# disanda/Deep-GAN-Encoders

Measured on AMD Instinct MI355X. Metric: encoder-train images/sec (E_align_s2 step, StyleGAN2 FFHQ-1024), higher is better.
Workload: dtype bf16; 1 GPU; E_align_s2 two-phase step, StyleGAN2-1024 G (train mode) + BE(startf=16, L=9) + LPIPS-VGG16 (seeded stand-in weights), batch 8/GPU; global_batch=8, img_size=1024, parallelism=dp1

## Files before the change

deep-gan-encoders_amd/_lib.py:

```python
import ctypes as C
import os

_HERE = os.path.dirname(os.path.abspath(__file__))
LIB_PATH = os.environ.get("DGE_LIB_PATH", os.path.join(_HERE, "libdge_hip.so"))


class DgeError(RuntimeError):
    pass


class ConvDesc(C.Structure):
    _fields_ = [
        ("x", C.c_void_p), ("w_packed", C.c_void_p), ("y", C.c_void_p), ("addend", C.c_void_p), ("dot_src", C.c_void_p),
        ("in_scale", C.c_void_p), ("in_shift", C.c_void_p), ("out_scale", C.c_void_p),
        ("bias", C.c_void_p), ("noise", C.c_void_p), ("noise_w", C.c_void_p), ("stats", C.c_void_p),
        ("B", C.c_int), ("H", C.c_int), ("W", C.c_int), ("Cin", C.c_int), ("Cout", C.c_int),
        ("ksize", C.c_int), ("up", C.c_int), ("in_s2d", C.c_int), ("noise_batch", C.c_int), ("noise_w_per_channel", C.c_int),
        ("act", C.c_int), ("bias_scale", C.c_float), ("gain", C.c_float), ("add_scale", C.c_float),
        ("dtype", C.c_int), ("in_up2", C.c_int), ("in_relu", C.c_int), ("stats_slots", C.c_int), ("w_layout", C.c_int),
        ("prep", C.c_int), ("prep_gain", C.c_float), ("prep_noise", C.c_void_p), ("prep_ns", C.c_void_p), ("prep_noise_batch", C.c_int),
        ("prep_stats", C.c_void_p), ("mask_relu", C.c_int), ("in_t2d", C.c_int),
        ("rgb_w", C.c_void_p), ("rgb_style", C.c_void_p), ("rgb_bias", C.c_void_p), ("rgb_out", C.c_void_p), ("rgb_wscale", C.c_float),
        ("rgb_skip_y", C.c_int), ("pool_out", C.c_int), ("pool_mask", C.c_void_p),
        ("prefetch_w", C.c_void_p), ("prefetch_ntot", C.c_int), ("prefetch_cin", C.c_int), ("in_bwd_coef", C.c_void_p),
        ("in_bwd_extra", C.c_void_p), ("in_bwd_extra_scale", C.c_float), ("fr_img4", C.c_void_p), ("fr_out", C.c_void_p),
    ]


class ConvPPDesc(C.Structure):
    _fields_ = [
        ("x", C.c_void_p), ("w_pp", C.c_void_p), ("y", C.c_void_p), ("w_bstride", C.c_longlong),
        ("out_scale", C.c_void_p), ("bias", C.c_void_p), ("noise", C.c_void_p), ("noise_w", C.c_void_p),
        ("B", C.c_int), ("H", C.c_int), ("W", C.c_int), ("Cin", C.c_int), ("Cout", C.c_int),
        ("noise_batch", C.c_int), ("noise_w_per_channel", C.c_int), ("act", C.c_int), ("bias_scale", C.c_float), ("gain", C.c_float),
        ("dgrad", C.c_int), ("in_s2d", C.c_int), ("stats_slots", C.c_int), ("prep", C.c_int), ("prep_noise_batch", C.c_int), ("mask_relu", C.c_int),
        ("in_t2d", C.c_int), ("add_scale", C.c_float), ("prep_gain", C.c_float),
        ("dot_src", C.c_void_p), ("addend", C.c_void_p), ("stats", C.c_void_p), ("prep_stats", C.c_void_p), ("prep_noise", C.c_void_p), ("prep_ns", C.c_void_p),
    ]


class DenseLayer(C.Structure):
    _fields_ = [("w", C.c_void_p), ("bias", C.c_void_p), ("I", C.c_int), ("O", C.c_int), ("wscale", C.c_float), ("bscale", C.c_float),
                ("add", C.c_float), ("act", C.c_int), ("gain", C.c_float)]


class S2GradEntry(C.Structure):
    _fields_ = [("P", C.c_void_p), ("st", C.c_void_p), ("d", C.c_void_p), ("s", C.c_void_p), ("bias", C.c_void_p), ("wsq", C.c_void_p),
                ("gs", C.c_void_p), ("wstyle", C.c_void_p),
                ("nslot_p", C.c_int), ("nslot_s", C.c_int), ("in_c", C.c_int), ("out_c", C.c_int), ("row", C.c_int), ("bscale", C.c_float)]


class SumPlanarEntry(C.Structure):
    _fields_ = [("partial", C.c_void_p), ("out", C.c_void_p), ("nslot", C.c_int), ("C", C.c_int), ("NS", C.c_int), ("pad", C.c_int)]


_P, _I, _F = C.c_void_p, C.c_int, C.c_float
SIGNATURES = {
    "dge_conv2d": [C.POINTER(ConvDesc), _P],
    "dge_fir_t2d": [_P, _P, _P, _I, _I, _I, _I, _I, _P],
    "dge_s2_style_grads": [C.POINTER(S2GradEntry), _I, _P, _I, _I, _I, _F, _P],
    "dge_conv_small_supported": [_I, _I, _I, _I, _I, _I, _I, _I],
    "dge_torgb_bwd_prep": [_P, _P, _P, _P, _P, _P, _I, _P, _P, _P, _I, _I, _I, _F, _F, _I, _P],
    "dge_demod_bwd_prep": [_P, _I, _P, _P, _P, _I, _I, _F, _P],
    "dge_sum_slots": [_P, _P, _I, _I, _I, _P],
    "dge_sum_slots_planar": [_P, _P, _I, _I, _I, _P],
    "dge_set_deterministic": [_I],
    "dge_get_deterministic": [],
    "dge_packed_n": [_I],
    "dge_pack_conv_weight": [_P, _P, _I, _I, _I, _I, _I, _F, _P],
    "dge_pack_conv_weights_multi": [_P, _P, _I, _I, _P],
    "dge_pack_desc_bytes": [],
    "dge_weight_sumsq": [_P, _P, _I, _I, _I, _F, _P],
    "dge_linear": [_P, _I, _P, _P, _P, _I, _I, _I, _I, _F, _F, _F, _I, _F, _I, _P],
    "dge_pixelnorm": [_P, _P, _I, _I, _F, _P],
    "dge_truncation": [_P, _P, _P, _I, _I, _I, _F, _I, _I, _P],
    "dge_torgb": [_P, _P, _P, _P, _P, _P, _I, _I, _I, _I, _F, _I, _P],
    "dge_conv_rgb_supported": [_I, _I, _I, _I, _I, _I, _I],
    "dge_conv_in_bwd_supported": [_I, _I, _I, _I, _I, _I, _I],
    "dge_conv_in_bwd_fromrgb_supported": [_I, _I, _I, _I, _I, _I, _I],
    "dge_conv_in_bwd_x_supported": [_I, _I, _I, _I, _I, _I, _I],
    "dge_conv_pool_supported": [_I, _I, _I, _I, _I, _I, _I],
    "dge_rgb_upsample_add": [_P, _P, _I, _I, _I, _P],
    "dge_nchw_to_nhwc": [_P, _P, _I, _I, _I, _I, _I, _P],
    "dge_nhwc_to_nchw": [_P, _P, _I, _I, _I, _I, _P],
    "dge_fromrgb": [_P, _P, _P, _P, _P, _I, _I, _I, _I, _P],
    "dge_fromrgb2": [_P, _P, _P, _P, _P, _P, _I, _I, _I, _I, _P],
    "dge_stats_finalize": [_P, _P, _P, _P, _I, _I, _I, _F, _P],
    "dge_stats_finalize_slots": [_P, _I, _P, _P, _P, _I, _I, _I, _F, _P],
    "dge_blend": [_P, _P, _P, _P, _P, _P, _I, _I, _I, _I, _I, _F, _F, _I, _P],
    "dge_loss_reduce": [_P, _P, _P, _I, _I, _I, _I, _I, _I, _I, _I, _P],
    "dge_ssim_fwd": [_P, _P, _P, _P, _I, _I, _I, _P],
    "dge_ssim_box7": [_P, _P, _P, _I, _I, _I, _F, _F, _F, _P],
    "dge_ssim_bwd": [_P, _P, _P, _P, _I, _I, _I, _F, _I, _P],
    "dge_space_loss_finalize": [_P, _P, _P, _P, _F, _F, _I, _P],
    "dge_space_loss_bwd": [_P, _P, _P, _P, _P, _I, _I, _I, _I, _I, _I, _I, _I, _F, _F, _I, _P],
    "dge_axpy_scalar": [_P, _P, _P, C.c_long, _F, _I, _P],
    "dge_lreq_adam_multi": [_I, _P, _P, _P, _P, _P, _F, _F, _P, _P, _P],
    "dge_modconv_bwd_prep": [_P, _P, _P, _P, _P, _P, _I, _I, _I, _I, _F, _I, _P],
    "dge_demod_bwd": [_P, _P, _P, _P, _P, _I, _I, _F, _P],
    "dge_linear_t": [_P, _I, _I, _P, _P, _P, _I, _I, _I, _I, _I, _F, _I, _P],
    "dge_torgb_bwd": [_P, _P, _P, _P, _P, _P, _I, _I, _I, _F, _I, _P],
    "dge_up2_bwd": [_P, _P, _I, _I, _I, _P],
    "dge_conv_wgrad": [_P, _P, _P, _P, _P, _I, _I, _I, _I, _I, _I, _I, _P],
    "dge_act_bwd": [_P, _P, _P, _P, _P, _I, _I, _I, _I, _I, _I, _F, _F, _I, _P],
    "dge_in_bwd_coef": [_P, _P, _P, _P, _P, _P, _I, _I, _I, _P],
    "dge_in_bwd_coef_slots": [_P, _I, _P, _P, _P, _P, _P, _I, _I, _I, _P],
    "dge_in_bwd": [_P, _P, _P, _P, _P, _P, _P, _I, _I, _I, _I, _I, _F, _I, _I, _P],
    "dge_chan_sum": [_P, _P, _I, _I, _I, _F, _I, _P],
    "dge_fromrgb_bwd": [_P, _P, _P, _P, _I, _I, _I, _I, _P],
    "dge_head_entry_size": [],
    "dge_heads_bwd": [_P, _I, _I, _P, _I, _P, _P, _P, _P, _I, _I, _P],
    "dge_head_rows_entry_size": [],
    "dge_heads_rows_fwd": [_P, _I, _P, _P, C.c_long, C.c_long, _I, _I, _I, _P],
    "dge_heads_rows_bwd": [_P, _I, _I, _P, C.c_long, C.c_long, _I, _P, _P, _P, _P, _I, _I, _P],
    "dge_dense_wgrad": [_P, _I, _P, _I, _P, _P, _I, _I, _I, _I, _P],
    "dge_lpips_prep": [_P, _P, _I, _I, _I, _P, _P, _I, _P],
    "dge_lpips_prep_bwd": [_P, _P, _I, _I, _I, _P, _F, _I, _I, _P],
    "dge_maxpool2": [_P, _P, _I, _I, _I, _I, _I, _P],
    "dge_maxpool2_bwd": [_P, _P, _P, _P, _I, _I, _I, _I, _I, _P],
    "dge_lpips_head": [_P, _P, _P, _P, _I, _I, _I, _F, _I, _P],
    "dge_mean": [_P, _P, _I, _P],
    "dge_blur_noise_act": [_P, _P, _P, _P, _P, _P, _I, _I, _I, _I, _I, _I, _I, _I, _P],
    "dge_affine_compose": [_P, _P, _P, _P, _P, _I, _I, _P],
    "dge_lerp_layers": [_P, _P, _I, _P, _P, _I, _I, _I, _P],
    "dge_linear_rows": [_P, _I, _P, _P, _P, _P, _P, _P, _I, _I, _I, _F, _F, _F, _P],
    "dge_demod_rows": [_P, _P, _P, _P, _P, _P, _P, _P, _I, _I, _F, _P],
    "dge_fromrgb_dgrad": [_P, _P, _P, _P, _I, _I, _I, _I, _P],
    "dge_nearest_up2": [_P, _P, _I, _I, _I, _I, _F, _I, _P],
    "dge_sg1_in_bwd_coef": [_P, _P, _P, _P, _P, _P, _I, _I, _I, _P],
    "dge_dot_stats": [_P, _P, _P, _I, _I, _I, _I, _P],
    "dge_nearest_up2_bwd": [_P, _P, _P, _P, _I, _I, _I, _I, _I, _P],
    "dge_pixelnorm_nhwc": [_P, _P, C.c_long, _I, _F, _I, _P],
    "dge_pixelnorm_nhwc_bwd": [_P, _P, _P, C.c_long, _I, _F, _I, _P],
    "dge_pixelnorm_act_bwd": [_P, _P, _P, _I, _I, _I, _I, _I, _I, _F, _I, _P],
    "dge_affine_relu_bwd": [_P, _P, _P, _P, _P, _P, _I, _I, _I, _I, _P],
    "dge_slice_up_bwd": [_P, _P, _I, _I, _I, _I, _I, _I, _I, _P],
    "dge_softmax_rows": [_P, C.c_long, _I, _I, _P],
    "dge_softmax_rows_bwd": [_P, _P, C.c_long, _I, _I, _P],
    "dge_rgb_tanh_bwd": [_P, _P, _P, _I, _I, _I, _I, _P],
    "dge_sn_group": [_P, _I, _I, _I, _P, _F, _I, _P],
    "dge_sn_entry_size": [],
    "dge_cbn_sn_wgrad_entry_size": [],
    "dge_cbn_sn_wgrad_group": [_P, _I, C.c_longlong, _I, _P, _I, _I, _P, _P],
    "dge_upconv_supported": [_I, _I, _I],
    "dge_pack_upconv_weight": [_P, _P, _I, _I, _F, _I, _P],
    "dge_upconv_fir": [_P, _P, _P, _P, _P, _P, _I, _P, _I, _P, _F, _F, _I, _I, _I, _I, _I, _I, _I, _P],
    "dge_up_dgrad_stream_supported": [_I, _I, _I, _I, _I, _I],
    "dge_up_dgrad_stream": [_P, _P, _P, _P, _P, _P, _P, _P, _I, _I, _F, _P, _I, _P, _P, _I, _I, _I, _I, _I, _I, _P],
    "dge_cbn_affine": [_P, _P, _I, _P, _P, _F, _P, _P, _I, _I, _P],
    "dge_slice_up": [_P, _P, _I, _I, _I, _I, _I, _I, _I, _P],
    "dge_attention": [_P, _P, _P, _P, _I, _I, _I, _I, _I, _I, _P],
    "dge_rgb_tanh": [_P, _P, _I, _I, _I, _I, _P],
    "dge_guided_relu_bwd": [_P, _P, _P, C.c_long, _I, _I, _P],
    "dge_maxpool2_relu_bwd": [_P, _P, _P, _I, _I, _I, _I, _I, _I, _P],
    "dge_maxpool2_bwd_relu": [_P, _P, _P, _P, _I, _I, _I, _I, _I, _P],
    "dge_adaptive_pool7": [_P, _P, _I, _I, _I, _I, _I, _P],
    "dge_adaptive_pool7_bwd": [_P, _P, _I, _I, _I, _I, _I, _P],
    "dge_class_target": [_P, _P, _P, _P, _I, _I, _P],
    "dge_gather_row": [_P, _P, _P, _I, _I, _F, _P],
    "dge_class_target_rows": [_P, _P, _P, _P, _I, _I, _P],
    "dge_gather_rows": [_P, _P, _P, _I, _I, _P],
    "dge_campp_map": [_P, _P, _P, _P, _P, _I, _I, _I, _I, _I, _P],
    "dge_cam_resize": [_P, _P, _P, _I, _I, _I, _I, _I, _P],
    "dge_mask2cam_blocks": [_I],
    "dge_mask2cam": [_P, _P, _P, _P, _P, _P, _P, _I, _I, _P],
    "dge_mask2cam_rows": [_P, _P, _P, _P, _P, _P, _I, _I, _P],
    "dge_class_target_groups": [_P, _P, _P, _P, _I, _I, _I, _P],
    "dge_gather_row_groups": [_P, _P, _P, _I, _I, _I, _F, _P],
    "dge_mask2cam_groups": [_P, _P, _P, _P, _P, _P, _P, _I, _I, _I, _P],
    "dge_randn": [_P, _I, _P, _P, _P, _P, C.c_ulonglong, _P, _P],
    "dge_version": [],
    "dge_env_reload": [],
    "dge_blend_pool_mask": [_P, _P, _P, _P, _P, _I, _I, _I, _I, _F, _F, _I, _P],
    "dge_act_bwd_mask": [_P, _P, _P, _P, _P, _I, _I, _I, _I, _I, _F, _F, _I, _P],
    "dge_loss_reduce3": [_P, _P, _P, _I, _I, _I, _I, _P, _I, _P],
    "dge_crop_pool_multi": [_P, _P, _P, _P, _I, _I, _I, _I, _P],
    "dge_space_loss_bwd3": [_P, _P, _P, _P, _P, _I, _I, _I, _P, _P, _P, _P, _I, _P],
    "dge_space_loss_bwd_split": [_P, _P, _P, _P, _P, _I, _I, _I, _P, _P, _P, _P, _I, _P],
    "dge_in_bwd_fromrgb": [_P, _P, _P, _I, _P, _P, _P, _P, _I, _P, _P, _P, _I, _I, _I, _I, _I, _F, _I, _P],
    "dge_in_bwd_fromrgb_img": [_P, _P, _P, _I, _P, _P, _P, _P, _I, _P, _P, _P, _P, _P, _I, _I, _I, _I, _I, _F, _I, _P],
    "dge_affine_bwd_fromrgb_img": [_P, _P, _P, _P, _P, _P, _P, _P, _I, _I, _I, _I, _I, _F, _I, _P],
    "dge_in_bwd_fused": [_P, _P, _P, _I, _P, _P, _P, _P, _I, _P, _P, _P, _P, _I, _I, _I, _I, _I, _F, _I, _I, _P],
    "dge_sum_slots_planar_multi": [C.POINTER(SumPlanarEntry), _I, _P],
    "dge_heads_fwd": [_P, _I, _P, _P, _I, _I, _I, _P],
    "dge_conv_pp_supported": [_I, _I, _I, _I, _I, _I],
    "dge_pack_conv_pp": [_P, _P, _I, _I, _F, _P, _P, _F, _I, _I, _P],
    "dge_dense_chain": [_P, _I, C.POINTER(DenseLayer), _I, _P, _I, _I, _I, _F, _P],
    "dge_conv_wgrad_dots": [_P, _P, _P, _P, _P, _P, _P, _I, _I, _I, _I, _I, _I, _I, _P],
    "dge_pack_conv_pp_rows": [_P, _I, _P, _I, _I, _P, _I, _P, _F, _I, _I, _P],
    "dge_conv_pp": [C.POINTER(ConvPPDesc), _P],
    "dge_up_pp_supported": [_I, _I, _I, _I, _I, _I],
    "dge_pack_up_pp": [_P, _P, _I, _I, _P, _P, _F, _I, _P],
    "dge_up_pp": [_P, _P, C.c_longlong, _P, _P, _I, _P, _P, _F, _F, _I, _I, _I, _I, _I, _I, _P],
    "dge_latent_pnorm_fwd": [_P, _P, _P, C.c_long, _I, _P],
    "dge_latent_pnorm_bwd": [_P, _P, _P, _P, C.c_long, _I, _F, _P],
    "dge_wplus_lerp": [_P, _P, _I, _F, _P, _I, _I, _I, _P],
    "dge_wplus_lerp_bwd": [_P, _F, _P, C.c_long, _I, _P],
    "dge_embed_track": [_P, _P, _P, C.c_long, _P, _P, _P, _P, _P, _I, _I, _I, _F, _F, _P],
    "dge_loss_reduce_rows": [_P, _P, _P, _I, _I, _I, _I, _P, _I, _I, _P],
    "dge_ssim_fwd_rows": [_P, _P, _P, _P, _I, _I, _I, _P],
    "dge_space_loss_finalize_rows": [_P, _I, _P, _P, _P, _P, _P, _I, _I, _P, _P, _I, _P],
    "dge_space_loss_bwd_rows": [_P, _P, _P, _P, _P, _I, _I, _I, _I, _P, _P, _P, _P, _I, _I, _P],
    "dge_latent_pnorm_rows_fwd": [_P, _P, _P, _I, C.c_long, _I, _P],
    "dge_latent_pnorm_rows_bwd": [_P, _P, _P, _P, _I, C.c_long, _I, _F, _P],
    "dge_embed_track_rows": [_P, _P, _P, _I, C.c_long, _P, _P, _P, _P, _P, _I, _I, _I, _F, _F, _P],
    "dge_mapping_bwd": [_P, _I, C.POINTER(DenseLayer), _I, _P, _P, _I, _P, _P, _I, _I, _I, _F, _P],
    "dge_quantize_u8": [_P, _I, _P, _I, _I, _I, _I, _P],
    "dge_image_metrics_u8_work_bytes": [_I, _I, _I],
    "dge_image_metrics_u8": [_P, _P, _I, _I, _I, _P, _P, _P, _P, _P],
    "dge_minmax_unit_slots": [C.c_long],
    "dge_minmax_unit": [_P, _P, C.c_long, _P, _P],
}

_lib = None


def lib():
    global _lib
    if _lib is None:
        if not os.path.exists(LIB_PATH):
            raise DgeError(f"{LIB_PATH} is missing: build it with deep-gan-encoders_amd/csrc/build.sh "
                           "(__graft_entry__.build()). There is no fallback path.")
        _lib = C.CDLL(LIB_PATH)
        for name, args in SIGNATURES.items():
            fn = getattr(_lib, name)
            fn.argtypes = args
            fn.restype = C.c_int
        for name in ("dge_last_error", "dge_last_kernel"):
            getattr(_lib, name).restype = C.c_char_p
            getattr(_lib, name).argtypes = []
        if os.environ.get("DGE_DETERMINISTIC") == "1":
            import torch
            if torch.cuda.is_available() and _lib.dge_set_deterministic(1) != 0:
                raise DgeError("DGE_DETERMINISTIC=1: " + _lib.dge_last_error().decode())
    return _lib


def last_kernel():
    return lib().dge_last_kernel().decode()


def check(rc, what=""):
    if rc != 0:
        raise DgeError(f"{what} failed ({rc}): {lib().dge_last_error().decode()}")
```

deep-gan-encoders_amd/csrc/capi.hip:

```cpp
#include <stdarg.h>
#include <stdio.h>
#include "common.h"
#include "conv_params.h"
#include "../../include/dge_hip.h"

static thread_local char g_err[512] = "";
void dge_set_error(const char* fmt, ...) {
    va_list ap; va_start(ap, fmt); vsnprintf(g_err, sizeof(g_err), fmt, ap); va_end(ap);
}
extern "C" const char* dge_last_error(void) { return g_err; }
static thread_local char g_kernel[160] = "";
void dge_note_kernel(const char* fmt, ...) {
    va_list ap; va_start(ap, fmt); vsnprintf(g_kernel, sizeof(g_kernel), fmt, ap); va_end(ap);
}
extern "C" const char* dge_last_kernel(void) { return g_kernel; }
extern "C" int dge_version(void) { return 100; }

#include <vector>
static std::vector<void (*)(const DgeDet*)>& det_setters() { static std::vector<void (*)(const DgeDet*)> v; return v; }
void dge_det_register(void (*setter)(const DgeDet*)) { det_setters().push_back(setter); }
static DgeDet g_det_host = {0, nullptr, nullptr, 0, 0};
int dge_det_upload_failed = 0;
bool dge_det_fits(long long ndomains, long long nslots, long long L) {
    return !g_det_host.enabled || (ndomains * nslots * L <= g_det_host.ws_floats && ndomains <= (long long)g_det_host.ncounters);
}
extern "C" int dge_set_deterministic(int on) {
    if (on && !g_det_host.ws) {
        const long long nf = 32LL << 20;
        const int nc = 1 << 16;
        float* ws = nullptr; unsigned* ct = nullptr;
        DGE_CHECK(hipMalloc((void**)&ws, (size_t)nf * 4) == hipSuccess, "set_deterministic: workspace allocation failed");
        DGE_CHECK(hipMalloc((void**)&ct, (size_t)nc * 4) == hipSuccess, "set_deterministic: counter allocation failed");
        DGE_CHECK(hipMemset(ct, 0, (size_t)nc * 4) == hipSuccess, "set_deterministic: counter reset failed");
        g_det_host.ws = ws; g_det_host.counters = ct; g_det_host.ws_floats = nf; g_det_host.ncounters = nc;
    }
    g_det_host.enabled = on ? 1 : 0;
    DGE_CHECK(hipDeviceSynchronize() == hipSuccess, "set_deterministic: device synchronisation failed");
    dge_det_upload_failed = 0;
    for (auto f : det_setters()) f(&g_det_host);
    DGE_CHECK(hipDeviceSynchronize() == hipSuccess && !dge_det_upload_failed, "set_deterministic: state upload failed");
    return 0;
}
extern "C" int dge_get_deterministic(void) { return g_det_host.enabled; }

static DgeEnv g_env;
static bool g_env_loaded = false;
static int env_int(const char* name, int dflt) { const char* e = getenv(name); return e ? atoi(e) : dflt; }
static void env_load() {
    g_env.force_stream = getenv("DGE_FORCE_STREAM") ? 1 : 0;
    g_env.no_stream = getenv("DGE_NO_STREAM") ? 1 : 0;
    g_env.no_pw = getenv("DGE_NO_PW") ? 1 : 0;
    g_env.stream_nseg = env_int("DGE_STREAM_NSEG", 0);
    g_env.conv_dbg = env_int("DGE_CONV_DBG", 0);
    g_env.conv_bn = env_int("DGE_CONV_BN", 0);
    g_env.conv_kc = env_int("DGE_CONV_KC", 0);
    g_env.conv_small = env_int("DGE_CONV_SMALL", -1);
    g_env.conv_nok4 = getenv("DGE_CONV_NOK4") ? 1 : 0;
    g_env.conv_nok2 = getenv("DGE_CONV_NOK2") ? 1 : 0;
    g_env.torgb_thread = getenv("DGE_TORGB_THREAD") ? 1 : 0;
    g_env.wgrad_th8 = getenv("DGE_WGRAD_TH8") ? 1 : 0;
    g_env.wgrad_groups = env_int("DGE_WGRAD_GROUPS", 0);
    if (g_env.wgrad_groups < 0) g_env.wgrad_groups = 0;
    g_env.up_dbg = env_int("DGE_UP_DBG", 0);
    { const char* v = getenv("DGE_UP_VARIANT"); g_env.up_variant = !v ? 0 : (v[0] == 's' ? 2 : 1); }
    g_env_loaded = true;
}
#include <mutex>
static std::once_flag g_env_once;
const DgeEnv& dge_env() { std::call_once(g_env_once, [] { if (!g_env_loaded) env_load(); }); return g_env; }
extern "C" void dge_env_reload(void) { env_load(); }

extern "C" int dge_conv2d(const dge_conv_desc* d, hipStream_t s) {
    DGE_CHECK(d && d->x && d->w_packed && d->y, "conv2d: null tensor");
    DGE_CHECK(d->B > 0 && d->H > 0 && d->W > 0 && d->Cin > 0 && d->Cout > 0, "conv2d: bad shape");
    DGE_CHECK(d->dtype == DGE_F32 || d->dtype == DGE_BF16, "conv2d: bad dtype %d", d->dtype);
    DGE_CHECK(!(d->up && d->stats), "conv2d: stats are not available in up mode");
    DGE_CHECK(!(d->up && d->in_s2d), "conv2d: up and in_s2d are exclusive");
    DGE_CHECK(!d->in_up2 || (!d->in_s2d && d->H % 2 == 0 && d->W % 2 == 0), "conv2d: in_up2 needs even H, W and no in_s2d");
    DGE_CHECK(!d->in_s2d || d->Cin % 4 == 0, "conv2d: in_s2d needs Cin %% 4 == 0");
    DGE_CHECK(!d->dot_src || d->stats || d->mask_relu || d->in_bwd_coef, "conv2d: dot_src needs a stats buffer");
    DGE_CHECK(!d->mask_relu || (d->dot_src && !d->prep && !d->up), "conv2d: mask_relu needs dot_src and excludes prep / up");
    DGE_CHECK(!d->in_relu || d->in_scale || d->in_shift, "conv2d: in_relu is applied together with the prologue affine");
    DGE_CHECK(d->gain > 0.f, "conv2d: gain must be positive (it is folded through the activation)");
    DGE_CHECK((((uintptr_t)d->in_scale | (uintptr_t)d->in_shift) & 15) == 0, "conv2d: in_scale/in_shift must be 16-byte aligned");
    DGE_CHECK(!d->noise || d->noise_w, "conv2d: noise without noise_w");
    ConvParams p;
    p.x = d->x; p.w = d->w_packed; p.y = d->y; p.addend = d->addend; p.dot_src = d->dot_src;
    p.in_scale = d->in_scale; p.in_shift = d->in_shift; p.out_scale = d->out_scale;
    p.bias = d->bias; p.noise = d->noise; p.noise_w = d->noise_w; p.stats = d->stats;
    p.B = d->B; p.H = d->H; p.W = d->W; p.Cin = d->Cin; p.Cout = d->Cout;
    p.Ntot_valid = d->up ? 4 * d->Cout : d->Cout;
    p.Ntot = dge_packed_n(p.Ntot_valid);
    p.up = d->up; p.in_s2d = d->in_s2d; p.in_up2 = d->in_up2; p.in_relu = d->in_relu;
    const int OH = d->up ? 2 * d->H : d->H, OW = d->up ? 2 * d->W : d->W;
    p.noise_bstride = d->noise_batch > 1 ? OH * OW : 0;
    p.noise_w_stride = d->noise_w_per_channel ? 1 : 0;
    p.act = d->act; p.bias_scale = d->bias_scale; p.gain = d->gain; p.add_scale = d->add_scale;
    p.tiles_x = p.tiles_y = 0;
    p.w_frag = d->w_layout == 1 ? 1 : 0;
    p.prep = d->prep ? 1 : 0;
    p.mask_relu = d->mask_relu ? 1 : 0;
    p.in_t2d = d->in_t2d ? 1 : 0;
    DGE_CHECK(!d->in_t2d || (d->ksize == 3 && !d->up && !d->in_s2d && !d->in_up2 && !d->in_scale && !d->in_shift && d->w_layout == 0),
              "conv2d: in_t2d is a plain 3x3 launch (no other read mode, no prologue affine, row-major weights)");
    p.prep_gain = d->prep_gain; p.prep_noise = d->prep_noise; p.prep_ns = d->prep_ns; p.prep_stats = d->prep_stats;
    p.prep_noise_bstride = d->prep_noise_batch > 1 ? OH * OW : 0;
    DGE_CHECK(!d->prep || (d->dot_src && d->prep_stats && d->prep_gain > 0.f && !d->up), "conv2d: prep needs dot_src, prep_stats, a positive prep_gain and no up mode");
    DGE_CHECK(!d->prep || !dge_get_deterministic(), "conv2d: the fused tail backward (prep) is not offered in deterministic mode; run dge_modconv_bwd_prep");
    DGE_CHECK(d->w_layout == 0 || d->w_layout == 1, "conv2d: bad w_layout %d", d->w_layout);
    p.stats_slots = d->stats_slots > 0 ? d->stats_slots : 1;
    p.rgb_w = d->rgb_out ? d->rgb_w : nullptr; p.rgb_style = d->rgb_style; p.rgb_bias = d->rgb_bias; p.rgb_out = d->rgb_out;
    p.rgb_wscale = d->rgb_wscale; p.rgb_skip_y = (d->rgb_out && d->rgb_skip_y) ? 1 : 0;
    p.pool_out = d->pool_out ? 1 : 0; p.pool_mask = d->pool_out ? (unsigned*)d->pool_mask : nullptr;
    const bool pf = d->w_layout == 1 && d->prefetch_w && d->prefetch_ntot >= 64 && d->prefetch_ntot % 64 == 0 &&
                    (d->prefetch_cin == 512 || d->prefetch_cin == 256);
    p.pf_w = pf ? d->prefetch_w : nullptr; p.pf_ntot = pf ? d->prefetch_ntot : 0; p.pf_cin = pf ? d->prefetch_cin : 0;
    p.in_coef = d->in_bwd_coef;
    p.in_extra = d->in_bwd_coef ? d->in_bwd_extra : nullptr; p.in_extra_scale = d->in_bwd_extra_scale;
    p.fr_img4 = d->in_bwd_coef ? d->fr_img4 : nullptr; p.fr_out = d->in_bwd_coef ? d->fr_out : nullptr;
    if (d->in_bwd_coef) {
        DGE_CHECK(!dge_get_deterministic(), "conv2d: in_bwd_coef is not offered in deterministic mode; run dge_in_bwd");
        DGE_CHECK(d->ksize == 3 && !d->up && dge_conv_stream_eligible(p, d->dtype, d->ksize), "conv2d: in_bwd_coef is offered where "
                  "dge_conv_in_bwd_supported() says so, with dot_src and prep_stats, without stats / prep");
    }
    if (d->pool_out)
        DGE_CHECK(!d->up && dge_conv_pool_ok(p, d->dtype, d->ksize), "conv2d: the pooled epilogue is offered where dge_conv_pool_supported() "
                  "says so (conv_2 of the first encoder blocks on the streaming kernel)");
    if (d->rgb_out) {
        DGE_CHECK(d->rgb_w && d->rgb_style && d->rgb_bias, "conv2d: rgb_out needs rgb_w, rgb_style, rgb_bias");
        DGE_CHECK(dge_conv_rgb_ok(p, d->dtype, d->ksize), "conv2d: the fused toRGB is offered where dge_conv_rgb_supported() says so "
                  "(bf16 3x3 32 -> 32 launches of the streaming kernel)");
    }
    return dge_conv_launch(p, d->dtype, d->ksize, s);
}

extern "C" int dge_conv_pool_supported(int B, int H, int W, int Cin, int Cout, int ksize, int dtype) {
    ConvParams p = {};
    p.B = B; p.H = H; p.W = W; p.Cin = Cin; p.Cout = Cout; p.Ntot_valid = Cout; p.Ntot = dge_packed_n(Cout);
    p.in_shift = (const float*)16; p.noise_w_stride = 1;
    return dge_conv_pool_ok(p, dtype, ksize) ? 1 : 0;
}

extern "C" int dge_conv_in_bwd_supported(int B, int H, int W, int Cin, int Cout, int ksize, int dtype) {
    ConvParams p = {};
    p.B = B; p.H = H; p.W = W; p.Cin = Cin; p.Cout = Cout; p.Ntot_valid = Cout; p.Ntot = dge_packed_n(Cout);
    p.dot_src = (const void*)16; p.prep_stats = (float*)16; p.in_coef = (const float*)16;
    return (ksize == 3 && !dge_get_deterministic() && dge_conv_stream_eligible(p, dtype, ksize)) ? 1 : 0;
}
extern "C" int dge_conv_in_bwd_x_supported(int B, int H, int W, int Cin, int Cout, int ksize, int dtype) {
    ConvParams p = {};
    p.B = B; p.H = H; p.W = W; p.Cin = Cin; p.Cout = Cout; p.Ntot_valid = Cout; p.Ntot = dge_packed_n(Cout);
    p.dot_src = (const void*)16; p.in_coef = (const float*)16;
    return (ksize == 3 && !dge_get_deterministic() && dge_conv_stream_eligible(p, dtype, ksize)) ? 1 : 0;
}
extern "C" int dge_conv_in_bwd_fromrgb_supported(int B, int H, int W, int Cin, int Cout, int ksize, int dtype) {
    ConvParams p = {};
    p.B = B; p.H = H; p.W = W; p.Cin = Cin; p.Cout = Cout; p.Ntot_valid = Cout; p.Ntot = dge_packed_n(Cout);
    p.dot_src = (const void*)16; p.in_coef = (const float*)16; p.fr_img4 = (const float*)16; p.fr_out = (float*)16;
    return (ksize == 3 && !dge_get_deterministic() && dge_conv_stream_eligible(p, dtype, ksize)) ? 1 : 0;
}

extern "C" int dge_conv_rgb_supported(int B, int H, int W, int Cin, int Cout, int ksize, int dtype) {
    ConvParams p = {};
    p.B = B; p.H = H; p.W = W; p.Cin = Cin; p.Cout = Cout; p.Ntot_valid = Cout; p.Ntot = dge_packed_n(Cout);
    return dge_conv_rgb_ok(p, dtype, ksize) ? 1 : 0;
}

__global__ void sum_slots_kernel(const float* __restrict__ partial, float* __restrict__ out, int nslot, int n, int accumulate) {
    const int i = blockIdx.x * blockDim.x + threadIdx.x;
    if (i >= n) return;
    float s = 0.f;
    int k = 0;
    for (; k + 8 <= nslot; k += 8) {
        float v[8];
#pragma unroll
        for (int j = 0; j < 8; j++) v[j] = partial[(size_t)(k + j) * n + i];
#pragma unroll
        for (int j = 0; j < 8; j++) s += v[j];
    }
    for (; k < nslot; k++) s += partial[(size_t)k * n + i];
    out[i] = accumulate ? out[i] + s : s;
}
__global__ void sum_slots_planar_kernel(const float* __restrict__ partial, float* __restrict__ out, int nslot, int C, int NS) {
    const int i = blockIdx.x * blockDim.x + threadIdx.x;
    if (i >= C * NS) return;
    float s = 0.f;
    int k = 0;
    for (; k + 8 <= nslot; k += 8) {
        float v[8];
#pragma unroll
        for (int j = 0; j < 8; j++) v[j] = partial[(size_t)(k + j) * C * NS + i];
#pragma unroll
        for (int j = 0; j < 8; j++) s += v[j];
    }
    for (; k < nslot; k++) s += partial[(size_t)k * C * NS + i];
    out[(size_t)(i % NS) * C + i / NS] = s;
}
extern "C" int dge_sum_slots_planar(const float* partial, float* out, int nslot, int C, int NS, hipStream_t s) {
    DGE_CHECK(nslot >= 1 && C >= 1 && NS >= 1, "sum_slots_planar: bad sizes");
    hipLaunchKernelGGL(sum_slots_planar_kernel, dim3((C * NS + 255) / 256), dim3(256), 0, s, partial, out, nslot, C, NS);
    DGE_LAUNCH_CHECK("sum_slots_planar");
    return 0;
}
struct SumPlanarTable { dge_sum_planar_entry e[32]; };
__global__ void sum_slots_planar_multi_kernel(SumPlanarTable tab) {
    const dge_sum_planar_entry e = tab.e[blockIdx.y];
    const int n = e.C * e.NS;
    for (int i = blockIdx.x * blockDim.x + threadIdx.x; i < n; i += gridDim.x * blockDim.x) {
        float s = 0.f;
        int k = 0;
        for (; k + 8 <= e.nslot; k += 8) {
            float v[8];
#pragma unroll
            for (int j = 0; j < 8; j++) v[j] = e.partial[(size_t)(k + j) * n + i];
#pragma unroll
            for (int j = 0; j < 8; j++) s += v[j];
        }
        for (; k < e.nslot; k++) s += e.partial[(size_t)k * n + i];
        e.out[(size_t)(i % e.NS) * e.C + i / e.NS] = s;
    }
}
extern "C" int dge_sum_slots_planar_multi(const dge_sum_planar_entry* entries, int n, hipStream_t s) {
    DGE_CHECK(entries && n >= 1 && n <= 32, "sum_slots_planar_multi: 1..32 entries");
    SumPlanarTable tab;
    int maxn = 1;
    for (int i = 0; i < n; i++) {
        const dge_sum_planar_entry& e = entries[i];
        DGE_CHECK(e.partial && e.out && e.nslot >= 1 && e.C >= 1 && e.NS >= 1, "sum_slots_planar_multi: bad entry %d", i);
        tab.e[i] = e;
        if (e.C * e.NS > maxn) maxn = e.C * e.NS;
    }
    hipLaunchKernelGGL(sum_slots_planar_multi_kernel, dim3((maxn + 255) / 256, n), dim3(256), 0, s, tab);
    DGE_LAUNCH_CHECK("sum_slots_planar_multi");
    return 0;
}
extern "C" int dge_sum_slots(const float* partial, float* out, int nslot, int n, int accumulate, hipStream_t s) {
    hipLaunchKernelGGL(sum_slots_kernel, dim3((n + 255) / 256), dim3(256), 0, s, partial, out, nslot, n, accumulate);
    DGE_LAUNCH_CHECK("sum_slots");
    return 0;
}
```

deep-gan-encoders_amd/csrc/conv_params.h:

```cpp
#pragma once
#include <hip/hip_runtime.h>

struct ConvParams {
    const void* x;
    const void* w;
    void* y;
    const void* addend;
    const void* dot_src;
    const float* in_scale;
    const float* in_shift;
    const float* out_scale;
    const float* bias;
    const float* noise;
    const float* noise_w;
    float* stats;
    int stats_slots;
    int B, H, W, Cin, Cout;
    int Ntot;
    int Ntot_valid;
    int up;
    int in_s2d;
    int in_relu;
    int in_up2;
    int noise_bstride;
    int noise_w_stride;
    int act;
    float bias_scale, gain, add_scale;
    int tiles_x, tiles_y;
    int dbg;
    int w_frag;
    int prep;
    float prep_gain;
    const float* prep_noise;
    const float* prep_ns;
    int prep_noise_bstride;
    float* prep_stats;
    int mask_relu;
    int in_t2d;
    const float* rgb_w;
    const float* rgb_style;
    const float* rgb_bias;
    float* rgb_out;
    float rgb_wscale;
    int rgb_skip_y;
    int pool_out;
    unsigned* pool_mask;
    const void* pf_w;
    int pf_ntot, pf_cin;
    const float* in_coef;
    const void* in_extra; float in_extra_scale; const float* fr_img4; float* fr_out;
};

int dge_conv_launch(const ConvParams& p, int dtype, int ksize, hipStream_t s);
extern "C" int dge_conv_ntile(int ntot);

bool dge_conv_stream_eligible(const ConvParams& p, int dtype, int ksize);
int dge_conv_stream_launch(const ConvParams& p, hipStream_t s);
bool dge_conv_rgb_ok(const ConvParams& p, int dtype, int ksize);
bool dge_conv_pool_ok(const ConvParams& p, int dtype, int ksize);
bool dge_conv_small_shape_ok(int H, int W, int cin, int ntot, int ksize, int in_s2d, int in_up2, int dtype);
int dge_conv_small_launch(const ConvParams& p, hipStream_t s);
bool dge_conv_pw_eligible(const ConvParams& p, int dtype, int ksize);
int dge_conv_pw_launch(const ConvParams& p, hipStream_t s);
```

deep-gan-encoders_amd/csrc/conv_small.hip:

```cpp
#include <stdlib.h>
#include "common.h"
#include "conv_params.h"
#include "conv_epilogue.h"

namespace {

struct SmallCfg {
    static constexpr int MT = 1, NT = 1, WTM = 32, WTN = 32, BM = 64;
    static constexpr int ESTR = 32 * 4 + 16;
};
constexpr int TH = 8, TW = 8, BN = 64, HH = 10, HW = 10, CIN_MAX = 512;
__host__ __device__ constexpr int pstr_of(int cin) { return 2 * cin + 16; }
__host__ __device__ constexpr int rpitch_of(int cin) { return HW * pstr_of(cin) + 224; }
constexpr int A_MAX = HH * rpitch_of(CIN_MAX);
constexpr int RED_BYTES = 8 * 2 * 16 * 64 * 4;
constexpr int EST_BYTES = 4 * 32 * SmallCfg::ESTR;
constexpr int N_BYTES = 4 * SmallCfg::BM * 4;
constexpr int PF_BYTES = 8 * 256;
constexpr int LDS_BYTES = A_MAX + N_BYTES + PF_BYTES;
static_assert(RED_BYTES + EST_BYTES <= A_MAX, "reduction + staging must fit the halo region");

__device__ __forceinline__ unsigned lds_base_u32(const void* p) {
    return (unsigned)(size_t)(const __attribute__((address_space(3))) unsigned char*)p;
}
__device__ __forceinline__ f32x16_t mma(const uint4& a, const uint4& b, f32x16_t c) {
    return __builtin_amdgcn_mfma_f32_32x32x16_bf16(*(const bf16x8_t*)&a, *(const bf16x8_t*)&b, c, 0, 0, 0);
}

template <int KQ, int MODE>
__global__ __launch_bounds__(512, 2) void conv_small_kernel(ConvParams p) {
    constexpr int CIN = KQ * 64, CH = CIN / 8;
    constexpr int PSTR = pstr_of(CIN), RPITCH = rpitch_of(CIN);
    constexpr int KST = CIN / 16;
    __shared__ __attribute__((aligned(256))) unsigned char lds[LDS_BYTES];
    float* ldsN = (float*)(lds + A_MAX);
    const int tid = threadIdx.x, lane = tid & 63;
    const int wave = __builtin_amdgcn_readfirstlane(tid >> 6);
    int bid = blockIdx.x;
    {
        const int nb = gridDim.x, per = nb >> 3;
        if (per > 0 && bid < (per << 3)) bid = (bid & 7) * per + (bid >> 3);
    }
    const int vbid = bid;
    const int tx_i = bid % p.tiles_x; bid /= p.tiles_x;
    const int ty_i = bid % p.tiles_y; bid /= p.tiles_y;
    const int b = bid % p.B;
    const int ntile = bid / p.B;
    const int x0 = tx_i * TW, y0 = ty_i * TH, bn0 = ntile * BN;
    const int nt = wave & 1, kq = wave >> 1;

    const unsigned char* wbase = (const unsigned char*)p.w + ((size_t)(bn0 / 32 + nt) * KST + kq * KQ) * 1024 + lane * 16;
    const size_t tap_stride = (size_t)(p.Ntot / 32) * KST * 1024;
    constexpr int PF = KQ >= 8 ? 3 : 4;
    uint4 bw[PF + 1][KQ];
#pragma unroll
    for (int t = 0; t < PF; t++)
#pragma unroll
        for (int j = 0; j < KQ; j++) bw[t][j] = *(const uint4*)(wbase + t * tap_stride + j * 1024);

    auto prefetch_next = [&]() {
        const int xcd = blockIdx.x & 7, r = blockIdx.x >> 3, R = max(1, (int)gridDim.x >> 3);
        const int nt_n = p.pf_ntot / BN, kst_n = p.pf_cin / 16;
        const int n_lo = xcd * nt_n / 8, n_hi = max(n_lo + 1, (xcd + 1) * nt_n / 8);
        const unsigned lines_tap = (unsigned)(n_hi - n_lo) * 2u * kst_n * 8u;
        const unsigned nlines = 9u * lines_tap;
        const size_t tap_stride_n = (size_t)(p.pf_ntot / 32) * kst_n * 1024;
        const unsigned m0v = lds_base_u32(lds) + A_MAX + N_BYTES + wave * 256;
        for (unsigned l = (unsigned)r * 512u + tid; l - lane < nlines; l += (unsigned)R * 512u) {
            const unsigned tp = l / lines_tap, within = l - tp * lines_tap;
            const unsigned char* a = (const unsigned char*)p.pf_w + tp * tap_stride_n + (size_t)n_lo * 2 * kst_n * 1024 + (size_t)within * 128;
            if (l >= nlines) a = (const unsigned char*)p.pf_w;
            asm volatile("s_mov_b32 m0, %1\n\ts_nop 0\n\tglobal_load_lds_dword %0, off" : : "v"(a), "s"(m0v) : "memory");
        }
    };
    const bool pf_late = gridDim.x <= 256;
    if (p.pf_w && !pf_late) prefetch_next();

    {
        const bf16_t* __restrict__ Xb = (const bf16_t*)p.x + (size_t)b * p.H * p.W * CIN;
        const bool affine = p.in_scale || p.in_shift;
        const int chunk = tid % CH;
        float asc[8], ash[8];
        if (affine) {
            const int ci = b * CIN + chunk * 8;
#pragma unroll
            for (int e = 0; e < 8; e++) { asc[e] = p.in_scale ? p.in_scale[ci + e] : 1.f; ash[e] = p.in_shift ? p.in_shift[ci + e] : 0.f; }
        }
        constexpr int NITEM = HH * HW * CH, NPER = (NITEM + 511) / 512;
        uint4 v[NPER];
        unsigned inmask = 0;
#pragma unroll
        for (int i = 0; i < NPER; i++) {
            const int idx = tid + i * 512;
            const int pix = idx / CH, hx = pix % HW, hy = pix / HW;
            const int gy = y0 + hy - 1, gx = x0 + hx - 1;
            const bool inside = ((unsigned)gy < (unsigned)p.H) & ((unsigned)gx < (unsigned)p.W) & (idx < NITEM);
            v[i] = make_uint4(0, 0, 0, 0);
            if (inside) v[i] = *(const uint4*)(Xb + (gy * p.W + gx) * CIN + chunk * 8);
            inmask |= (inside ? 1u : 0u) << i;
        }
        const float* __restrict__ nz_src = p.prep ? p.prep_noise : p.noise;
        if (nz_src) {
            const int nz_bs = p.prep ? p.prep_noise_bstride : p.noise_bstride;
            const int OWn = p.up ? 2 * p.W : p.W;
            const int nph = p.up ? 4 : 1;
            for (int idx = tid; idx < nph * SmallCfg::BM; idx += 512) {
                const int m = idx % SmallCfg::BM, ph = idx / SmallCfg::BM;
                const int gy = y0 + m / TW, gx = x0 + m % TW;
                const int oy = p.up ? 2 * gy + (ph >> 1) : gy, ox = p.up ? 2 * gx + (ph & 1) : gx;
                ldsN[idx] = (gy < p.H && gx < p.W) ? nz_src[(size_t)b * nz_bs + (size_t)oy * OWn + ox] : 0.f;
            }
        }
#pragma unroll
        for (int i = 0; i < NPER; i++) {
            const int idx = tid + i * 512;
            if (idx < NITEM) {
                const int pix = idx / CH, hx = pix % HW, hy = pix / HW;
                uint4 q = v[i];
                if (affine && ((inmask >> i) & 1u)) {
                    float f[8];
                    unpack16(q, f, (bf16_t*)nullptr);
#pragma unroll
                    for (int e = 0; e < 8; e++) f[e] = f[e] * asc[e] + ash[e];
                    if (p.in_relu) {
#pragma unroll
                        for (int e = 0; e < 8; e++) f[e] = fmaxf(f[e], 0.f);
                    }
                    q = pack16(f, (bf16_t*)nullptr);
                }
                *(uint4*)(lds + hy * RPITCH + hx * PSTR + chunk * 16) = q;
            }
        }
    }
    __syncthreads();

    f32x16_t acc[2];
#pragma unroll
    for (int g = 0; g < 2; g++)
#pragma unroll
        for (int r = 0; r < 16; r++) acc[g][r] = 0.f;
    int aoff[2];
#pragma unroll
    for (int g = 0; g < 2; g++) {
        const int m = g * 32 + (lane & 31);
        aoff[g] = (m / TW) * RPITCH + (m % TW) * PSTR + kq * KQ * 32 + (lane >> 5) * 16;
    }
    StaticFor<9>::run([&](auto tc) {
        constexpr int tap = decltype(tc)::value;
        constexpr int dy = tap / 3, dx = tap % 3;
        if (tap + PF < 9) {
            const unsigned char* wn = wbase + (size_t)(tap + PF) * tap_stride;
#pragma unroll
            for (int j = 0; j < KQ; j++) bw[(tap + PF) % (PF + 1)][j] = *(const uint4*)(wn + j * 1024);
        }
        const unsigned char* at = lds + dy * RPITCH + dx * PSTR;
#pragma unroll
        for (int j = 0; j < KQ; j++) {
            const uint4 a0 = *(const uint4*)(at + aoff[0] + j * 32);
            const uint4 a1 = *(const uint4*)(at + aoff[1] + j * 32);
            acc[0] = mma(a0, bw[tap % (PF + 1)][j], acc[0]);
            acc[1] = mma(a1, bw[tap % (PF + 1)][j], acc[1]);
        }
    });

    if (p.pf_w && pf_late) prefetch_next();
    __syncthreads();
    float* red = (float*)lds;
#pragma unroll
    for (int g = 0; g < 2; g++)
#pragma unroll
        for (int r = 0; r < 16; r++) red[((wave * 2 + g) * 16 + r) * 64 + lane] = acc[g][r];
    __syncthreads();
    const bool carrier = wave < 4;
    f32x16_t tile[1][1];
    if (carrier) {
        const int wm = wave >> 1, wn = wave & 1;
#pragma unroll
        for (int r = 0; r < 16; r++) {
            float s = 0.f;
#pragma unroll
            for (int q = 0; q < 4; q++) s += red[(((q * 2 + wn) * 2 + wm) * 16 + r) * 64 + lane];
            tile[0][0][r] = s;
        }
    }
    conv_epilogue<bf16_t, SmallCfg, TH, TW, BN, 2, 2, 512, MODE>(p, tile, lds + RED_BYTES, ldsN, b, x0, y0, bn0, ntile, vbid, tx_i, ty_i,
                                                            wave, lane, tid, carrier);
    if (p.pf_w) asm volatile("s_waitcnt vmcnt(0)" ::: "memory");
}

int max_hw() {
    static const int v = [] { const char* e = getenv("DGE_SMALL_MAXHW"); const int n = e ? atoi(e) : 24; return n < 0 ? 0 : n; }();
    return v;
}

}

bool dge_conv_small_shape_ok(int H, int W, int cin, int ntot, int ksize, int in_s2d, int in_up2, int dtype) {
    return dtype == DGE_BF16 && ksize == 3 && !in_s2d && !in_up2 && (cin == 512 || cin == 256) && ntot % BN == 0 && ntot >= BN &&
           H <= max_hw() && W <= max_hw();
}

extern "C" int dge_conv_small_supported(int H, int W, int cin, int ntot, int ksize, int in_s2d, int in_up2, int dtype) {
    return dge_conv_small_shape_ok(H, W, cin, ntot, ksize, in_s2d, in_up2, dtype) ? 1 : 0;
}

int dge_conv_small_launch(const ConvParams& p0, hipStream_t s) {
    ConvParams p = p0;
    p.dbg = 0;
    p.tiles_x = (p.W + TW - 1) / TW;
    p.tiles_y = (p.H + TH - 1) / TH;
    const long grid = (long)p.tiles_x * p.tiles_y * p.B * (p.Ntot / BN);
    DGE_CHECK(grid > 0 && grid < (1L << 31), "conv_small: bad grid");
    if (p.stats && !p.up)
        DGE_CHECK(dge_det_fits((long long)p.B * (p.Ntot / BN), (long long)p.tiles_x * p.tiles_y * 2, BN * 2),
                  "conv_small: the deterministic-mode workspace is too small for this launch");
    dge_note_kernel("conv_small<bf16,8,8,64,%d>%s", p.Cin, p.prep ? "+prep" : "");
    const int mode = p.prep ? 2 : ((p.addend || p.dot_src) ? 1 : 0);
#define DGE_GO(KQ, MODE) hipLaunchKernelGGL((conv_small_kernel<KQ, MODE>), dim3((unsigned)grid), dim3(512), 0, s, p)
    if (p.Cin == 512) { if (mode == 2) DGE_GO(8, 2); else if (mode == 1) DGE_GO(8, 1); else DGE_GO(8, 0); }
    else { if (mode == 2) DGE_GO(4, 2); else if (mode == 1) DGE_GO(4, 1); else DGE_GO(4, 0); }
#undef DGE_GO
    DGE_LAUNCH_CHECK("conv_small");
    return 0;
}
```

deep-gan-encoders_amd/csrc/s2_kernels.hip:

```cpp
#include <stdlib.h>
#include "common.h"
#include <vector>
#include <algorithm>
#include <string.h>
#include "conv_params.h"

__device__ __forceinline__ float sg1_up_weight(const float* __restrict__ w, int c, int o, int Cout, int ph, int tap) {
    const int py = ph >> 1, px = ph & 1, dy = tap / 3 - 1, dx = tap % 3 - 1;
    const int ky = py + 1 - 2 * dy, kx = px + 1 - 2 * dx;
    if (ky < 0 || ky > 3 || kx < 0 || kx > 3) return 0.f;
    const float* w3 = w + ((size_t)c * Cout + o) * 9;
    float v = 0.f;
    for (int a = 0; a < 2; a++)
        for (int bq = 0; bq < 2; bq++) {
            const int y = ky - a, x = kx - bq;
            if (y >= 0 && y < 3 && x >= 0 && x < 3) v += w3[y * 3 + x];
        }
    return v;
}

__device__ __forceinline__ float upfold_weight(const float* __restrict__ w, int o, int i, int Cin, int ph, int tap) {
    const int py = ph >> 1, px = ph & 1;
    const int dy = tap / 3 - 1, dx = tap % 3 - 1;
    const float k1[4] = {0.25f, 0.75f, 0.75f, 0.25f};
    float v = 0.f;
    for (int ty = 0; ty < 4; ty++) {
        const int wy = 3 - py - ty + 2 * dy;
        if (wy < 0 || wy > 2) continue;
        for (int tx = 0; tx < 4; tx++) {
            const int wx = 3 - px - tx + 2 * dx;
            if (wx < 0 || wx > 2) continue;
            v += k1[ty] * k1[tx] * w[((size_t)o * Cin + i) * 9 + wy * 3 + wx];
        }
    }
    return v;
}

__device__ __forceinline__ float upt2d_weight(const float* __restrict__ w, int o, int i, int Cin, int ph, int tap) {
    const int dy = tap / 3, dx = tap % 3;
    if (dy == 0 || dx == 0) return 0.f;
    const int ky = 2 * (dy - 1) + (ph >> 1), kx = 2 * (dx - 1) + (ph & 1);
    if (ky > 2 || kx > 2) return 0.f;
    return w[((size_t)o * Cin + i) * 9 + (2 - ky) * 3 + (2 - kx)];
}

__device__ __forceinline__ size_t pack_out_index(int frag, int tap, int n, int k, int Ntot, int Kdim) {
    if (!frag) return ((size_t)tap * Ntot + n) * Kdim + k;
    const size_t blk = ((size_t)tap * (Ntot >> 5) + (n >> 5)) * (Kdim >> 4) + (k >> 4);
    return blk * 512 + (size_t)(((n & 31) + 32 * ((k & 15) >> 3)) * 8 + (k & 7));
}

template <typename T>
__global__ void pack_weight_kernel(const float* __restrict__ w, T* __restrict__ out, int Cout, int Cin, int KS,
                                   int Ntot, int mode, float scale) {
    const int frag = mode & 0x100;
    mode &= 0xff;
    const int ntap = KS * KS;
    const int Kdim = (mode == 2) ? Cout : ((mode == 3 || mode == 5 || mode == 6) ? 4 * Cout : Cin);
    const int total = ntap * Ntot * Kdim;
    for (int idx = blockIdx.x * blockDim.x + threadIdx.x; idx < total; idx += gridDim.x * blockDim.x) {
        const int k = idx % Kdim;
        const int n = (idx / Kdim) % Ntot;
        const int tap = idx / (Kdim * Ntot);
        float v = 0.f;
        if (mode == 0) {
            if (n < Cout) v = w[((size_t)n * Cin + k) * ntap + tap];
        } else if (mode == 2) {
            if (n < Cin) v = w[((size_t)k * Cin + n) * ntap + (ntap - 1 - tap)];
        } else if (mode == 1) {
            if (n < 4 * Cout) v = upfold_weight(w, n % Cout, k, Cin, n / Cout, tap);
        } else if (mode == 4) {
            if (n < 4 * Cout) v = sg1_up_weight(w, k, n % Cout, Cout, n / Cout, tap);
        } else if (mode == 5) {
            if (n < Cin) v = sg1_up_weight(w, n, k % Cout, Cout, k / Cout, 8 - tap);
        } else if (mode == 6) {
            if (n < Cin) v = upt2d_weight(w, k % Cout, n, Cin, k / Cout, tap);
        } else {
            if (n < Cin) v = upfold_weight(w, k % Cout, n, Cin, k / Cout, 8 - tap);
        }
        Elem<T>::st(out + pack_out_index(frag, tap, n, k, Ntot, Kdim), v * scale);
    }
}

struct DgePackDesc {
    const float* w; void* out;
    int cout, cin, ks, ntot, mode, dtype, kdim;
    float scale;
    long long pair_start;
    long long tile_start;
    void* out2;
    int ntot2, kdim2, mode2, tiles_i;
};
__device__ __forceinline__ float pack_gather(const float* __restrict__ w, int mode, int Cout, int Cin, int ntap, int n, int k, int tap) {
    if (mode == 0) return n < Cout ? w[((size_t)n * Cin + k) * ntap + tap] : 0.f;
    if (mode == 2) return n < Cin ? w[((size_t)k * Cin + n) * ntap + (ntap - 1 - tap)] : 0.f;
    if (mode == 1) return n < 4 * Cout ? upfold_weight(w, n % Cout, k, Cin, n / Cout, tap) : 0.f;
    if (mode == 4) return n < 4 * Cout ? sg1_up_weight(w, k, n % Cout, Cout, n / Cout, tap) : 0.f;
    if (mode == 5) return n < Cin ? sg1_up_weight(w, n, k % Cout, Cout, k / Cout, 8 - tap) : 0.f;
    if (mode == 6) return n < Cin ? upt2d_weight(w, k % Cout, n, Cin, k / Cout, tap) : 0.f;
    return n < Cin ? upfold_weight(w, k % Cout, n, Cin, k / Cout, 8 - tap) : 0.f;
}
__global__ void pack_multi_kernel(const DgePackDesc* __restrict__ descs, int nd, long long total_pairs) {
    for (long long pidx = (long long)blockIdx.x * blockDim.x + threadIdx.x; pidx < total_pairs; pidx += (long long)gridDim.x * blockDim.x) {
        int lo = 0, hi = nd - 1;
        while (lo < hi) { const int mid = (lo + hi + 1) >> 1; if (descs[mid].pair_start <= pidx) lo = mid; else hi = mid - 1; }
        const DgePackDesc e = descs[lo];
        const long long local = pidx - e.pair_start;
        const int k = (int)(local % e.kdim), n = (int)(local / e.kdim);
        const int ntap = e.ks * e.ks;
        for (int tap = 0; tap < ntap; tap++) {
            const float v = pack_gather(e.w, e.mode & 0xff, e.cout, e.cin, ntap, n, k, tap) * e.scale;
            const size_t o = pack_out_index(e.mode & 0x100, tap, n, k, e.ntot, e.kdim);
            if (e.dtype == DGE_BF16) ((bf16_t*)e.out)[o] = f2bf(v);
            else ((float*)e.out)[o] = v;
        }
    }
}

constexpr int PK_LDW = 32 * 9 + 1;
template <bool TR>
__device__ __forceinline__ void pack_emit_bf16(const float* __restrict__ tile, int ntap, int n0, int k0, bf16_t* __restrict__ out, int ntot, int kdim,
                                               int frag, float scale) {
    for (int idx = threadIdx.x; idx < 128 * ntap; idx += 256) {
        const int kc = idx & 3, nn = (idx >> 2) & 31, tap = idx >> 7;
        const int n = n0 + nn, k = k0 + kc * 8;
        if (k >= kdim || n >= ntot) continue;
        float v[8];
#pragma unroll
        for (int j = 0; j < 8; j++)
            v[j] = scale * (!TR ? tile[nn * PK_LDW + (kc * 8 + j) * ntap + tap] : tile[(kc * 8 + j) * PK_LDW + nn * ntap + (ntap - 1 - tap)]);
        *(uint4*)(out + pack_out_index(frag, tap, n, k, ntot, kdim)) =
            make_uint4(pack2bf(v[0], v[1]), pack2bf(v[2], v[3]), pack2bf(v[4], v[5]), pack2bf(v[6], v[7]));
    }
}
__global__ __launch_bounds__(256) void pack_multi_tiled_kernel(const DgePackDesc* __restrict__ descs, int nd, long long total_tiles) {
    __shared__ float tile[32 * PK_LDW];
    constexpr int NDL = 512;
    __shared__ long long tstart[NDL];
    const bool lds_search = nd <= NDL;
    if (lds_search) {
        for (int i = threadIdx.x; i < nd; i += 256) tstart[i] = descs[i].tile_start;
        __syncthreads();
    }
    for (long long tix = blockIdx.x; tix < total_tiles; tix += gridDim.x) {
        int lo = 0, hi = nd - 1;
        if (lds_search) { while (lo < hi) { const int mid = (lo + hi + 1) >> 1; if (tstart[mid] <= tix) lo = mid; else hi = mid - 1; } }
        else { while (lo < hi) { const int mid = (lo + hi + 1) >> 1; if (descs[mid].tile_start <= tix) lo = mid; else hi = mid - 1; } }
        const DgePackDesc e = descs[lo];
        const int local = (int)(tix - e.tile_start);
        const int ntap = e.ks * e.ks, mode = e.mode & 0xff, frag = e.mode & 0x100;
        const bool paired = e.out2 != nullptr;
        const int kt = paired ? e.tiles_i : (e.kdim + 31) / 32;
        const int n0 = (local / kt) * 32, k0 = (local % kt) * 32;
        const bool staged = (mode == 0 || mode == 2) && ntap <= 9;
        __syncthreads();
        if (staged) {
            const int o0 = mode == 0 ? n0 : k0, i0 = mode == 0 ? k0 : n0;
            const int run = 32 * ntap;
            const int iv = min(32, e.cin - i0);
            if ((e.cin & 3) == 0 && ntap == 9) {
                const int upr = iv > 0 ? iv * 9 / 4 : 0;
                float4 v[9];
                int rr[9], cc[9];
#pragma unroll
                for (int q = 0; q < 9; q++) {
                    const int u = threadIdx.x + q * 256;
                    rr[q] = u / 72; cc[q] = u - rr[q] * 72;
                    const int o = o0 + rr[q];
                    v[q] = make_float4(0.f, 0.f, 0.f, 0.f);
                    if (o < e.cout && cc[q] < upr) v[q] = *(const float4*)(e.w + ((size_t)o * e.cin + i0) * 9 + cc[q] * 4);
                }
#pragma unroll
                for (int q = 0; q < 9; q++) {
                    float* t = tile + rr[q] * PK_LDW + cc[q] * 4;
                    t[0] = v[q].x; t[1] = v[q].y; t[2] = v[q].z; t[3] = v[q].w;
                }
            } else {
                for (int idx = threadIdx.x; idx < 32 * run; idx += 256) {
                    const int r = idx / run, c = idx - r * run;
                    const int o = o0 + r, i = i0 + c / ntap;
                    tile[r * PK_LDW + c] = (o < e.cout && i < e.cin) ? e.w[((size_t)o * e.cin + i0) * ntap + c] : 0.f;
                }
            }
            __syncthreads();
        }
        if (staged && e.dtype == DGE_BF16 && (e.kdim & 7) == 0) {
            if (mode == 0) pack_emit_bf16<false>(tile, ntap, n0, k0, (bf16_t*)e.out, e.ntot, e.kdim, frag, e.scale);
            else pack_emit_bf16<true>(tile, ntap, n0, k0, (bf16_t*)e.out, e.ntot, e.kdim, frag, e.scale);
            if (paired) pack_emit_bf16<true>(tile, ntap, k0, n0, (bf16_t*)e.out2, e.ntot2, e.kdim2, e.mode2 & 0x100, e.scale);
            continue;
        }
        for (int idx = threadIdx.x; idx < 1024 * ntap; idx += 256) {
            const int kk = idx & 31, nn = (idx >> 5) & 31, tap = idx >> 10;
            const int n = n0 + nn, k = k0 + kk;
            if (k >= e.kdim) continue;
            float v;
            if (staged) v = mode == 0 ? tile[nn * PK_LDW + kk * ntap + tap] : tile[kk * PK_LDW + nn * ntap + (ntap - 1 - tap)];
            else v = pack_gather(e.w, mode, e.cout, e.cin, ntap, n, k, tap);
            v *= e.scale;
            const size_t o = pack_out_index(frag, tap, n, k, e.ntot, e.kdim);
            if (e.dtype == DGE_BF16) ((bf16_t*)e.out)[o] = f2bf(v);
            else ((float*)e.out)[o] = v;
        }
    }
}

__global__ void wsq_kernel(const float* __restrict__ w, float* __restrict__ wsq, int n_oi, int ntap, float scale2) {
    const int idx = blockIdx.x * blockDim.x + threadIdx.x;
    if (idx >= n_oi) return;
    float s = 0.f;
    for (int t = 0; t < ntap; t++) { const float v = w[(size_t)idx * ntap + t]; s += v * v; }
    wsq[idx] = s * scale2;
}

enum { LIN_ACT_NONE = 0, LIN_ACT_LRELU = 1, LIN_ACT_RELU = 2, LIN_ACT_RSQRT = 3 };
__global__ void linear_kernel(const float* __restrict__ x, int ldx, const float* __restrict__ W,
                              const float* __restrict__ bias, float* __restrict__ y, int ldy, int B, int I, int O,
                              float wscale, float bscale, float add, int act, float gain, int square) {
    const int wave = (blockIdx.x * blockDim.x + threadIdx.x) >> 6, lane = threadIdx.x & 63;
    if (wave >= B * O) return;
    const int b = wave / O, o = wave % O;
    const float* xr = x + (size_t)b * ldx;
    const float* wr = W + (size_t)o * I;
    float s = 0.f;
    for (int i = lane; i < I; i += 64) { float xv = xr[i]; if (square) xv *= xv; s += xv * wr[i]; }
    s = wave_sum(s);
    if (lane == 0) {
        float v = s * wscale + (bias ? bias[o] * bscale : 0.f) + add;
        if (act == LIN_ACT_LRELU) v = v > 0.f ? v : 0.2f * v;
        else if (act == LIN_ACT_RELU) v = v > 0.f ? v : 0.f;
        else if (act == LIN_ACT_RSQRT) v = rsqrtf(v);
        y[(size_t)b * ldy + o] = v * gain;
    }
}

struct DenseChain { const float* w[8]; const float* bias[8]; int I[8], O[8], act[8]; float wscale[8], bscale[8], add[8], gain[8]; int n; };
__global__ __launch_bounds__(1024) void dense_chain_kernel(const float* __restrict__ x, int ldx, DenseChain c, float* __restrict__ y, int ldy,
                                                           int pixelnorm, float eps) {
    __shared__ float buf[2][1024];
    const int b = blockIdx.x, tid = threadIdx.x, wave = tid >> 6, lane = tid & 63;
    const int I0 = c.I[0];
    if (pixelnorm) {
        if (wave == 0) {
            float s = 0.f;
            for (int i = lane; i < I0; i += 64) { const float v = x[(size_t)b * ldx + i]; s += v * v; }
            s = wave_sum(s);
            const float r = rsqrtf(s / I0 + eps);
            for (int i = lane; i < I0; i += 64) buf[0][i] = x[(size_t)b * ldx + i] * r;
        }
    } else {
        for (int i = tid; i < I0; i += 1024) buf[0][i] = x[(size_t)b * ldx + i];
    }
    __syncthreads();
    int cur = 0;
    for (int l = 0; l < c.n; l++) {
        const int I = c.I[l], O = c.O[l];
        const float* __restrict__ W = c.w[l];
        const float* __restrict__ bias = c.bias[l];
        const bool last = l == c.n - 1;
        for (int o = wave; o < O; o += 16) {
            const float* wr = W + (size_t)o * I;
            float s = 0.f;
            for (int i = lane; i < I; i += 64) s += buf[cur][i] * wr[i];
            s = wave_sum(s);
            if (lane == 0) {
                float v = s * c.wscale[l] + (bias ? bias[o] * c.bscale[l] : 0.f) + c.add[l];
                if (c.act[l] == LIN_ACT_LRELU) v = v > 0.f ? v : 0.2f * v;
                else if (c.act[l] == LIN_ACT_RELU) v = v > 0.f ? v : 0.f;
                v *= c.gain[l];
                if (last) y[(size_t)b * ldy + o] = v; else buf[cur ^ 1][o] = v;
            }
        }
        __syncthreads();
        cur ^= 1;
    }
}

__global__ void linear_rows_kernel(const float* __restrict__ x, int ldx_b, const int* __restrict__ row_xoff,
                                   const float* __restrict__ W, const float* __restrict__ bias, float* __restrict__ y,
                                   const int* __restrict__ row_ybase, const int* __restrict__ row_ybstride, int B, int R, int K,
                                   float wscale, float bscale, float add) {
    const int wave = (blockIdx.x * blockDim.x + threadIdx.x) >> 6, lane = threadIdx.x & 63;
    if (wave >= B * R) return;
    const int b = wave / R, r = wave % R;
    const float* xr = x + (size_t)b * ldx_b + row_xoff[r];
    const float* wr = W + (size_t)r * K;
    float s = 0.f;
    for (int i = lane; i < K; i += 64) s += xr[i] * wr[i];
    s = wave_sum(s);
    if (lane == 0) y[(size_t)row_ybase[r] + (size_t)b * row_ybstride[r]] = s * wscale + bias[r] * bscale + add;
}

__global__ void demod_rows_kernel(const float* __restrict__ s_all, const float* __restrict__ wsq_cat, const int* __restrict__ row_woff,
                                  const int* __restrict__ row_sbase, const int* __restrict__ row_cin, float* __restrict__ d_all,
                                  const int* __restrict__ row_dbase, const int* __restrict__ row_dbstride, int B, int R, float eps) {
    const int wave = (blockIdx.x * blockDim.x + threadIdx.x) >> 6, lane = threadIdx.x & 63;
    if (wave >= B * R) return;
    const int b = wave / R, r = wave % R;
    const int cin = row_cin[r];
    const float* sr = s_all + (size_t)row_sbase[r] + (size_t)b * cin;
    const float* wr = wsq_cat + (size_t)row_woff[r];
    float a = 0.f;
    for (int i = lane; i < cin; i += 64) { const float v = sr[i]; a += v * v * wr[i]; }
    a = wave_sum(a);
    if (lane == 0) d_all[(size_t)row_dbase[r] + (size_t)b * row_dbstride[r]] = rsqrtf(a + eps);
}

__global__ void pixelnorm_kernel(const float* __restrict__ x, float* __restrict__ y, int B, int D, float eps) {
    const int wave = (blockIdx.x * blockDim.x + threadIdx.x) >> 6, lane = threadIdx.x & 63;
    if (wave >= B) return;
    float s = 0.f;
    for (int i = lane; i < D; i += 64) { const float v = x[(size_t)wave * D + i]; s += v * v; }
    s = wave_sum(s);
    const float r = rsqrtf(s / D + eps);
    for (int i = lane; i < D; i += 64) y[(size_t)wave * D + i] = x[(size_t)wave * D + i] * r;
}

__global__ void truncation_kernel(const float* __restrict__ w, const float* __restrict__ w_avg, float* __restrict__ wp,
                                  int B, int L, int D, float psi, int layers, int w_is_wp, int apply) {
    const long idx = blockIdx.x * (long)blockDim.x + threadIdx.x;
    if (idx >= (long)B * L * D) return;
    const int d = idx % D, l = (idx / D) % L, b = idx / ((long)D * L);
    const float v = w_is_wp ? w[idx] : w[(size_t)b * D + d];
    if (!apply) { wp[idx] = v; return; }
    const float coef = l < layers ? psi : 1.f;
    wp[idx] = w_avg[d] + (v - w_avg[d]) * coef;
}

template <typename T, int NC>
__global__ void torgb_kernel(const T* __restrict__ x, const float* __restrict__ wrgb, const float* __restrict__ s,
                             const float* __restrict__ bias, const float* __restrict__ prev, float* __restrict__ img,
                             int B, int H, int W, int Cin, float wscale) {
    extern __shared__ float wl[];
    const int b = blockIdx.y;
    for (int i = threadIdx.x; i < NC * Cin; i += blockDim.x) wl[i] = wrgb[i] * wscale * s[(size_t)b * Cin + i % Cin];
    __syncthreads();
    constexpr int EP16 = Elem<T>::PER16;
    const int HW = H * W;
    for (int pix = blockIdx.x * blockDim.x + threadIdx.x; pix < HW; pix += gridDim.x * blockDim.x) {
        const T* xp = x + ((size_t)b * HW + pix) * Cin;
        float acc[NC];
#pragma unroll
        for (int c = 0; c < NC; c++) acc[c] = 0.f;
        for (int i = 0; i < Cin; i += EP16) {
            const uint4 v = *(const uint4*)(xp + i);
            float f[EP16];
            unpack16(v, f, (T*)nullptr);
#pragma unroll
            for (int e = 0; e < EP16; e++)
#pragma unroll
                for (int c = 0; c < NC; c++) acc[c] += f[e] * wl[c * Cin + i + e];
        }
        const int y = pix / W, xx = pix % W;
#pragma unroll
        for (int c = 0; c < NC; c++) {
            float v = acc[c] + bias[c];
            if (prev) {
                const int h2 = H >> 1, w2 = W >> 1;
                const float* pp = prev + ((size_t)b * NC + c) * h2 * w2;
                const int my = y >> 1, mx = xx >> 1;
                const int ya = (y & 1) ? my : my - 1, yb = (y & 1) ? my + 1 : my;
                const int xa = (xx & 1) ? mx : mx - 1, xb = (xx & 1) ? mx + 1 : mx;
                const float wya = (y & 1) ? 0.75f : 0.25f, wyb = 1.f - wya;
                const float wxa = (xx & 1) ? 0.75f : 0.25f, wxb = 1.f - wxa;
                auto at = [&](int yy, int xq) { return (yy >= 0 && yy < h2 && xq >= 0 && xq < w2) ? pp[yy * w2 + xq] : 0.f; };
                v += wya * (wxa * at(ya, xa) + wxb * at(ya, xb)) + wyb * (wxa * at(yb, xa) + wxb * at(yb, xb));
            }
            img[((size_t)b * NC + c) * HW + pix] = v;
        }
    }
}

template <typename T, int NC>
__global__ __launch_bounds__(256) void torgb_wave_kernel(const T* __restrict__ x, const float* __restrict__ wrgb, const float* __restrict__ s,
                                                         const float* __restrict__ bias, const float* __restrict__ prev, float* __restrict__ img,
                                                         int B, int H, int W, int Cin, float wscale) {
    constexpr int EP16 = Elem<T>::PER16;
    const int lane = threadIdx.x & 63;
    const int HW = H * W;
    const long gp = (long)blockIdx.x * 4 + (threadIdx.x >> 6);
    if (gp >= (long)B * HW) return;
    const int b = (int)(gp / HW), pix = (int)(gp - (long)b * HW);
    const T* xp = x + (size_t)gp * Cin;
    float acc[NC];
#pragma unroll
    for (int c = 0; c < NC; c++) acc[c] = 0.f;
    for (int i = lane * EP16; i < Cin; i += 64 * EP16) {
        float f[EP16], sv[EP16];
        unpack16(*(const uint4*)(xp + i), f, (T*)nullptr);
#pragma unroll
        for (int e4 = 0; e4 < EP16 / 4; e4++) *(float4*)&sv[e4 * 4] = *(const float4*)(s + (size_t)b * Cin + i + e4 * 4);
#pragma unroll
        for (int e = 0; e < EP16; e++) f[e] *= sv[e];
#pragma unroll
        for (int c = 0; c < NC; c++) {
            float wv[EP16];
#pragma unroll
            for (int e4 = 0; e4 < EP16 / 4; e4++) *(float4*)&wv[e4 * 4] = *(const float4*)(wrgb + (size_t)c * Cin + i + e4 * 4);
#pragma unroll
            for (int e = 0; e < EP16; e++) acc[c] = fmaf(f[e], wv[e], acc[c]);
        }
    }
#pragma unroll
    for (int c = 0; c < NC; c++) acc[c] = wave_sum(acc[c]) * wscale;
    if (lane < NC) {
        const int c = lane;
        float v = bias[c];
#pragma unroll
        for (int k = 0; k < NC; k++) v += (k == c) ? acc[k] : 0.f;
        if (prev) {
            const int y = pix / W, xx = pix % W;
            const int h2 = H >> 1, w2 = W >> 1;
            const float* pp = prev + ((size_t)b * NC + c) * h2 * w2;
            const int my = y >> 1, mx = xx >> 1;
            const int ya = (y & 1) ? my : my - 1, yb = (y & 1) ? my + 1 : my;
            const int xa = (xx & 1) ? mx : mx - 1, xb = (xx & 1) ? mx + 1 : mx;
            const float wya = (y & 1) ? 0.75f : 0.25f, wyb = 1.f - wya;
            const float wxa = (xx & 1) ? 0.75f : 0.25f, wxb = 1.f - wxa;
            auto at = [&](int yy, int xq) { return (yy >= 0 && yy < h2 && xq >= 0 && xq < w2) ? pp[yy * w2 + xq] : 0.f; };
            v += wya * (wxa * at(ya, xa) + wxb * at(ya, xb)) + wyb * (wxa * at(yb, xa) + wxb * at(yb, xb));
        }
        img[((size_t)b * NC + c) * HW + pix] = v;
    }
}

template <typename T>
__global__ void nchw_to_nhwc_kernel(const float* __restrict__ src, T* __restrict__ dst, int B, int C, int HW, int src_B) {
    const long idx = blockIdx.x * (long)blockDim.x + threadIdx.x;
    if (idx >= (long)B * C * HW) return;
    const int c = idx % C; const long r = idx / C; const int pix = r % HW; const int b = r / HW;
    const int sb = src_B == 1 ? 0 : b;
    Elem<T>::st(dst + idx, src[((size_t)sb * C + c) * HW + pix]);
}
template <typename T>
__global__ void nhwc_to_nchw_kernel(const T* __restrict__ src, float* __restrict__ dst, int B, int C, int HW) {
    const long idx = blockIdx.x * (long)blockDim.x + threadIdx.x;
    if (idx >= (long)B * C * HW) return;
    const int pix = idx % HW; const long r = idx / HW; const int c = r % C; const int b = r / C;
    dst[idx] = Elem<T>::ld(src + ((size_t)b * HW + pix) * C + c);
}

__global__ void lerp_layers_kernel(const float* __restrict__ w, const float* __restrict__ avg, int avg_stride,
                                   const float* __restrict__ coefs, float* __restrict__ out, int B, int L, int D) {
    const long idx = blockIdx.x * (long)blockDim.x + threadIdx.x;
    if (idx >= (long)B * L * D) return;
    const int d = idx % D, l = (idx / D) % L, b = idx / ((long)D * L);
    const float a = avg[(size_t)l * avg_stride + d];
    out[idx] = a + (w[(size_t)b * D + d] - a) * coefs[l];
}

#include "../../include/dge_hip.h"

extern "C" int dge_lerp_layers(const float* w, const float* avg, int avg_stride, const float* coefs, float* out, int B, int L,
                               int D, hipStream_t s) {
    const long n = (long)B * L * D;
    hipLaunchKernelGGL(lerp_layers_kernel, dim3((unsigned)((n + 255) / 256)), dim3(256), 0, s, w, avg, avg_stride, coefs, out, B, L, D);
    DGE_LAUNCH_CHECK("lerp_layers");
    return 0;
}

extern "C" int dge_linear_rows(const float* x, int ldx_b, const int* row_xoff, const float* w, const float* bias, float* y,
                               const int* row_ybase, const int* row_ybstride, int B, int R, int K, float wscale, float bscale,
                               float add, hipStream_t s) {
    const long waves = (long)B * R;
    hipLaunchKernelGGL(linear_rows_kernel, dim3((unsigned)((waves + 3) / 4)), dim3(256), 0, s, x, ldx_b, row_xoff, w, bias, y, row_ybase,
                       row_ybstride, B, R, K, wscale, bscale, add);
    DGE_LAUNCH_CHECK("linear_rows");
    return 0;
}

extern "C" int dge_demod_rows(const float* s_all, const float* wsq_cat, const int* row_woff, const int* row_sbase, const int* row_cin,
                              float* d_all, const int* row_dbase, const int* row_dbstride, int B, int R, float eps, hipStream_t s) {
    const long waves = (long)B * R;
    hipLaunchKernelGGL(demod_rows_kernel, dim3((unsigned)((waves + 3) / 4)), dim3(256), 0, s, s_all, wsq_cat, row_woff, row_sbase, row_cin,
                       d_all, row_dbase, row_dbstride, B, R, eps);
    DGE_LAUNCH_CHECK("demod_rows");
    return 0;
}

extern "C" int dge_pack_conv_weight(const float* w_oihw, void* out, int cout, int cin, int ksize, int mode, int dtype,
                                    float scale, hipStream_t s) {
    const int frag = mode & 0x100;
    const int mode_full = mode;
    mode &= 0xff;
    DGE_CHECK(mode >= 0 && mode <= 6 && (mode_full & ~0x1ff) == 0, "pack: bad mode %d", mode_full);
    DGE_CHECK((mode != 1 && mode < 3) || ksize == 3, "pack: up fold needs a 3x3 kernel");
    const int nvalid = (mode == 1 || mode == 4) ? 4 * cout : (mode >= 2 ? cin : cout);
    const int ntot = dge_packed_n(nvalid);
    const int kdim = mode == 2 ? cout : ((mode == 3 || mode == 5 || mode == 6) ? 4 * cout : cin);
    DGE_CHECK(!frag || (dtype == DGE_BF16 && ntot % 32 == 0 && kdim % 16 == 0), "pack: fragment order needs bf16, N %% 32 == 0, K %% 16 == 0");
    mode = mode_full;
    const long total = (long)ksize * ksize * ntot * kdim;
    DGE_CHECK(total < (1L << 31) - (4096L * 256), "pack: weight too large (%ld elements)", total);
    const int grid = (int)((total + 255) / 256 > 4096 ? 4096 : (total + 255) / 256);
    if (dtype == DGE_BF16)
        hipLaunchKernelGGL(pack_weight_kernel<bf16_t>, dim3(grid), dim3(256), 0, s, w_oihw, (bf16_t*)out, cout, cin, ksize, ntot, mode, scale);
    else
        hipLaunchKernelGGL(pack_weight_kernel<float>, dim3(grid), dim3(256), 0, s, w_oihw, (float*)out, cout, cin, ksize, ntot, mode, scale);
    DGE_LAUNCH_CHECK("pack_conv_weight");
    return 0;
}

extern "C" int dge_pack_conv_weights_multi(const long long* table_host, void* descs_dev, int n, int upload, hipStream_t s) {
    DGE_CHECK(n > 0 && n <= 4096, "pack_multi: bad entry count %d", n);
    static thread_local std::vector<DgePackDesc> host;
    host.resize(n);
    long long pairs = 0, tiles = 0;
    for (int i = 0; i < n; i++) {
        const long long* r = table_host + (size_t)i * 8;
        DgePackDesc& d = host[i];
        d.w = (const float*)r[0]; d.out = (void*)r[1];
        d.cout = (int)(r[2] & 0xffffffffLL); d.cin = (int)(r[2] >> 32);
        d.ks = (int)(r[3] & 0xffffffffLL); d.mode = (int)(r[3] >> 32);
        d.dtype = (int)r[4];
        const unsigned bits = (unsigned)r[5]; memcpy(&d.scale, &bits, 4);
        const int bm = d.mode & 0xff;
        DGE_CHECK(bm >= 0 && bm <= 6 && (d.mode & ~0x1ff) == 0, "pack_multi: bad mode %d", d.mode);
        DGE_CHECK((bm != 1 && bm < 3) || d.ks == 3, "pack_multi: up fold needs a 3x3 kernel");
        const int nvalid = (bm == 1 || bm == 4) ? 4 * d.cout : (bm >= 2 ? d.cin : d.cout);
        d.ntot = dge_packed_n(nvalid);
        d.kdim = bm == 2 ? d.cout : ((bm == 3 || bm == 5 || bm == 6) ? 4 * d.cout : d.cin);
        DGE_CHECK(!(d.mode & 0x100) || (d.dtype == DGE_BF16 && d.ntot % 32 == 0 && d.kdim % 16 == 0),
                  "pack_multi: fragment order needs bf16, N %% 32 == 0, K %% 16 == 0");
        d.pair_start = pairs;
        pairs += (long long)d.ntot * d.kdim;
        d.out2 = nullptr; d.ntot2 = d.kdim2 = d.mode2 = d.tiles_i = 0;
        DGE_CHECK(d.ntot % 32 == 0, "pack_multi: packed N is padded to the N tile (multiple of 32)");
    }
    static int nopair = -1;
    if (nopair < 0) nopair = getenv("DGE_PACK_NOPAIR") ? 1 : 0;
    std::vector<char> absorbed(n, 0);
    if (!nopair)
        for (int i = 0; i < n; i++) {
            DgePackDesc& f = host[i];
            if ((f.mode & 0xff) != 0 || f.dtype != DGE_BF16 || f.ks != 3 || (f.kdim & 7) || absorbed[i]) continue;
            for (int j = 0; j < n; j++) {
                const DgePackDesc& g = host[j];
                if (j == i || absorbed[j] || g.out2 || (g.mode & 0xff) != 2 || g.w != f.w || g.dtype != DGE_BF16 || g.ks != 3 || (g.kdim & 7) ||
                    g.cout != f.cout || g.cin != f.cin || g.scale != f.scale)
                    continue;
                f.out2 = g.out; f.ntot2 = g.ntot; f.kdim2 = g.kdim; f.mode2 = g.mode;
                absorbed[j] = 1;
                break;
            }
        }
    for (int i = 0; i < n; i++) {
        DgePackDesc& d = host[i];
        d.tile_start = tiles;
        if (absorbed[i]) continue;
        if (d.out2) {
            const int to = std::max(d.ntot / 32, (d.kdim2 + 31) / 32);
            d.tiles_i = std::max((d.kdim + 31) / 32, d.ntot2 / 32);
            tiles += (long long)to * d.tiles_i;
        } else {
            tiles += (long long)(d.ntot / 32) * ((d.kdim + 31) / 32);
        }
    }
    if (upload) {
        hipStreamCaptureStatus cs = hipStreamCaptureStatusNone;
        if (hipStreamIsCapturing(s, &cs) == hipSuccess)
            DGE_CHECK(cs == hipStreamCaptureStatusNone, "pack_multi: the descriptor table changed inside a stream capture; run the step eagerly once first");
        hipError_t e = hipMemcpyAsync(descs_dev, host.data(), (size_t)n * sizeof(DgePackDesc), hipMemcpyHostToDevice, s);
        DGE_CHECK(e == hipSuccess, "pack_multi: descriptor upload failed: %s", hipGetErrorString(e));
    }
    static int untiled = -1;
    if (untiled < 0) untiled = getenv("DGE_PACK_UNTILED") ? 1 : 0;
    if (untiled) {
        long long blocks = (pairs + 255) / 256;
        const int grid = (int)(blocks > 8192 ? 8192 : blocks);
        hipLaunchKernelGGL(pack_multi_kernel, dim3(grid), dim3(256), 0, s, (const DgePackDesc*)descs_dev, n, pairs);
    } else {
        const int grid = (int)(tiles > 4096 ? 4096 : tiles);
        hipLaunchKernelGGL(pack_multi_tiled_kernel, dim3(grid), dim3(256), 0, s, (const DgePackDesc*)descs_dev, n, tiles);
    }
    DGE_LAUNCH_CHECK("pack_conv_weights_multi");
    return 0;
}
extern "C" int dge_pack_desc_bytes(void) { return (int)sizeof(DgePackDesc); }

extern "C" int dge_packed_n(int nvalid) {
    const int t = dge_conv_ntile(nvalid);
    return (nvalid + t - 1) / t * t;
}

extern "C" int dge_weight_sumsq(const float* w_oihw, float* wsq, int cout, int cin, int ksize, float scale, hipStream_t s) {
    const int n = cout * cin;
    hipLaunchKernelGGL(wsq_kernel, dim3((n + 255) / 256), dim3(256), 0, s, w_oihw, wsq, n, ksize * ksize, scale * scale);
    DGE_LAUNCH_CHECK("weight_sumsq");
    return 0;
}

extern "C" int dge_linear(const float* x, int ldx, const float* w, const float* bias, float* y, int ldy, int B, int I, int O,
                          float wscale, float bscale, float add, int act, float gain, int square_input, hipStream_t s) {
    DGE_CHECK(B > 0 && I > 0 && O > 0, "linear: bad shape");
    const long waves = (long)B * O;
    hipLaunchKernelGGL(linear_kernel, dim3((unsigned)((waves + 3) / 4)), dim3(256), 0, s, x, ldx, w, bias, y, ldy, B, I, O,
                       wscale, bscale, add, act, gain, square_input);
    DGE_LAUNCH_CHECK("linear");
    return 0;
}

extern "C" int dge_pixelnorm(const float* x, float* y, int B, int D, float eps, hipStream_t s) {
    hipLaunchKernelGGL(pixelnorm_kernel, dim3((B + 3) / 4), dim3(256), 0, s, x, y, B, D, eps);
    DGE_LAUNCH_CHECK("pixelnorm");
    return 0;
}

extern "C" int dge_dense_chain(const float* x, int ldx, const dge_dense_layer* layers, int n, float* y, int ldy, int B, int pixelnorm,
                               float eps, hipStream_t s) {
    DGE_CHECK(x && y && layers && n >= 1 && n <= 8 && B >= 1, "dense_chain: 1 .. 8 layers");
    DenseChain c;
    c.n = n;
    for (int l = 0; l < n; l++) {
        const dge_dense_layer& L = layers[l];
        DGE_CHECK(L.w && L.I >= 1 && L.I <= 1024 && L.O >= 1 && L.O <= 1024 && (l == 0 || L.I == layers[l - 1].O), "dense_chain: layer %d: widths up to 1024, I = previous O", l);
        DGE_CHECK(L.act == DGE_ACT_NONE || L.act == DGE_ACT_LRELU || L.act == DGE_ACT_RELU, "dense_chain: activation %d", L.act);
        c.w[l] = L.w; c.bias[l] = L.bias; c.I[l] = L.I; c.O[l] = L.O;
        c.act[l] = L.act == DGE_ACT_LRELU ? LIN_ACT_LRELU : (L.act == DGE_ACT_RELU ? LIN_ACT_RELU : LIN_ACT_NONE);
        c.wscale[l] = L.wscale; c.bscale[l] = L.bscale; c.add[l] = L.add; c.gain[l] = L.gain;
    }
    hipLaunchKernelGGL(dense_chain_kernel, dim3(B), dim3(1024), 0, s, x, ldx, c, y, ldy, pixelnorm ? 1 : 0, eps);
    DGE_LAUNCH_CHECK("dense_chain");
    return 0;
}

extern "C" int dge_truncation(const float* w, const float* w_avg, float* wp, int B, int L, int D, float psi, int layers,
                              int w_is_wp, hipStream_t s) {
    const long n = (long)B * L * D;
    const int apply = (psi < 1.0f && layers > 0) ? 1 : 0;
    hipLaunchKernelGGL(truncation_kernel, dim3((unsigned)((n + 255) / 256)), dim3(256), 0, s, w, w_avg, wp, B, L, D, psi,
                       layers, w_is_wp, apply);
    DGE_LAUNCH_CHECK("truncation");
    return 0;
}

extern "C" int dge_torgb(const void* x, const float* wrgb, const float* style, const float* bias, const float* prev,
                         float* img, int B, int H, int W, int cin, float wscale, int dtype, hipStream_t s) {
    const int esz = dtype == DGE_BF16 ? 2 : 4;
    DGE_CHECK(cin % (16 / esz) == 0, "torgb: Cin=%d not a multiple of %d", cin, 16 / esz);
    const int hw = H * W;
    if (cin >= 256 && cin % (64 * (16 / esz)) == 0 && (long)B * hw <= (1L << 16) && !dge_env().torgb_thread) {
        const unsigned nblk = (unsigned)(((long)B * hw + 3) / 4);
        if (dtype == DGE_BF16)
            hipLaunchKernelGGL((torgb_wave_kernel<bf16_t, 3>), dim3(nblk), dim3(256), 0, s, (const bf16_t*)x, wrgb, style, bias, prev, img, B, H, W, cin, wscale);
        else
            hipLaunchKernelGGL((torgb_wave_kernel<float, 3>), dim3(nblk), dim3(256), 0, s, (const float*)x, wrgb, style, bias, prev, img, B, H, W, cin, wscale);
        DGE_LAUNCH_CHECK("torgb");
        return 0;
    }
    int gx = (hw + 255) / 256; if (gx > 2048) gx = 2048;
    const size_t shm = (size_t)3 * cin * sizeof(float);
    if (dtype == DGE_BF16)
        hipLaunchKernelGGL((torgb_kernel<bf16_t, 3>), dim3(gx, B), dim3(256), shm, s, (const bf16_t*)x, wrgb, style, bias, prev, img, B, H, W, cin, wscale);
    else
        hipLaunchKernelGGL((torgb_kernel<float, 3>), dim3(gx, B), dim3(256), shm, s, (const float*)x, wrgb, style, bias, prev, img, B, H, W, cin, wscale);
    DGE_LAUNCH_CHECK("torgb");
    return 0;
}

__global__ __launch_bounds__(256) void rgb_upsample_add_kernel(float* __restrict__ img, const float* __restrict__ prev, int H, int W) {
    const int x = (blockIdx.x * 256 + threadIdx.x) * 4;
    if (x >= W) return;
    const int y = blockIdx.y, bc = blockIdx.z;
    const int h2 = H >> 1, w2 = W >> 1;
    const float* pp = prev + (size_t)bc * h2 * w2;
    const int my = y >> 1, mx = x >> 1;
    const int ya = (y & 1) ? my : my - 1, yb = ya + 1;
    const float wya = (y & 1) ? 0.75f : 0.25f, wyb = 1.f - wya;
    float v[4];
#pragma unroll
    for (int j = 0; j < 4; j++) {
        const int xq = mx - 1 + j;
        const bool xin = xq >= 0 && xq < w2;
        const float pa = (xin && ya >= 0) ? pp[(size_t)ya * w2 + xq] : 0.f, pb = (xin && yb < h2) ? pp[(size_t)yb * w2 + xq] : 0.f;
        v[j] = wya * pa + wyb * pb;
    }
    float4* ip = (float4*)(img + ((size_t)bc * H + y) * W + x);
    float4 o = *ip;
    o.x += 0.25f * v[0] + 0.75f * v[1]; o.y += 0.75f * v[1] + 0.25f * v[2];
    o.z += 0.25f * v[1] + 0.75f * v[2]; o.w += 0.75f * v[2] + 0.25f * v[3];
    *ip = o;
}
extern "C" int dge_rgb_upsample_add(float* img, const float* prev, int BC, int H, int W, hipStream_t s) {
    DGE_CHECK(img && prev && BC > 0 && H > 0 && W % 4 == 0 && H % 2 == 0 && H <= 65535 && BC <= 65535, "rgb_upsample_add: needs W %% 4 == 0, even H");
    hipLaunchKernelGGL(rgb_upsample_add_kernel, dim3((W / 4 + 255) / 256, H, BC), dim3(256), 0, s, img, prev, H, W);
    DGE_LAUNCH_CHECK("rgb_upsample_add");
    return 0;
}

extern "C" int dge_nchw_to_nhwc(const float* src, void* dst, int B, int C, int HW, int src_B, int dtype, hipStream_t s) {
    const long n = (long)B * C * HW;
    if (dtype == DGE_BF16)
        hipLaunchKernelGGL(nchw_to_nhwc_kernel<bf16_t>, dim3((unsigned)((n + 255) / 256)), dim3(256), 0, s, src, (bf16_t*)dst, B, C, HW, src_B);
    else
        hipLaunchKernelGGL(nchw_to_nhwc_kernel<float>, dim3((unsigned)((n + 255) / 256)), dim3(256), 0, s, src, (float*)dst, B, C, HW, src_B);
    DGE_LAUNCH_CHECK("nchw_to_nhwc");
    return 0;
}

extern "C" int dge_nhwc_to_nchw(const void* src, float* dst, int B, int C, int HW, int dtype, hipStream_t s) {
    const long n = (long)B * C * HW;
    if (dtype == DGE_BF16)
        hipLaunchKernelGGL(nhwc_to_nchw_kernel<bf16_t>, dim3((unsigned)((n + 255) / 256)), dim3(256), 0, s, (const bf16_t*)src, dst, B, C, HW);
    else
        hipLaunchKernelGGL(nhwc_to_nchw_kernel<float>, dim3((unsigned)((n + 255) / 256)), dim3(256), 0, s, (const float*)src, dst, B, C, HW);
    DGE_LAUNCH_CHECK("nhwc_to_nchw");
    return 0;
}
```

deep-gan-encoders_amd/ops.py:

```python
import ctypes as C
import math

import torch

from ._lib import lib, check, ConvDesc, ConvPPDesc, DgeError, last_kernel

F32, BF16 = 0, 1
ACT_NONE, ACT_LRELU, ACT_RELU, LIN_RSQRT = 0, 1, 2, 3
PACK_FWD, PACK_UPFOLD, PACK_DGRAD, PACK_UPFOLD_DGRAD, PACK_SG1_UP, PACK_SG1_UP_DGRAD, PACK_UPT2D_DGRAD = 0, 1, 2, 3, 4, 5, 6
PACK_FRAG = 0x100
import os as _os
import weakref as _weakref
KERNEL_LOG = None
PROFILE = None


class _ZeroArena:

    def __init__(self):
        self.buf, self.off, self.high, self.active = None, 0, 0, False


_ARENA = _ZeroArena()


def zero_arena_begin(device, nbytes=512 << 20):
    a = _ARENA
    if a.buf is None or a.buf.device != torch.device(device) or a.buf.numel() * 4 < nbytes:
        a.buf = torch.zeros(nbytes // 4, dtype=torch.float32, device=device)
    else:
        a.buf[:a.high].zero_()
    a.off, a.high, a.active = 0, 0, True


def zero_arena_end():
    _ARENA.active = False


def zeros(shape, device):
    a = _ARENA
    n = int(math.prod(shape))
    if a.active and a.buf.device == torch.device(device) and a.off + n <= a.buf.numel():
        t = a.buf[a.off:a.off + n].view(shape)
        a.off = (a.off + n + 63) & ~63
        a.high = max(a.high, a.off)
        return t
    return torch.zeros(shape, dtype=torch.float32, device=device)


class SlotStats:
    __slots__ = ("B", "C", "device", "buf", "nslot")

    def __init__(self, B, C, device):
        self.B, self.C, self.device, self.buf, self.nslot = B, C, device, None, 1

    def alloc(self, nslot):
        self.nslot = nslot
        self.buf = zeros((nslot, self.B, self.C, 2), self.device)
        return self.buf

    def plain(self):
        return self.alloc(1)[0]


def _sum_over_batch(partial, out=None):
    n = partial[0].numel()
    acc = out is not None
    if out is None:
        out = torch.empty(partial.shape[1:], dtype=torch.float32, device=partial.device)
    check(lib().dge_sum_slots(_p(partial), _p(out), partial.shape[0], n, 1 if acc else 0, _stream()), "dge_sum_slots")
    return out


class _Noise:

    def __init__(self):
        self.seed, self.counter, self.rank, self.world, self.seed_dev, self.graph_base = None, 0, 0, 1, None, 0


NOISE = _Noise()


def noise_seed(seed):
    NOISE.seed = int(seed) & 0xFFFFFFFFFFFFFFFF
    NOISE.counter = 0
    if NOISE.seed_dev is not None:
        NOISE.seed_dev.copy_(torch.tensor([NOISE.seed - (1 << 64) if NOISE.seed >= (1 << 63) else NOISE.seed], dtype=torch.int64))


def noise_dp(rank, world):
    NOISE.rank, NOISE.world = int(rank), int(world)


def noise_graph_begin(device):
    if NOISE.seed_dev is None or NOISE.seed_dev.device != torch.empty(0, device=device).device:
        NOISE.seed_dev = torch.zeros(1, dtype=torch.int64, device=device)
    NOISE.graph_base = NOISE.seed or 0
    if NOISE.seed is not None:
        noise_seed(NOISE.seed)


def noise_graph_seed(iteration):
    noise_seed(NOISE.graph_base + iteration + 1)


def randn_rows(shapes, device):
    if NOISE.seed is None:
        noise_seed(torch.initial_seed())
    n = len(shapes)
    sizes = [int(math.prod(sh)) for sh in shapes]
    starts, off = [], 0
    for sz in sizes:
        starts.append(off)
        off += (sz + 3) & ~3
    flat = torch.empty(max(off, 1), dtype=torch.float32, device=device)
    LL, ULL, UI = C.c_longlong * n, C.c_ulonglong * n, C.c_uint * n
    goff = [NOISE.rank * sz for sz in sizes]
    sub = [(NOISE.counter + k) & 0xFFFFFFFF for k in range(n)]
    NOISE.counter += n
    sd = C.c_void_p(NOISE.seed_dev.data_ptr()) if NOISE.seed_dev is not None else None
    check(lib().dge_randn(_p(flat), n, LL(*starts), LL(*sizes), ULL(*goff), UI(*sub), C.c_ulonglong(NOISE.seed), sd, _stream()),
          "dge_randn")
    return [flat[st:st + sz].view(sh) for st, sz, sh in zip(starts, sizes, shapes)]


def randn(shape, device):
    return randn_rows([tuple(shape)], device)[0]


def tdtype(dtype):
    return torch.bfloat16 if dtype == BF16 else torch.float32


def dtype_of(t):
    if t.dtype == torch.bfloat16:
        return BF16
    if t.dtype == torch.float32:
        return F32
    raise DgeError(f"unsupported activation dtype {t.dtype}")


_raw_stream = getattr(torch._C, "_cuda_getCurrentRawStream", None)
_raw_device = getattr(torch._C, "_cuda_getDevice", None)


def _stream():
    if _raw_stream is not None and _raw_device is not None:
        return C.c_void_p(_raw_stream(_raw_device()))
    return C.c_void_p(torch.cuda.current_stream().cuda_stream)


def _p(t):
    if t is None:
        return None
    if not t.is_cuda:
        raise DgeError("tensor is not on the GPU: the HIP path has no CPU fallback")
    if not t.is_contiguous():
        raise DgeError("tensor must be contiguous")
    return C.c_void_p(t.data_ptr())


def _f32(t):
    if t is not None and t.dtype != torch.float32:
        raise DgeError(f"expected float32, got {t.dtype}")
    return _p(t)


def packed_n(n):
    return lib().dge_packed_n(int(n))


def small_conv(H, W, kdim, nvalid, ksize=3, in_s2d=False, in_up2=False, dtype=BF16):
    return bool(lib().dge_conv_small_supported(int(H), int(W), int(kdim), packed_n(nvalid), int(ksize), int(bool(in_s2d)),
                                               int(bool(in_up2)), int(dtype)))


def _pack_io(w, mode):
    return (w.shape[1], w.shape[0]) if (mode & 0xff) in (PACK_SG1_UP, PACK_SG1_UP_DGRAD) else (w.shape[0], w.shape[1])


def pack_dims(w, mode):
    cout, cin = _pack_io(w, mode)
    mode &= 0xff
    nvalid = 4 * cout if mode in (PACK_UPFOLD, PACK_SG1_UP) else (cin if mode in (PACK_DGRAD, PACK_UPFOLD_DGRAD, PACK_SG1_UP_DGRAD, PACK_UPT2D_DGRAD) else cout)
    kdim = cout if mode == PACK_DGRAD else (4 * cout if mode in (PACK_UPFOLD_DGRAD, PACK_SG1_UP_DGRAD, PACK_UPT2D_DGRAD) else cin)
    return nvalid, kdim


def pack_mode_for(w, mode, H, W, dtype):
    nvalid, kdim = pack_dims(w, mode)
    in_s2d = (mode & 0xff) in (PACK_UPFOLD_DGRAD, PACK_SG1_UP_DGRAD)
    return mode | PACK_FRAG if small_conv(H, W, kdim, nvalid, w.shape[-1], in_s2d, False, dtype) else mode


def pack_conv_weight(w, mode=PACK_FWD, dtype=BF16, scale=1.0):
    (cout, cin), k = _pack_io(w, mode), w.shape[2]
    nvalid, kdim = pack_dims(w, mode)
    out = torch.empty((k * k, packed_n(nvalid), kdim), dtype=tdtype(dtype), device=w.device)
    check(lib().dge_pack_conv_weight(_f32(w.detach().contiguous()), _p(out), cout, cin, k, mode, dtype, float(scale),
                                     _stream()), "dge_pack_conv_weight")
    if mode & PACK_FRAG:
        out._dge_frag = True
    return out


def set_deterministic(on=True):
    check(lib().dge_set_deterministic(1 if on else 0), "dge_set_deterministic")


def is_deterministic():
    return bool(lib().dge_get_deterministic())


def pack_conv_weights_multi(entries, scratch=None):
    import struct
    n = len(entries)
    if n == 0:
        return scratch
    rows = []
    for (w, mode, dtype, scale, out) in entries:
        (cout, cin), k = _pack_io(w, mode), w.shape[2]
        if not (w.is_cuda and w.is_contiguous() and w.dtype == torch.float32):
            raise DgeError("pack_conv_weights_multi: weights must be contiguous f32 device tensors")
        rows += [w.data_ptr(), out.data_ptr(), cout | (cin << 32), k | (mode << 32), dtype,
                 struct.unpack("<I", struct.pack("<f", float(scale)))[0], 0, 0]
    tab = (C.c_longlong * (8 * n))(*rows)
    need = n * lib().dge_pack_desc_bytes()
    key = tuple(rows)
    if scratch is None or scratch[0].numel() < need:
        scratch = [torch.empty(max(need, 4096), dtype=torch.uint8, device=entries[0][0].device), None]
    upload = 0 if scratch[1] == key else 1
    check(lib().dge_pack_conv_weights_multi(tab, _p(scratch[0]), n, upload, _stream()), "dge_pack_conv_weights_multi")
    scratch[1] = key
    return scratch


def weight_sumsq(w, scale=1.0):
    cout, cin, k, _ = w.shape
    out = torch.empty((cout, cin), dtype=torch.float32, device=w.device)
    check(lib().dge_weight_sumsq(_f32(w.detach().contiguous()), _p(out), cout, cin, k, float(scale), _stream()),
          "dge_weight_sumsq")
    return out


def linear(x, w, bias=None, wscale=1.0, bscale=1.0, add=0.0, act=ACT_NONE, gain=1.0, square_input=False, out=None):
    B, I = x.shape
    O = w.shape[0]
    if x.stride(1) != 1:
        raise DgeError("linear: inner stride must be 1")
    if out is None:
        out = torch.empty((B, O), dtype=torch.float32, device=x.device)
    if not x.is_cuda:
        raise DgeError("tensor is not on the GPU: the HIP path has no CPU fallback")
    check(lib().dge_linear(C.c_void_p(x.data_ptr()), x.stride(0), _f32(w), _f32(bias), C.c_void_p(out.data_ptr()),
                           out.stride(0), B, I, O, float(wscale), float(bscale), float(add), act, float(gain),
                           1 if square_input else 0, _stream()), "dge_linear")
    _log_dense("dge_linear")
    return out


def _dense_layers(layers):
    from ._lib import DenseLayer
    arr = (DenseLayer * len(layers))()
    for e, L in zip(arr, layers):
        e.w, e.bias = _p(L.weight.detach()), _p(L.bias.detach())
        e.O, e.I = L.weight.shape
        e.wscale, e.bscale, e.add, e.act, e.gain = float(L.wscale), float(L.bscale), float(L.additional_bias), int(L.act), float(L.gain)
    return arr


def mapping_bwd(z, layers, g, coefs=None, acts=None, pixelnorm=True, eps=1e-8):
    B, L = g.shape[0], g.shape[1]
    if not z.is_cuda or z.stride(1) != 1:
        raise DgeError("mapping_bwd: z must be a CUDA tensor with unit inner stride")
    if z.shape[1] != layers[0].weight.shape[1] or z.shape[0] != B:
        raise DgeError(f"mapping_bwd: z {tuple(z.shape)} does not match B = {B}, first layer width {layers[0].weight.shape[1]}")
    g = g.float().contiguous()
    if g.shape[2] != layers[-1].weight.shape[0]:
        raise DgeError(f"mapping_bwd: gradient width {g.shape[2]} != last layer width {layers[-1].weight.shape[0]}")
    if coefs is not None and coefs.numel() != L:
        raise DgeError(f"mapping_bwd: {coefs.numel()} coefficients for {L} rows")
    arr = arr_p = None
    if acts is not None:
        if len(acts) != len(layers) or any(tuple(a.shape) != (B, Ly.weight.shape[0]) for a, Ly in zip(acts, layers)):
            raise DgeError("mapping_bwd: acts must hold one [B, O_l] output per layer")
        arr = (C.c_void_p * len(acts))(*[_f32(a).value for a in acts])
        arr_p = C.cast(arr, C.c_void_p)
    dz = torch.empty((B, z.shape[1]), dtype=torch.float32, device=z.device)
    check(lib().dge_mapping_bwd(_f32(z), z.stride(0), _dense_layers(layers), len(layers), arr_p, _p(g), L,
                                _f32(None if coefs is None else coefs.contiguous()), _p(dz), dz.stride(0), B, 1 if pixelnorm else 0,
                                float(eps), _stream()), "dge_mapping_bwd")
    return dz


def dense_chain(x, layers, pixelnorm=False, eps=1e-8):
    B = x.shape[0]
    arr = _dense_layers(layers)
    y = torch.empty((B, layers[-1].weight.shape[0]), dtype=torch.float32, device=x.device)
    if not x.is_cuda or x.stride(1) != 1:
        raise DgeError("dense_chain: x must be a CUDA tensor with unit inner stride")
    check(lib().dge_dense_chain(_f32(x), x.stride(0), arr, len(layers), _p(y), y.stride(0), B, 1 if pixelnorm else 0, float(eps), _stream()),
          "dge_dense_chain")
    return y


def pixelnorm(x, eps=1e-8):
    y = torch.empty_like(x)
    check(lib().dge_pixelnorm(_f32(x), _p(y), x.shape[0], x.shape[1], eps, _stream()), "dge_pixelnorm")
    return y


def truncation(w, w_avg, num_layers, psi, layers):
    w_is_wp = (w.ndim == 3)
    B, D = w.shape[0], w.shape[-1]
    wp = torch.empty((B, num_layers, D), dtype=torch.float32, device=w.device)
    check(lib().dge_truncation(_f32(w.contiguous()), _f32(w_avg), _p(wp), B, num_layers, D, float(psi), int(layers),
                               1 if w_is_wp else 0, _stream()), "dge_truncation")
    return wp


def log_kernel():
    if KERNEL_LOG is not None:
        KERNEL_LOG.append((last_kernel(), _stream()))


def _log_dense(name):
    if KERNEL_LOG is not None:
        KERNEL_LOG.append((name, _stream()))


def _launch(fn, args, name, macs, tag, tensors, wbytes=0, log=False):
    if PROFILE is None:
        check(fn(*args), name)
    else:
        e0, e1 = torch.cuda.Event(enable_timing=True), torch.cuda.Event(enable_timing=True)
        e0.record()
        check(fn(*args), name)
        e1.record()
        PROFILE.append((e0, e1, 2.0 * macs, tag, sum(t.numel() * t.element_size() for t in tensors if t is not None) + wbytes))
    if log and KERNEL_LOG is not None:
        log_kernel()


def _stats_slots(B, H, W, tile_w):
    return max(1, min(64, ((H + 15) // 16) * ((W + tile_w - 1) // tile_w) * B // 16))


def _mask_as_dot_src(name, relu_mask, dot_src, prep):
    if relu_mask is not None and (dot_src is not None or prep is not None):
        raise DgeError(f"{name}: relu_mask excludes dot_src / prep")
    return dot_src if relu_mask is None else relu_mask


def _set_prep(d, prep, nslot):
    pn = prep.get("noise")
    d.prep, d.prep_gain = 1, float(prep["gain"])
    d.prep_noise, d.prep_ns = _f32(pn), _f32(prep.get("ns") if pn is not None else None)
    d.prep_noise_batch = 1 if pn is None else pn.shape[0]
    d.prep_stats = _f32(prep["stats"].alloc(nslot))


def _weight_images(in_scale, out_scale):
    t = in_scale if out_scale is None else out_scale
    return 1 if t is None else t.shape[0]


class _PrefetchChain:

    def __init__(self, on=True):
        self.on, self.prev, self.next = on, {}, {}

    def link(self, stream, w_packed):
        if not self.on:
            return None
        key = w_packed.data_ptr()
        prev = self.prev.get(stream)
        if prev is not None and prev != key:
            if len(self.next) > 512:
                self.next.clear()
            self.next[(stream, prev)] = (key, w_packed.shape[1], w_packed.shape[2], _weakref.ref(w_packed))
        self.prev[stream] = key
        nxt = self.next.get((stream, key))
        if nxt is None:
            return None
        t = nxt[3]()
        if t is None or t.data_ptr() != nxt[0]:
            del self.next[(stream, key)]
            return None
        return nxt[:3]


_PREFETCH = _PrefetchChain(on=not _os.environ.get("DGE_NO_PREFETCH"))


def conv2d(x, w_packed, cout, ksize=3, up=False, in_scale=None, in_shift=None, out_scale=None, bias=None,
           bias_scale=1.0, noise=None, noise_w=None, act=ACT_NONE, gain=1.0, addend=None, add_scale=1.0, stats=None,
           out=None, in_s2d=False, dot_src=None, in_up2=False, in_relu=False, prep=None, relu_mask=None, in_t2d=False, rgb=None, pool_out=False, pool_mask=False,
           in_bwd=None):
    B, H, W, Cin = x.shape
    if in_s2d:
        H, W, Cin = H // 2, W // 2, Cin * 4
    if in_up2:
        H, W = 2 * H, 2 * W
    if in_t2d:
        H, W = H - 1, W - 1
    dt = dtype_of(x)
    OH, OW = (2 * H, 2 * W) if up else (H, W)
    mask = None
    if pool_out:
        if out is not None or up:
            raise DgeError("conv2d: pool_out allocates its own result and excludes up")
        out = torch.empty((B, OH // 2, OW // 2, cout), dtype=x.dtype, device=x.device)
        if pool_mask:
            mask = torch.empty((B, (OH // 2) * (OW // 2), cout // 8), dtype=torch.int32, device=x.device)
    if out is None:
        out = torch.empty((B, OH, OW, cout), dtype=x.dtype, device=x.device)
    d = ConvDesc()
    d.pool_out, d.pool_mask = 1 if pool_out else 0, _p(mask)
    dot_src = _mask_as_dot_src("conv2d", relu_mask, dot_src, prep)
    d.mask_relu = 0 if relu_mask is None else 1
    d.in_t2d = 1 if in_t2d else 0
    d.x, d.w_packed, d.y, d.addend, d.dot_src = _p(x), _p(w_packed), _p(out), _p(addend), _p(dot_src)
    d.in_scale, d.in_shift, d.out_scale = _f32(in_scale), _f32(in_shift), _f32(out_scale)
    partial, nslot = None, 1
    lazy = isinstance(stats, SlotStats)
    if stats is not None:
        nslot = _stats_slots(B, H, W, 16)
        if lazy:
            partial = stats.alloc(nslot)
        elif nslot > 1:
            partial = zeros((nslot,) + tuple(stats.shape), x.device)
    d.bias, d.noise, d.noise_w, d.stats = _f32(bias), _f32(noise), _f32(noise_w), _f32(partial if partial is not None else stats)
    d.stats_slots = nslot
    d.B, d.H, d.W, d.Cin, d.Cout = B, H, W, Cin, cout
    d.ksize, d.up, d.in_s2d, d.in_up2 = ksize, 1 if up else 0, 1 if in_s2d else 0, 1 if in_up2 else 0
    d.in_relu = 1 if in_relu else 0
    d.w_layout = 1 if getattr(w_packed, "_dge_frag", False) else 0
    if d.w_layout:
        nxt = _PREFETCH.link(_stream().value or 0, w_packed)
        if nxt is not None:
            d.prefetch_w, d.prefetch_ntot, d.prefetch_cin = C.c_void_p(nxt[0]), int(nxt[1]), int(nxt[2])
    if prep is not None:
        if stats is None or dot_src is None:
            raise DgeError("conv2d: prep needs stats and dot_src")
        _set_prep(d, prep, nslot)
    if in_bwd is not None:
        if dot_src is None or stats is not None or prep is not None:
            raise DgeError("conv2d: in_bwd needs dot_src and excludes stats / prep")
        d.stats_slots = _stats_slots(B, H, W, 16)
        pn = in_bwd.get("noise")
        d.in_bwd_coef = _f32(in_bwd["coef"])
        d.prep_noise, d.prep_noise_batch = _f32(pn), 1 if pn is None else pn.shape[0]
        if in_bwd.get("fr") is not None:
            d.fr_img4, d.in_bwd_extra, d.in_bwd_extra_scale = _f32(in_bwd["img4"]), _p(in_bwd.get("extra")), float(in_bwd.get("extra_scale", 1.0))
            in_bwd["fr"].buf = zeros((d.stats_slots, B, cout, 4), x.device)
            d.fr_out = _f32(in_bwd["fr"].buf)
        elif in_bwd.get("red") is not None:
            d.prep_stats = _f32(in_bwd["red"].alloc(d.stats_slots))
        else:
            d.prep_noise = None
            d.in_bwd_extra, d.in_bwd_extra_scale = _p(in_bwd.get("extra")), float(in_bwd.get("extra_scale", 1.0))
    if rgb is not None:
        d.rgb_w, d.rgb_style, d.rgb_bias, d.rgb_out = _f32(rgb["w"]), _f32(rgb["style"]), _f32(rgb["bias"]), _f32(rgb["out"])
        d.rgb_wscale, d.rgb_skip_y = float(rgb["wscale"]), 1 if rgb.get("skip_y") else 0
    d.noise_batch = 1 if noise is None else noise.shape[0]
    d.noise_w_per_channel = 0 if (noise_w is None or noise_w.numel() == 1) else 1
    d.act, d.bias_scale, d.gain, d.add_scale, d.dtype = act, bias_scale, gain, add_scale, dt
    if w_packed.dtype != x.dtype:
        raise DgeError("conv2d: packed weight dtype differs from activation dtype")
    taps_cin = 9.0 * Cin if up else 9.0 * (Cin // 4) if (in_s2d or in_t2d) else float(ksize * ksize) * Cin
    skip_y = rgb is not None and rgb.get("skip_y")
    _launch(lib().dge_conv2d, (C.byref(d), _stream()), "dge_conv2d", taps_cin * cout * H * W * B, (B, H, W, Cin, cout, ksize, up, in_s2d),
            (x, None if skip_y else out, addend, dot_src, w_packed, rgb["out"] if rgb is not None else None))
    if partial is not None and not lazy:
        check(lib().dge_sum_slots(_p(partial), _p(stats), nslot, stats.numel(), 1, _stream()), "dge_sum_slots")
    if skip_y:
        return None
    if pool_out and pool_mask:
        return out, mask
    return out


def conv_in_bwd_supported(B, H, W, cin, cout, dtype):
    return bool(lib().dge_conv_in_bwd_supported(int(B), int(H), int(W), int(cin), int(cout), 3, int(dtype)))


def conv_in_bwd_x_supported(B, H, W, cin, cout, dtype):
    return bool(lib().dge_conv_in_bwd_x_supported(int(B), int(H), int(W), int(cin), int(cout), 3, int(dtype)))
# ... 469 lines not shown
                                _f32(gb), B, O, I, 1 if accumulate else 0, _stream()), "dge_dense_wgrad")
    _log_dense("dge_dense_wgrad")
    return gw, gb


def _rows_view(t, what):
    if not t.is_cuda or t.dtype != torch.float32 or t.ndim != 3 or t.stride(2) != 1:
        raise DgeError(f"{what}: expected a float32 GPU tensor [B, rows, O] with unit inner stride")
    return C.c_void_p(t.data_ptr()), t.stride(0), t.stride(1), t.shape[1]


def heads_fwd(tab, n, musig_all, w):
    check(lib().dge_heads_fwd(_p(tab), n, _f32(musig_all), _p(w), w.stride(0), w.shape[0], w.shape[2], _stream()), "dge_heads_fwd")
    return w


def heads_bwd(tab, n, max_I, g, musig_all, gms_all, gw_all, gb_all):
    check(lib().dge_heads_bwd(_p(tab), n, int(max_I), _f32(g), g.stride(0), _f32(musig_all), _p(gms_all), _p(gw_all), _p(gb_all),
                              g.shape[0], g.shape[2], _stream()), "dge_heads_bwd")
    return gms_all


def heads_rows_fwd(tab, n, musig_all, w):
    wp, ldb, ldr, rows = _rows_view(w, "heads_rows_fwd")
    check(lib().dge_heads_rows_fwd(_p(tab), n, _f32(musig_all), wp, ldb, ldr, rows, w.shape[0], w.shape[2], _stream()), "dge_heads_rows_fwd")
    _log_dense("dge_heads_rows_fwd")
    return w


def heads_rows_bwd(tab, n, max_I, g, musig_all, gms_all, gw_all=None, gb_all=None):
    gp, ldb, ldr, rows = _rows_view(g, "heads_rows_bwd")
    check(lib().dge_heads_rows_bwd(_p(tab), n, int(max_I), gp, ldb, ldr, rows, _f32(musig_all), _f32(gms_all), _f32(gw_all), _f32(gb_all),
                                   g.shape[0], g.shape[2], _stream()), "dge_heads_rows_bwd")
    _log_dense("dge_heads_rows_bwd")
    return gms_all


def scale_(t, factor):
    check(lib().dge_axpy_scalar(_f32(t), None, _p(t), t.numel(), float(factor), 0, _stream()), "dge_axpy_scalar")
    return t


def blur_noise_act(x, noise, noise_w, bias, blur=True, stats=None, act=True):
    B, H, W, Cc = x.shape
    y = torch.empty_like(x)
    check(lib().dge_blur_noise_act(_p(x), _f32(noise), _f32(noise_w), _f32(bias), _p(y), _f32(stats), B, H, W, Cc,
                                   1 if blur else 0, 1 if noise is None else noise.shape[0], 1 if act else 0, dtype_of(x),
                                   _stream()), "dge_blur_noise_act")
    return y


def affine_compose(sc, sh, style):
    B, Cc = sc.shape
    a = torch.empty_like(sc)
    b = torch.empty_like(sc)
    check(lib().dge_affine_compose(_f32(sc), _f32(sh), _f32(style), _p(a), _p(b), B, Cc, _stream()), "dge_affine_compose")
    return a, b


def lerp_layers(w, avg, coefs):
    B, D = w.shape
    L = coefs.numel()
    out = torch.empty((B, L, D), dtype=torch.float32, device=w.device)
    stride = D if avg.numel() == L * D else 0
    check(lib().dge_lerp_layers(_f32(w), _f32(avg.contiguous()), stride, _f32(coefs.contiguous()), _p(out), B, L, D, _stream()),
          "dge_lerp_layers")
    return out


def pixelnorm_nhwc(x, eps=1e-8):
    B, H, W, Cc = x.shape
    y = torch.empty_like(x)
    check(lib().dge_pixelnorm_nhwc(_p(x), _p(y), B * H * W, Cc, float(eps), dtype_of(x), _stream()), "dge_pixelnorm_nhwc")
    return y


def cbn_affine(scale, offset, mean, var, eps):
    B, Cc = scale.shape
    a = torch.empty((B, Cc), dtype=torch.float32, device=scale.device)
    b = torch.empty_like(a)
    ld = scale.stride(0) if B > 1 else Cc
    if scale.dtype != torch.float32 or offset.dtype != torch.float32 or scale.stride(1) != 1 or offset.stride(1) != 1 or \
            (B > 1 and offset.stride(0) != ld):
        raise DgeError("cbn_affine: scale / offset must be float32 rows with unit inner stride and a common row stride")
    check(lib().dge_cbn_affine(C.c_void_p(scale.data_ptr()), C.c_void_p(offset.data_ptr()), ld, _f32(mean.contiguous()),
                               _f32(var.contiguous()), float(eps), _p(a), _p(b), B, Cc, _stream()), "dge_cbn_affine")
    return a, b


def slice_up(x, cout, up):
    B, H, W, Cin = x.shape
    f = 2 if up else 1
    y = torch.empty((B, H * f, W * f, cout), dtype=x.dtype, device=x.device)
    check(lib().dge_slice_up(_p(x), _p(y), B, H, W, Cin, cout, 1 if up else 0, dtype_of(x), _stream()), "dge_slice_up")
    return y


def attention(q, k, v):
    B, N, D = q.shape
    M, DV = k.shape[1], v.shape[2]
    o = torch.empty((B, N, DV), dtype=q.dtype, device=q.device)
    check(lib().dge_attention(_p(q), _p(k), _p(v), _p(o), B, N, M, D, DV, dtype_of(q), _stream()), "dge_attention")
    return o


def maxpool2(x):
    B, H, W, Cc = x.shape
    y = torch.empty((B, H // 2, W // 2, Cc), dtype=x.dtype, device=x.device)
    check(lib().dge_maxpool2(_p(x), _p(y), B, H, W, Cc, dtype_of(x), _stream()), "dge_maxpool2")
    return y


def rgb_tanh(x):
    B, H, W, Cc = x.shape
    img = torch.empty((B, 3, H, W), dtype=torch.float32, device=x.device)
    check(lib().dge_rgb_tanh(_p(x), _p(img), B, H * W, Cc, dtype_of(x), _stream()), "dge_rgb_tanh")
    return img


def sg1_in_bwd_coef(dots, sc, sh, style, npix):
    B, Cc = sc.shape
    coef = torch.empty((B, Cc, 3), dtype=torch.float32, device=sc.device)
    gstyle = torch.empty((B, 2 * Cc), dtype=torch.float32, device=sc.device)
    check(lib().dge_sg1_in_bwd_coef(_f32(dots), _f32(sc), _f32(sh), _f32(style), _p(coef), _p(gstyle), B, Cc, int(npix), _stream()),
          "dge_sg1_in_bwd_coef")
    return coef, gstyle


def dot_stats(g, x):
    B, H, W, Cc = x.shape
    st = zeros((B, Cc, 2), x.device)
    check(lib().dge_dot_stats(_p(g), _p(x), _p(st), B, H * W, Cc, dtype_of(x), _stream()), "dge_dot_stats")
    return st


def nearest_up2_bwd(ghi, x=None):
    B, H2, W2, Cc = ghi.shape
    glow = torch.empty((B, H2 // 2, W2 // 2, Cc), dtype=ghi.dtype, device=ghi.device)
    st = zeros((B, Cc, 2), ghi.device) if x is not None else None
    check(lib().dge_nearest_up2_bwd(_p(ghi), _p(x), _p(glow), _f32(st), B, H2 // 2, W2 // 2, Cc, dtype_of(ghi), _stream()),
          "dge_nearest_up2_bwd")
    return glow, st


def fromrgb_dgrad(gx, x0, w):
    B, H, W, Cc = x0.shape
    gimg = torch.empty((B, 3, H, W), dtype=torch.float32, device=x0.device)
    check(lib().dge_fromrgb_dgrad(_p(gx), _p(x0), _f32(w.reshape(Cc, 3).contiguous()), _p(gimg), B, H * W, Cc, dtype_of(x0), _stream()),
          "dge_fromrgb_dgrad")
    return gimg


def nearest_up2(x, scale=1.0):
    B, H, W, Cc = x.shape
    y = torch.empty((B, 2 * H, 2 * W, Cc), dtype=x.dtype, device=x.device)
    check(lib().dge_nearest_up2(_p(x), _p(y), B, H, W, Cc, float(scale), dtype_of(x), _stream()), "dge_nearest_up2")
    return y


def linear_rows(x, ldx_b, row_xoff, w, bias, y, row_ybase, row_ybstride, B, wscale, bscale, add):
    R, K = w.shape
    check(lib().dge_linear_rows(_f32(x), int(ldx_b), _p(row_xoff), _f32(w), _f32(bias), _p(y), _p(row_ybase), _p(row_ybstride), B, R, K,
                                float(wscale), float(bscale), float(add), _stream()), "dge_linear_rows")
    return y


def demod_rows(s_all, wsq_cat, row_woff, row_sbase, row_cin, d_all, row_dbase, row_dbstride, B, eps):
    R = row_woff.numel()
    check(lib().dge_demod_rows(_f32(s_all), _f32(wsq_cat), _p(row_woff), _p(row_sbase), _p(row_cin), _p(d_all), _p(row_dbase),
                               _p(row_dbstride), B, R, float(eps), _stream()), "dge_demod_rows")
    return d_all


def pixelnorm_nhwc_bwd(gy, x, eps=1e-8):
    Cc = x.shape[-1]
    gx = torch.empty_like(x)
    check(lib().dge_pixelnorm_nhwc_bwd(_p(gy), _p(x), _p(gx), x.numel() // Cc, Cc, float(eps), dtype_of(x), _stream()), "dge_pixelnorm_nhwc_bwd")
    return gx


def pixelnorm_act_bwd_supported(Cc, dtype):
    chunks, rem = divmod(int(Cc), 8 if dtype == BF16 else 4)
    return rem == 0 and chunks >= 1 and chunks & (chunks - 1) == 0 and chunks <= 128


def pixelnorm_act_bwd(g, x, up=False, act=True, eps=1e-8):
    B, H, W, Cc = x.shape
    if tuple(g.shape) != ((B, 2 * H, 2 * W, Cc) if up else (B, H, W, Cc)) or g.dtype != x.dtype:
        raise DgeError(f"pixelnorm_act_bwd: g {tuple(g.shape)} {g.dtype} does not go with x {tuple(x.shape)} {x.dtype} (up={bool(up)})")
    out = torch.empty_like(x)
    check(lib().dge_pixelnorm_act_bwd(_p(g), _p(x), _p(out), B, H, W, Cc, 1 if up else 0, 1 if act else 0, float(eps), dtype_of(x),
                                      _stream()), "dge_pixelnorm_act_bwd")
    log_kernel()
    return out


def affine_relu_bwd(gu, x, a, b):
    B, H, W, Cc = x.shape
    gx = torch.empty_like(x)
    st = zeros((B, Cc, 2), x.device)
    check(lib().dge_affine_relu_bwd(_p(gu), _p(x), _f32(a), _f32(b), _p(gx), _p(st), B, H * W, Cc, dtype_of(x), _stream()),
          "dge_affine_relu_bwd")
    return gx, st


def slice_up_bwd(gy, gx, up):
    B, H, W, Cin = gx.shape
    check(lib().dge_slice_up_bwd(_p(gy), _p(gx), B, H, W, Cin, gy.shape[3], 1 if up else 0, dtype_of(gx), _stream()), "dge_slice_up_bwd")
    return gx


def softmax_rows_(s):
    M = s.shape[-1]
    check(lib().dge_softmax_rows(_p(s), s.numel() // M, M, dtype_of(s), _stream()), "dge_softmax_rows")
    return s


def softmax_rows_bwd_(p, gp):
    M = p.shape[-1]
    check(lib().dge_softmax_rows_bwd(_p(p), _p(gp), p.numel() // M, M, dtype_of(p), _stream()), "dge_softmax_rows_bwd")
    return gp


def rgb_tanh_bwd(gimg, img, Cc, dtype):
    B, _, H, W = img.shape
    gy = torch.empty((B, H, W, Cc), dtype=tdtype(dtype), device=img.device)
    check(lib().dge_rgb_tanh_bwd(_f32(gimg.contiguous()), _f32(img), _p(gy), B, H * W, Cc, dtype, _stream()), "dge_rgb_tanh_bwd")
    return gy


def maxpool2_bwd(gy, x, addend=None, relu=False):
    B, H, W, Cc = x.shape
    gx = torch.empty_like(x)
    fn = lib().dge_maxpool2_bwd_relu if relu else lib().dge_maxpool2_bwd
    check(fn(_p(gy), _p(x), _p(addend), _p(gx), B, H, W, Cc, dtype_of(x), _stream()), "dge_maxpool2_bwd")
    return gx


def upconv_supported(cin, cout, dtype):
    return bool(lib().dge_upconv_supported(int(cin), int(cout), int(dtype)))


def pack_upconv_weight(w, dtype=BF16, scale=1.0):
    cout, cin = w.shape[0], w.shape[1]
    out = torch.empty((9, cout, cin), dtype=tdtype(dtype), device=w.device)
    check(lib().dge_pack_upconv_weight(_f32(w.detach().contiguous()), _p(out), cout, cin, float(scale), dtype, _stream()),
          "dge_pack_upconv_weight")
    return out


def upconv_fir(x, w_packed, cout, in_scale=None, out_scale=None, bias=None, bias_scale=1.0, noise=None, noise_w=None,
               act=ACT_NONE, gain=1.0):
    B, H, W, Cin = x.shape
    y = torch.empty((B, 2 * H, 2 * W, cout), dtype=x.dtype, device=x.device)
    nbs = 0 if (noise is None or noise.shape[0] == 1) else 4 * H * W
    nws = 0 if (noise_w is None or noise_w.numel() == 1) else 1
    _launch(lib().dge_upconv_fir, (_p(x), _p(w_packed), _p(y), _f32(in_scale), _f32(out_scale), _f32(noise), nbs, _f32(noise_w), nws,
                                   _f32(bias), float(bias_scale), float(gain), int(act), B, H, W, Cin, cout, dtype_of(x), _stream()),
            "dge_upconv_fir", 9.0 * Cin * cout * H * W * B, (B, H, W, Cin, cout, 3, "upfir", False), (x, y, w_packed))
    return y


def up_dgrad_stream_supported(B, Hin, Win, cin, cout, dtype):
    return (not is_deterministic()) and bool(lib().dge_up_dgrad_stream_supported(int(B), int(Hin), int(Win), int(cin), int(cout), int(dtype)))


def pack_up_dgrad_stream(w, dtype=BF16, scale=1.0):
    if dtype != BF16:
        raise DgeError("pack_up_dgrad_stream: bf16 only")
    cout, cin = w.shape[0], w.shape[1]
    return (w.detach().float() * float(scale)).flip(2, 3).permute(2, 3, 1, 0).reshape(9, cin, cout).to(torch.bfloat16).contiguous()


def up_dgrad_stream(g_z, w_packed, d_in, out_scale, addend, stats, dot_src, prep=None):
    B, FH, FW, cout = g_z.shape
    H, W = FH // 2, FW // 2
    _, cin, _ = w_packed.shape
    dt = dtype_of(g_z)
    if dot_src is None or stats is None:
        raise DgeError("up_dgrad_stream: needs stats and dot_src")
    if not up_dgrad_stream_supported(B, H, W, cin, cout, dt):
        raise DgeError(f"up_dgrad_stream: unsupported launch {cin} <- {cout} channels, dtype {dt}")
    out = torch.empty((B, H, W, cin), dtype=g_z.dtype, device=g_z.device)
    nslot = _stats_slots(B, H, W, 32)
    lazy = isinstance(stats, SlotStats)
    partial = stats.alloc(nslot) if lazy else (zeros((nslot,) + tuple(stats.shape), g_z.device) if nslot > 1 else stats)
    pn = pns = pst = None
    pgain, pbs = 1.0, 0
    if prep is not None:
        pn = prep.get("noise")
        pns = prep.get("ns") if pn is not None else None
        pbs = 0 if (pn is None or pn.shape[0] == 1) else H * W
        pgain, pst = float(prep["gain"]), prep["stats"].alloc(nslot)
    _launch(lib().dge_up_dgrad_stream,
            (_p(g_z), _p(w_packed), _p(out), _f32(d_in), _f32(out_scale), _p(addend), _p(dot_src), _f32(partial), nslot,
             0 if prep is None else 1, pgain, _f32(pn), pbs, _f32(pns), _f32(pst), B, H, W, cin, cout, dt, _stream()),
            "dge_up_dgrad_stream", 9.0 * cin * cout * H * W * B, (B, H, W, 4 * cout, cin, 3, False, True),
            (g_z, out, addend, dot_src, w_packed))
    if not lazy and partial is not stats:
        check(lib().dge_sum_slots(_p(partial), _p(stats), nslot, stats.numel(), 1, _stream()), "dge_sum_slots")
    return out


TRACK_ARM_AT, TRACK_ARM_AFTER = 0, 1


def latent_pnorm(w, p=2, out=None, out_l2=None):
    if out is None:
        out = torch.empty((), dtype=torch.float32, device=w.device)
    check(lib().dge_latent_pnorm_fwd(_f32(w.contiguous()), _p(out), _f32(out_l2), w.numel(), int(p), _stream()), "dge_latent_pnorm_fwd")
    return out


def latent_l2(w, out=None):
    if out is None:
        out = torch.empty((), dtype=torch.float32, device=w.device)
    check(lib().dge_latent_pnorm_fwd(_f32(w.contiguous()), None, _p(out), w.numel(), 2, _stream()), "dge_latent_pnorm_fwd")
    return out


def latent_pnorm_bwd(w, norm, g, p=2, beta=1.0, gout=None):
    check(lib().dge_latent_pnorm_bwd(_f32(w.contiguous()), _f32(norm), _f32(gout), _f32(g), w.numel(), int(p), float(beta), _stream()),
          "dge_latent_pnorm_bwd")
    return g


def wplus_lerp(w, avg, psi, out=None):
    B, L, D = w.shape
    if out is None:
        out = torch.empty((B, L, D), dtype=torch.float32, device=w.device)
    stride = D if avg.numel() == L * D else 0
    check(lib().dge_wplus_lerp(_f32(w.contiguous()), _f32(avg.contiguous()), stride, float(psi), _p(out), B, L, D, _stream()),
          "dge_wplus_lerp")
    return out


def wplus_lerp_bwd(g, psi, out=None, accumulate=False):
    g = g.float().contiguous()
    if out is None:
        out = torch.empty_like(g)
    check(lib().dge_wplus_lerp_bwd(_p(g), float(psi), _f32(out), g.numel(), 1 if accumulate else 0, _stream()), "dge_wplus_lerp_bwd")
    return out


def embed_track(loss, norm, w, istate, fstate, best_loss_w, best_norm_w, events, arm_rule, arm_iter, loss_hyst, norm_hyst):
    if istate.dtype != torch.int32:
        raise DgeError("embed_track: istate must be int32")
    cap = events.shape[0]
    check(lib().dge_embed_track(_f32(loss), _f32(norm), _f32(w.contiguous()), w.numel(), _p(istate), _f32(fstate), _f32(best_loss_w),
                                _f32(best_norm_w), _f32(events), int(cap), int(arm_rule), int(arm_iter), float(loss_hyst),
                                float(norm_hyst), _stream()), "dge_embed_track")


def latent_pnorm_rows(w, p=2, out=None, out_l2=None):
    B = w.shape[0]
    if out is None:
        out = torch.empty(B, dtype=torch.float32, device=w.device)
    check(lib().dge_latent_pnorm_rows_fwd(_f32(w.contiguous()), _p(out), _f32(out_l2), B, w.numel() // B, int(p), _stream()),
          "dge_latent_pnorm_rows_fwd")
    log_kernel()
    return out


def latent_l2_rows(w, out=None):
    B = w.shape[0]
    if out is None:
        out = torch.empty(B, dtype=torch.float32, device=w.device)
    check(lib().dge_latent_pnorm_rows_fwd(_f32(w.contiguous()), None, _p(out), B, w.numel() // B, 2, _stream()), "dge_latent_pnorm_rows_fwd")
    log_kernel()
    return out


def latent_pnorm_rows_bwd(w, norm, g, p=2, beta=1.0, gout=None):
    B = w.shape[0]
    check(lib().dge_latent_pnorm_rows_bwd(_f32(w.contiguous()), _f32(norm), _f32(gout), _f32(g), B, w.numel() // B, int(p), float(beta),
                                          _stream()), "dge_latent_pnorm_rows_bwd")
    log_kernel()
    return g


def embed_track_rows(loss, norm, w, istate, fstate, best_loss_w, best_norm_w, events, arm_rule, arm_iter, loss_hyst, norm_hyst):
    if istate.dtype != torch.int32:
        raise DgeError("embed_track_rows: istate must be int32")
    B = w.shape[0]
    if tuple(istate.shape) != (B, 4) or tuple(fstate.shape) != (B, 2) or events.shape[0] != B or loss.numel() != B or norm.numel() != B:
        raise DgeError("embed_track_rows: state shapes do not match the batch")
    for t in (loss, norm, istate, fstate, best_loss_w, best_norm_w, events):
        if not t.is_contiguous():
            raise DgeError("embed_track_rows: arguments must be contiguous")
    check(lib().dge_embed_track_rows(_f32(loss), _f32(norm), _f32(w.contiguous()), B, w.numel() // B, _p(istate), _f32(fstate),
                                     _f32(best_loss_w), _f32(best_norm_w), _f32(events), int(events.shape[1]), int(arm_rule),
                                     int(arm_iter), float(loss_hyst), float(norm_hyst), _stream()), "dge_embed_track_rows")
    log_kernel()



def quantize_u8(x, out=None):
    if x.dim() != 4:
        raise DgeError("quantize_u8: expected [B,C,H,W]")
    B, Cc, H, W = x.shape
    if out is None:
        out = torch.empty((B, H, W, Cc), dtype=torch.uint8, device=x.device)
    elif out.dtype != torch.uint8 or tuple(out.shape) != (B, H, W, Cc):
        raise DgeError("quantize_u8: out must be uint8 [B,H,W,C]")
    check(lib().dge_quantize_u8(_p(x), dtype_of(x), _p(out), B, Cc, H, W, _stream()), "dge_quantize_u8")
    log_kernel()
    return out


def image_metrics_u8_work_bytes(B, H, W):
    n = lib().dge_image_metrics_u8_work_bytes(int(B), int(H), int(W))
    if n < 0:
        check(n, "dge_image_metrics_u8_work_bytes")
    return n


def image_metrics_u8(a, b, work=None, isums=None, ssim=None, out=None):
    for t in (a, b):
        if t.dtype != torch.uint8:
            raise DgeError(f"image_metrics_u8: expected uint8 images, got {t.dtype}")
    if a.dim() != 4 or a.shape[3] != 3 or a.shape != b.shape:
        raise DgeError(f"image_metrics_u8: expected two [B,H,W,3] images of one shape, got {tuple(a.shape)} and {tuple(b.shape)}")
    B, H, W, _ = a.shape
    nbytes = image_metrics_u8_work_bytes(B, H, W)
    dev = a.device
    if work is None:
        work = torch.empty(nbytes // 8, dtype=torch.int64, device=dev)
    elif work.numel() * work.element_size() < nbytes:
        raise DgeError(f"image_metrics_u8: work holds {work.numel() * work.element_size()} bytes, {nbytes} needed")
    isums = torch.empty((B, 5), dtype=torch.int64, device=dev) if isums is None else isums
    ssim = torch.empty(B, dtype=torch.float64, device=dev) if ssim is None else ssim
    out = torch.empty((B, 4), dtype=torch.float64, device=dev) if out is None else out
    if isums.dtype != torch.int64 or ssim.dtype != torch.float64 or out.dtype != torch.float64 \
            or isums.numel() != 5 * B or ssim.numel() != B or out.numel() != 4 * B:
        raise DgeError("image_metrics_u8: isums int64 [B,5], ssim float64 [B], out float64 [B,4]")
    check(lib().dge_image_metrics_u8(_p(a), _p(b), B, H, W, _p(work), _p(isums), _p(ssim), _p(out), _stream()), "dge_image_metrics_u8")
    log_kernel()
    return isums, ssim, out
```

deep-gan-encoders_amd/s2_conv.py:

```python
import os

from . import ops
from .weight_cache import lookup, store

PP_GEN = not os.environ.get("DGE_NO_PP_GEN")
UP_PP = os.environ.get("DGE_UP_PP", "1") != "0"
UP_FOLDED = os.environ.get("DGE_UP_FOLDED") == "1"
T2D = not os.environ.get("DGE_NO_T2D")
PP_DG = not os.environ.get("DGE_NO_PP_DG")
UP_DG_STREAM = not os.environ.get("DGE_NO_UP_DG_STREAM")


def prepared(L, dtype):
    c = lookup(L._cache, ("w", dtype), L.weight)
    if c is None:
        mode = ops.PACK_UPFOLD if L.up else ops.PACK_FWD
        hin = L.res // 2 if L.up else L.res
        packed = ops.pack_conv_weight(L.weight, ops.pack_mode_for(L.weight, mode, hin, hin, dtype), dtype, L.wscale) \
            if L.ksize == 3 else None
        wsq = ops.weight_sumsq(L.weight, L.wscale) if L.demodulate else None
        c = store(L._cache, ("w", dtype), L.weight, (packed, wsq))
    return c


def _prepared_up(L, dtype):
    if not L.up or L.res < 32 or UP_FOLDED or not ops.upconv_supported(L.in_c, L.out_c, dtype):
        return None
    c = lookup(L._cache, ("wu", dtype), L.weight)
    return c if c is not None else store(L._cache, ("wu", dtype), L.weight, ops.pack_upconv_weight(L.weight, dtype, L.wscale))


def forward(L, x, s, d, noise, dt, rgb=None):
    nw = L.noise_strength.detach().reshape(1) if noise is not None else None
    B, H, W, _ = x.shape
    wu = _prepared_up(L, dt)
    if wu is not None:
        assert rgb is None
        if (UP_PP and s is not None and d is not None and (noise is None or nw.numel() == 1)
                and ops.up_pp_supported(B, H, W, L.in_c, L.out_c, dt)):
            wimg = ops.pack_up_pp(wu, L.out_c, L.in_c, in_scale=s, out_scale=d, gain=L.gain)
            return ops.up_pp(x, wimg, L.out_c, bias=L.bias, bias_scale=L.bscale, noise=noise, noise_w=nw, act=L.act, gain=L.gain)
        return ops.upconv_fir(x, wu, L.out_c, in_scale=s, out_scale=d, bias=L.bias, bias_scale=L.bscale, noise=noise, noise_w=nw, act=L.act, gain=L.gain)
    if (rgb is None and not L.up and d is not None and s is not None and L.ksize == 3 and PP_GEN
            and ops.conv_pp_supported(B, H, W, L.in_c, L.out_c, dt)):
        wpp = ops.pack_conv_pp(L.weight, L.wscale, in_scale=s, out_scale=d, gain=L.gain)
        return ops.conv_pp(x, wpp, L.out_c, bias=L.bias, bias_scale=L.bscale, noise=noise, noise_w=nw, act=L.act, gain=L.gain)
    packed, _ = prepared(L, dt)
    return ops.conv2d(x, packed, L.out_c, 3, up=L.up, in_scale=s, out_scale=d, bias=L.bias, bias_scale=L.bscale, noise=noise, noise_w=nw, act=L.act, gain=L.gain, rgb=rgb)


def _up_phase_form(L):
    return L.up and 32 <= L.res // 2 <= 128 and L.in_c >= 64 and L.in_c % 32 == 0 and L.out_c % 8 == 0 and T2D


def _dgrad_weight(L, dtype):
    hg = L.res // 2 if L.up else L.res
    if _up_phase_form(L):
        mode = ops.PACK_UPT2D_DGRAD
    else:
        mode = ops.pack_mode_for(L.weight, ops.PACK_UPFOLD_DGRAD if L.up else ops.PACK_DGRAD, hg, hg, dtype)
    c = lookup(L._cache, ("dg", dtype, mode), L.weight)
    return c if c is not None else store(L._cache, ("dg", dtype, mode), L.weight, ops.pack_conv_weight(L.weight, mode, dtype, L.wscale))


def _pp_dgrad(L, B, hg, dtype):
    K = 4 * L.out_c if L.up else L.out_c
    return PP_DG and (not L.up or L.out_c % 32 == 0) and ops.conv_pp_supported(B, hg, hg, K, L.in_c, dtype)


def _dgrad_weight_pp(L, d, t2d=False):
    if not L.up:
        return ops.pack_conv_pp(L.weight, L.wscale, in_scale=d, dgrad=True)
    name = "dgpp_t2d" if t2d else "dgpp"
    c = lookup(L._cache, name, L.weight)
    if c is None:
        rows = ops.pack_conv_weight(L.weight, ops.PACK_UPT2D_DGRAD if t2d else ops.PACK_UPFOLD_DGRAD, ops.F32, L.wscale)
        c = store(L._cache, name, L.weight, ops.pack_conv_pp_rows(rows, L.in_c, t2d=True) if t2d else rows)
    return c if t2d else ops.pack_conv_pp_rows(c, L.in_c, in_scale=d, in_period=L.out_c)


def _up_stream_dgrad(L, B, dtype, fused):
    return UP_DG_STREAM and fused and L.up and L.ksize == 3 and ops.up_dgrad_stream_supported(B, L.res // 2, L.res // 2, L.in_c, L.out_c, dtype)


def _dgrad_weight_stream(L, dtype):
    c = lookup(L._cache, ("dgs", dtype), L.weight)
    return c if c is not None else store(L._cache, ("dgs", dtype), L.weight, ops.pack_up_dgrad_stream(L.weight, dtype, L.wscale))


def dgrad_takes_prep(L, B=None, dtype=None):
    if B is not None and L.up and _up_stream_dgrad(L, B, dtype, not ops.is_deterministic()):
        return True
    return _up_phase_form(L) or not (L.up and L.in_c < 128)


def dgrad(L, g_y, d_in, dt, fused, prep=None, **epilogue):
    B, hg = g_y.shape[0], (L.res // 2 if L.up else L.res)
    if L.up and _up_stream_dgrad(L, B, dt, fused) and epilogue.get("dot_src") is not None and epilogue.get("stats") is not None \
            and set(epilogue) <= {"out_scale", "addend", "stats", "dot_src"}:
        return ops.up_dgrad_stream(g_y, _dgrad_weight_stream(L, dt), d_in, epilogue.get("out_scale"), epilogue.get("addend"),
                                   epilogue.get("stats"), epilogue["dot_src"], prep=prep)
    t2d = _up_phase_form(L)
    if fused and d_in is not None and not t2d and _pp_dgrad(L, B, hg, dt):
        return ops.conv_pp(g_y, _dgrad_weight_pp(L, d_in), L.in_c, dgrad=True, in_s2d=L.up, add_scale=1.0, prep=prep, **epilogue)
    if t2d and fused and prep is not None and _pp_dgrad(L, B, hg, dt):
        return ops.conv_pp(ops.fir_t2d(g_y, d_in), _dgrad_weight_pp(L, None, t2d=True), L.in_c, dgrad=True, in_t2d=True, add_scale=1.0, prep=prep, **epilogue)
    if t2d:
        return ops.conv2d(ops.fir_t2d(g_y, d_in), _dgrad_weight(L, dt), L.in_c, 3, in_t2d=True, add_scale=1.0, prep=prep, **epilogue)
    return ops.conv2d(g_y, _dgrad_weight(L, dt), L.in_c, 3, in_s2d=L.up, in_scale=d_in, add_scale=1.0, prep=prep, **epilogue)
```

include/dge_hip.h:

```cpp
#ifndef DGE_HIP_H
#define DGE_HIP_H
#include <stddef.h>
#ifdef __cplusplus
extern "C" {
#endif

typedef struct ihipStream_t* dge_stream_t;

#define DGE_DTYPE_F32 0
#define DGE_DTYPE_BF16 1
#define DGE_ACT_LINEAR 0
#define DGE_ACT_LRELU02 1
#define DGE_ACT_RELU_ 2
#define DGE_LIN_RSQRT 3
#define DGE_PACK_FWD 0
#define DGE_PACK_UPFOLD 1
#define DGE_PACK_DGRAD 2
#define DGE_PACK_UPFOLD_DGRAD 3
#define DGE_PACK_SG1_UP 4
#define DGE_PACK_SG1_UP_DGRAD 5
#define DGE_PACK_UPT2D_DGRAD 6

const char* dge_last_error(void);
int dge_version(void);

typedef struct dge_conv_desc {
    const void* x;
    const void* w_packed;
    void* y;
    const void* addend;
    const void* dot_src;
    const float* in_scale;
    const float* in_shift;
    const float* out_scale;
    const float* bias;
    const float* noise;
    const float* noise_w;
    float* stats;
    int B, H, W, Cin, Cout;
    int ksize;
    int up;
    int in_s2d;
    int noise_batch;
    int noise_w_per_channel;
    int act;
    float bias_scale, gain, add_scale;
    int dtype;
    int in_up2;
    int in_relu;
    int stats_slots;
    int w_layout;
    int prep;
    float prep_gain;
    const float* prep_noise;
    const float* prep_ns;
    int prep_noise_batch;
    float* prep_stats;
    int mask_relu;
    int in_t2d;
    const float* rgb_w;
    const float* rgb_style;
    const float* rgb_bias;
    float* rgb_out;
    float rgb_wscale;
    int rgb_skip_y;
    int pool_out;
    void* pool_mask;
    const void* prefetch_w;
    int prefetch_ntot, prefetch_cin;
    const float* in_bwd_coef;
    const void* in_bwd_extra;
    float in_bwd_extra_scale;
    const float* fr_img4;
    float* fr_out;
} dge_conv_desc;
int dge_conv2d(const dge_conv_desc* d, dge_stream_t stream);
int dge_conv_small_supported(int H, int W, int cin, int ntot, int ksize, int in_s2d, int in_up2, int dtype);
#define DGE_PACK_FRAG 0x100
const char* dge_last_kernel(void);
void dge_env_reload(void);
int dge_sum_slots(const float* partial, float* out, int nslot, int n, int accumulate, dge_stream_t stream);
int dge_sum_slots_planar(const float* partial, float* out, int nslot, int C, int NS, dge_stream_t stream);
typedef struct dge_sum_planar_entry { const float* partial; float* out; int nslot, C, NS, pad; } dge_sum_planar_entry;
int dge_sum_slots_planar_multi(const dge_sum_planar_entry* entries, int n, dge_stream_t stream);

int dge_linear_rows(const float* x, int ldx_b, const int* row_xoff, const float* w, const float* bias, float* y,
                    const int* row_ybase, const int* row_ybstride, int B, int R, int K, float wscale, float bscale, float add,
                    dge_stream_t stream);
int dge_demod_rows(const float* s_all, const float* wsq_cat, const int* row_woff, const int* row_sbase, const int* row_cin,
                   float* d_all, const int* row_dbase, const int* row_dbstride, int B, int R, float eps, dge_stream_t stream);
int dge_set_deterministic(int on);
int dge_get_deterministic(void);
int dge_packed_n(int n_valid);
int dge_pack_conv_weight(const float* w_oihw, void* out, int cout, int cin, int ksize, int mode, int dtype,
                         float scale, dge_stream_t stream);
int dge_pack_conv_weights_multi(const long long* table_host, void* descs_dev, int n, int upload, dge_stream_t stream);
int dge_pack_desc_bytes(void);
int dge_weight_sumsq(const float* w_oihw, float* wsq, int cout, int cin, int ksize, float scale, dge_stream_t stream);

int dge_linear(const float* x, int ldx, const float* w, const float* bias, float* y, int ldy, int B, int I, int O,
               float wscale, float bscale, float add, int act, float gain, int square_input, dge_stream_t stream);
int dge_pixelnorm(const float* x, float* y, int B, int D, float eps, dge_stream_t stream);
typedef struct dge_dense_layer { const float* w; const float* bias; int I, O; float wscale, bscale, add; int act; float gain; } dge_dense_layer;
int dge_dense_chain(const float* x, int ldx, const dge_dense_layer* layers, int n, float* y, int ldy, int B, int pixelnorm, float eps,
                    dge_stream_t stream);
int dge_truncation(const float* w, const float* w_avg, float* wp, int B, int L, int D, float psi, int layers,
                   int w_is_wp, dge_stream_t stream);

int dge_torgb(const void* x, const float* wrgb, const float* style, const float* bias, const float* prev, float* img,
              int B, int H, int W, int cin, float wscale, int dtype, dge_stream_t stream);

int dge_conv_rgb_supported(int B, int H, int W, int Cin, int Cout, int ksize, int dtype);
int dge_conv_in_bwd_supported(int B, int H, int W, int Cin, int Cout, int ksize, int dtype);
int dge_conv_in_bwd_fromrgb_supported(int B, int H, int W, int Cin, int Cout, int ksize, int dtype);
int dge_conv_in_bwd_x_supported(int B, int H, int W, int Cin, int Cout, int ksize, int dtype);
int dge_conv_pool_supported(int B, int H, int W, int Cin, int Cout, int ksize, int dtype);
int dge_rgb_upsample_add(float* img, const float* prev, int BC, int H, int W, dge_stream_t stream);
int dge_nchw_to_nhwc(const float* src, void* dst, int B, int C, int HW, int src_B, int dtype, dge_stream_t stream);
int dge_nhwc_to_nchw(const void* src, float* dst, int B, int C, int HW, int dtype, dge_stream_t stream);

int dge_fromrgb(const float* img, const float* w, const float* bias, void* y, float* stats, int B, int HW, int C,
                int dtype, dge_stream_t stream);
int dge_fromrgb2(const float* img, const float* w, const float* bias, void* y, float* stats, float* img4, int B, int HW, int C,
                 int dtype, dge_stream_t stream);
int dge_stats_finalize(const float* stats, float* musig, float* sc, float* sh, int B, int C, int npix, float eps,
                       dge_stream_t stream);
int dge_stats_finalize_slots(const float* stats, int nslot, float* musig, float* sc, float* sh, int B, int C, int npix, float eps,
                             dge_stream_t stream);
int dge_blend(const void* x, const void* z, void* y, const float* sc, const float* sh, float* stats, int B, int OH,
              int OW, int C, int pool, float alpha, float beta, int dtype, dge_stream_t stream);

int dge_loss_reduce(const float* a, const float* b, float* sums7, int B, int C, int H, int W, int y0, int x0, int h, int w,
                    dge_stream_t stream);
int dge_ssim_fwd(const float* a, const float* b, float* ssim_sum, float* dmap, int BC, int h, int w, dge_stream_t stream);
int dge_ssim_box7(const float* a, const float* b, float* sums, int BC, int h, int w, float scale, float shift, float data_range,
                  dge_stream_t stream);
int dge_ssim_bwd(const float* a, const float* b, const float* dmap, float* g, int BC, int h, int w, float scale,
                 int accumulate, dge_stream_t stream);
int dge_space_loss_finalize(const float* sums7, const float* ssim_sum, const float* lpips, float* out8, float n,
                            float n_pooled, int image_space, dge_stream_t stream);
int dge_space_loss_bwd(const float* a, const float* b, const float* sums7, const float* g_pooled, float* g, int BC, int H,
                       int W, int y0, int x0, int h, int w, int k, float n, float weight, int accumulate, dge_stream_t stream);
int dge_loss_reduce3(const float* a, const float* b, float* sums, int B, int C, int H, int W, const int* wins, int nwin, dge_stream_t stream);
int dge_crop_pool_multi(const float* const* src, float* const* dst, const int* wins, const int* ks, int n, int BC, int H, int W,
                        dge_stream_t stream);
int dge_space_loss_bwd3(const float* a, const float* b, const float* const* sums7, const float* const* g_pooled, float* g, int BC, int H,
                        int W, const int* wins, const int* ks, const float* n, const float* weight, int nwin, dge_stream_t stream);
int dge_space_loss_bwd_split(const float* a, const float* b, const float* const* sums7, const float* const* g_pooled, float* const* g,
                             int BC, int H, int W, const int* wins, const int* ks, const float* n, const float* weight, int nwin,
                             dge_stream_t stream);
int dge_loss_reduce_rows(const float* a, const float* b, float* partials, int B, int C, int H, int W, const int* wins, int nwin, int nblk,
                         dge_stream_t stream);
int dge_ssim_fwd_rows(const float* a, const float* b, float* tile_sums, float* dmap, int BC, int h, int w, dge_stream_t stream);
int dge_space_loss_finalize_rows(const float* partials, int nblk, const float* const* ssim_tiles, const int* ssim_cnt,
                                 const float* const* lpips_val, float* sums7, float* out8, int B, int nwin, const float* n,
                                 const float* n_pooled, int image_space, dge_stream_t stream);
int dge_space_loss_bwd_rows(const float* a, const float* b, const float* sums7, const float* const* g_pooled, float* g, int B, int C,
                            int H, int W, const int* wins, const int* ks, const float* n, const float* weight, int nwin, int swap_ab,
                            dge_stream_t stream);
int dge_axpy_scalar(const float* x, const float* scalar, float* y, long n, float extra, int accumulate, dge_stream_t stream);

int dge_lreq_adam_multi(int ntensors, float* const* host_p, const float* const* host_g, float* const* host_v,
                        const long* host_n, const float* host_step, float beta2, float eps, const float* gscale,
                        const float* step_mult, dge_stream_t stream);

int dge_modconv_bwd_prep(const void* gx, const void* x, const float* d, const float* noise, void* gy, float* R, int B,
                         int HW, int C, int noise_batch, float gain, int dtype, dge_stream_t stream);
int dge_demod_bwd(const float* R, const float* d, const float* bias, const float* noise_strength, float* t, int B, int C,
                  float bscale, dge_stream_t stream);
int dge_linear_t(const float* x, int ldx, int incx, const float* w, const float* mul, float* y, int ldy, int incy, int B,
                 int O, int K, float scale, int accumulate, dge_stream_t stream);
int dge_torgb_bwd(const float* gimg, const void* x, const float* wrgb, const float* style, void* gx, float* gs, int B,
                  int HW, int C, float wscale, int dtype, dge_stream_t stream);
int dge_torgb_bwd_prep(const float* gimg, const void* x, const float* wrgb, const float* style, const float* noise,
                       const float* noise_strength, int noise_batch, void* gz, float* gs, float* P, int B, int HW, int C,
                       float wscale, float gain, int dtype, dge_stream_t stream);
int dge_fir_t2d(const void* g, const float* scale, void* z, int B, int H, int W, int C, int dtype, dge_stream_t stream);
typedef struct dge_s2_grad_entry {
    const float* P; const float* st; const float* d; const float* s; const float* bias; const float* wsq;
    const float* gs; const float* wstyle;
    int nslot_p, nslot_s, in_c, out_c, row;
    float bscale;
} dge_s2_grad_entry;
int dge_s2_style_grads(const dge_s2_grad_entry* entries, int n, float* g_wp, int B, int nrows, int K, float wscale, dge_stream_t stream);
int dge_demod_bwd_prep(const float* P, int nslot, const float* d, const float* bias, float* t, int B, int C, float bscale,
                       dge_stream_t stream);
int dge_up2_bwd(const float* g, float* gprev, int BC, int h, int w, dge_stream_t stream);

int dge_conv_wgrad(const void* g, const void* x, const float* in_scale, const float* in_shift, float* dw, int B, int H, int W,
                   int cout, int cin, int ksize, int dtype, dge_stream_t stream);
int dge_conv_wgrad_dots(const void* g, const void* x, const float* in_scale, const float* in_shift, float* dw, const float* w,
                        float* dots, int dots_slots, int B, int H, int W, int cout, int cin, int dtype, dge_stream_t stream);
int dge_act_bwd(const void* gup, const void* a, const float* noise, void* gpre, float* red, int red_cols, int B, int H, int W, int C,
                int pool, float scale, float slope, int dtype, dge_stream_t stream);
int dge_blend_pool_mask(const void* x, const void* z, void* y, float* stats, unsigned* mask, int B, int OH, int OW, int C, float alpha,
                        float beta, int dtype, dge_stream_t stream);
int dge_act_bwd_mask(const void* gup, const unsigned* mask, const float* noise, void* gpre, float* red, int red_cols, int B, int H, int W,
                     int C, float scale, float slope, int dtype, dge_stream_t stream);
int dge_fromrgb_dgrad(const void* gx, const void* x0, const float* w, float* gimg, int B, int HW, int C, int dtype, dge_stream_t stream);
int dge_nearest_up2(const void* x, void* y, int B, int H, int W, int C, float scale, int dtype, dge_stream_t stream);
int dge_in_bwd_coef(const float* dots, const float* gms, const float* musig, const float* sc, const float* sh, float* coef,
                    int B, int C, int npix, dge_stream_t stream);
int dge_in_bwd_coef_slots(const float* dots, int nslot, const float* gms, const float* musig, const float* sc, const float* sh,
                          float* coef, int B, int C, int npix, dge_stream_t stream);
int dge_in_bwd(const void* gy, const void* x, const float* coef, const void* extra, const float* noise, void* gout, float* red,
               int B, int H, int W, int C, int extra_pool, float extra_scale, int act, int dtype, dge_stream_t stream);
int dge_in_bwd_fused(const void* gy, const void* x, const float* dots, int nslot, const float* gms, const float* musig,
                     const float* sc, const float* sh, int npix, const void* extra, const float* noise, void* gout, float* red,
                     int B, int H, int W, int C, int extra_pool, float extra_scale, int act, int dtype, dge_stream_t stream);
int dge_chan_sum(const void* x, float* out, int B, int HW, int C, float scale, int dtype, dge_stream_t stream);
int dge_fromrgb_bwd(const void* gx, const void* x0, const float* img, float* out4, int B, int HW, int C, int dtype,
                    dge_stream_t stream);
int dge_in_bwd_fromrgb(const void* gy, const void* x0, const float* dots, int nslot, const float* gms, const float* musig,
                       const float* sc, const float* sh, int npix, const void* extra, const float* img, float* out4,
                       int B, int H, int W, int C, int extra_pool, float extra_scale, int dtype, dge_stream_t stream);
int dge_in_bwd_fromrgb_img(const void* gy, const void* x0, const float* dots, int nslot, const float* gms, const float* musig,
                           const float* sc, const float* sh, int npix, const void* extra, const float* w, const float* img, float* out4,
                           float* gimg, int B, int H, int W, int C, int extra_pool, float extra_scale, int dtype, dge_stream_t stream);
int dge_affine_bwd_fromrgb_img(const void* gy, const void* x0, const float* a, const void* extra, const float* w, const float* img, float* out4,
                               float* gimg, int B, int H, int W, int C, int extra_pool, float extra_scale, int dtype, dge_stream_t stream);
int dge_heads_fwd(const void* dev_entries, int n, const float* musig_all, float* w, int ldw, int B, int O, dge_stream_t stream);
int dge_head_entry_size(void);
int dge_heads_bwd(const void* dev_entries, int n, int max_I, const float* g, int ldg, const float* musig_all, float* gms_all,
                  float* gw_all, float* gb_all, int B, int O, dge_stream_t stream);
int dge_head_rows_entry_size(void);
int dge_heads_rows_fwd(const void* dev_entries, int n, const float* musig_all, float* w, long ldb, long ldr, int nrows, int B, int O,
                       dge_stream_t stream);
int dge_heads_rows_bwd(const void* dev_entries, int n, int max_I, const float* g, long ldb, long ldr, int nrows,
                       const float* musig_all, float* gms_all, float* gw_all, float* gb_all, int B, int O, dge_stream_t stream);
int dge_dense_wgrad(const float* gy, int ldgy, const float* x, int ldx, float* gw, float* gb, int B, int O, int I,
                    int accumulate, dge_stream_t stream);

int dge_lpips_prep(const float* img, void* x, int B, int HW, int cpad, const float* host_shift3, const float* host_scale3,
                   int dtype, dge_stream_t stream);
int dge_lpips_prep_bwd(const void* gx, float* gimg, int B, int HW, int cpad, const float* host_scale3, float factor,
                       int accumulate, int dtype, dge_stream_t stream);
int dge_maxpool2(const void* x, void* y, int B, int H, int W, int C, int dtype, dge_stream_t stream);
int dge_maxpool2_bwd(const void* gy, const void* x, const void* addend, void* gx, int B, int H, int W, int C, int dtype,
                     dge_stream_t stream);
int dge_lpips_head(const void* feat, const float* lin, float* val, void* g1, int B, int HW, int C, float gscale, int dtype,
                   dge_stream_t stream);
int dge_mean(const float* v, float* out, int n, dge_stream_t stream);

int dge_blur_noise_act(const void* x, const float* noise, const float* noise_w, const float* bias, void* y, float* stats,
                       int B, int H, int W, int C, int do_blur, int noise_batch, int act, int dtype, dge_stream_t stream);
int dge_affine_compose(const float* sc, const float* sh, const float* style, float* a, float* b, int B, int C, dge_stream_t stream);
int dge_lerp_layers(const float* w, const float* avg, int avg_stride, const float* coefs, float* out, int B, int L, int D,
                    dge_stream_t stream);

int dge_sg1_in_bwd_coef(const float* dots, const float* sc, const float* sh, const float* style, float* coef, float* gstyle,
                        int B, int C, int npix, dge_stream_t stream);
int dge_dot_stats(const void* g, const void* x, float* stats, int B, int HW, int C, int dtype, dge_stream_t stream);
int dge_nearest_up2_bwd(const void* ghi, const void* x, void* glow, float* stats, int B, int H, int W, int C, int dtype,
                        dge_stream_t stream);

int dge_sn_group(const void* entries, int n, int maxO, int maxK, float* sigma, float eps, int training, dge_stream_t stream);
int dge_sn_entry_size(void);
int dge_cbn_sn_wgrad_entry_size(void);
int dge_cbn_sn_wgrad_group(const void* entries, int n, long long rows, int maxC, const float* cond, int B, int K, float* rowdot, dge_stream_t stream);

int dge_randn(float* out, int nseg, const long long* start, const long long* count, const unsigned long long* goff,
              const unsigned int* subseq, unsigned long long seed, const unsigned long long* seed_dev, dge_stream_t stream);

int dge_upconv_supported(int Cin, int Cout, int dtype);
int dge_pack_upconv_weight(const float* w, void* out, int Cout, int Cin, float scale, int dtype, dge_stream_t stream);
int dge_upconv_fir(const void* x, const void* w_packed, void* y, const float* in_scale, const float* out_scale,
                   const float* noise, int noise_bstride, const float* noise_w, int noise_w_stride, const float* bias,
                   float bias_scale, float gain, int act, int B, int H, int W, int Cin, int Cout, int dtype, dge_stream_t stream);

int dge_up_dgrad_stream_supported(int B, int H, int W, int Cin, int Cout, int dtype);
int dge_up_dgrad_stream(const void* g_z, const void* w_packed, void* y, const float* d_in, const float* out_scale,
                        const void* addend, const void* dot_src, float* stats, int stats_slots, int prep, float prep_gain,
                        const float* prep_noise, int prep_noise_bstride, const float* prep_ns, float* prep_stats,
                        int B, int H, int W, int Cin, int Cout, int dtype, dge_stream_t stream);

int dge_up_pp_supported(int B, int H, int W, int Cin, int Cout, int dtype);
int dge_pack_up_pp(const void* w_units, void* out, int Cout, int Cin, const float* in_scale, const float* out_scale, float gain,
                   int nb, dge_stream_t stream);
int dge_up_pp(const void* x, const void* w_img, long long w_bstride, void* y, const float* noise, int noise_bstride,
              const float* noise_w, const float* bias, float bias_scale, float gain, int act, int B, int H, int W, int Cin, int Cout,
              dge_stream_t stream);

typedef struct dge_conv_pp_desc {
    const void* x;
    const void* w_pp;
    void* y;
    long long w_bstride;
    const float* out_scale;
    const float* bias;
    const float* noise;
    const float* noise_w;
    int B, H, W, Cin, Cout;
    int noise_batch;
    int noise_w_per_channel;
    int act;
    float bias_scale, gain;
    int dgrad, in_s2d, stats_slots, prep, prep_noise_batch, mask_relu;
    int in_t2d;
    float add_scale, prep_gain;
    const void* dot_src;
    const void* addend;
    float* stats;
    float* prep_stats;
    const float* prep_noise;
    const float* prep_ns;
} dge_conv_pp_desc;
int dge_conv_pp_supported(int B, int H, int W, int Cin, int Cout, int dtype);
int dge_pack_conv_pp(const float* w_oihw, void* out, int N, int K, float wscale, const float* in_scale, const float* out_scale,
                     float gain, int nb, int mode, dge_stream_t stream);
int dge_pack_conv_pp_rows(const float* w_rows, int src_rows, void* out, int N, int K, const float* in_scale, int in_period,
                          const float* out_scale, float gain, int nb, int t2d, dge_stream_t stream);
int dge_conv_pp(const dge_conv_pp_desc* d, dge_stream_t stream);

int dge_pixelnorm_nhwc(const void* x, void* y, long npix, int C, float eps, int dtype, dge_stream_t stream);
int dge_pixelnorm_nhwc_bwd(const void* gy, const void* x, void* gx, long npix, int C, float eps, int dtype, dge_stream_t stream);
int dge_pixelnorm_act_bwd(const void* g, const void* x, void* out, int B, int H, int W, int C, int up, int act, float eps, int dtype,
                          dge_stream_t stream);

int dge_cbn_affine(const float* scale, const float* offset, int ld, const float* mean, const float* var, float eps, float* a,
                   float* b, int B, int C, dge_stream_t stream);
int dge_slice_up(const void* x, void* y, int B, int H, int W, int Cin, int Cout, int up, int dtype, dge_stream_t stream);
int dge_attention(const void* q, const void* k, const void* v, void* o, int B, int N, int M, int D, int DV, int dtype,
                  dge_stream_t stream);
int dge_rgb_tanh(const void* x, float* img, int B, int HW, int C, int dtype, dge_stream_t stream);
int dge_affine_relu_bwd(const void* gu, const void* x, const float* a, const float* b, void* gx, float* stats, int B, int HW, int C,
                        int dtype, dge_stream_t stream);
int dge_slice_up_bwd(const void* gy, void* gx, int B, int H, int W, int Cin, int Cout, int up, int dtype, dge_stream_t stream);
int dge_softmax_rows(void* S, long R, int M, int dtype, dge_stream_t stream);
int dge_softmax_rows_bwd(const void* P, void* gP, long R, int M, int dtype, dge_stream_t stream);
int dge_rgb_tanh_bwd(const float* gimg, const float* img, void* gy, int B, int HW, int C, int dtype, dge_stream_t stream);

int dge_guided_relu_bwd(const void* g, const void* a, void* gpre, long n, int guided, int dtype, dge_stream_t stream);
int dge_maxpool2_bwd_relu(const void* gy, const void* x, const void* addend, void* gx, int B, int H, int W, int C, int dtype,
                          dge_stream_t stream);
int dge_maxpool2_relu_bwd(const void* gy, const void* x, void* gx, int B, int H, int W, int C, int guided, int dtype,
                          dge_stream_t stream);
int dge_adaptive_pool7(const void* x, float* y, int B, int H, int W, int C, int dtype, dge_stream_t stream);
int dge_adaptive_pool7_bwd(const float* gy, void* gx, int B, int H, int W, int C, int dtype, dge_stream_t stream);
int dge_class_target(const float* logits, const int* index_in, int* index_out, float* glogits, int B, int K, dge_stream_t stream);
int dge_gather_row(const float* w, const int* index, float* y, int B, int I, float scale, dge_stream_t stream);
int dge_class_target_rows(const float* logits, const int* index_in, int* index_out, float* glogits, int B, int K, dge_stream_t stream);
int dge_gather_rows(const float* w, const int* index, float* y, int B, int I, dge_stream_t stream);
int dge_campp_map(const void* grad, const void* feat, float* wgt, float* cam, float* minmax, int B, int HW, int C, int mode,
                  int dtype, dge_stream_t stream);
int dge_cam_resize(const float* cam, const float* minmax, float* mask, int B, int h, int w, int H, int W, dge_stream_t stream);
int dge_mask2cam_blocks(int HW);
int dge_mask2cam(const float* mask, const float* img, const int* lut, float* heat, float* cam, float* part, float* coef, int B,
                 int HW, dge_stream_t stream);

int dge_mask2cam_rows(const float* mask, const float* img, const int* lut, float* heat, float* cam, float* part, int B, int HW,
                      dge_stream_t stream);

int dge_class_target_groups(const float* logits, const int* index_in, int* index_out, float* glogits, int G, int N, int K,
                            dge_stream_t stream);
int dge_gather_row_groups(const float* w, const int* index, float* y, int G, int N, int I, float scale, dge_stream_t stream);
int dge_mask2cam_groups(const float* mask, const float* img, const int* lut, float* heat, float* cam, float* part, float* coef, int G,
                        int N, int HW, dge_stream_t stream);

int dge_latent_pnorm_fwd(const float* w, float* out, float* out_l2, long n, int p, dge_stream_t stream);
int dge_latent_pnorm_bwd(const float* w, const float* norm, const float* gout, float* g, long n, int p, float beta,
                         dge_stream_t stream);
int dge_wplus_lerp(const float* w, const float* avg, int avg_stride, float psi, float* out, int B, int L, int D, dge_stream_t stream);
int dge_wplus_lerp_bwd(const float* g, float psi, float* gw, long n, int accumulate, dge_stream_t stream);
#define DGE_TRACK_ARM_AT 0
#define DGE_TRACK_ARM_AFTER 1
int dge_embed_track(const float* loss, const float* norm, const float* w, long n, int* istate, float* fstate, float* best_loss_w,
                    float* best_norm_w, float* events, int cap, int arm_rule, int arm_iter, float loss_hyst, float norm_hyst,
                    dge_stream_t stream);
int dge_latent_pnorm_rows_fwd(const float* w, float* out, float* out_l2, int B, long n, int p, dge_stream_t stream);
int dge_latent_pnorm_rows_bwd(const float* w, const float* norm, const float* gout, float* g, int B, long n, int p, float beta,
                              dge_stream_t stream);
int dge_embed_track_rows(const float* loss, const float* norm, const float* w, int B, long n, int* istate, float* fstate,
                         float* best_loss_w, float* best_norm_w, float* events, int cap, int arm_rule, int arm_iter, float loss_hyst,
                         float norm_hyst, dge_stream_t stream);

int dge_mapping_bwd(const float* z, int ldz, const dge_dense_layer* layers, int n, const float* const* acts, const float* g, int L,
                    const float* coefs, float* dz, int lddz, int B, int pixelnorm, float eps, dge_stream_t stream);

int dge_quantize_u8(const void* x, int dtype, unsigned char* out, int B, int C, int H, int W, dge_stream_t stream);
int dge_image_metrics_u8_work_bytes(int B, int H, int W);
int dge_image_metrics_u8(const unsigned char* a, const unsigned char* b, int B, int H, int W, void* work, long long* isums,
                         double* ssim, double* out, dge_stream_t stream);

int dge_minmax_unit_slots(long n);
int dge_minmax_unit(const float* x, float* y, long n, float* slots, dge_stream_t stream);

#ifdef __cplusplus
}
#endif
#endif
```

Before: 383.0 images/sec.

## Add phase-unit dgrad kernel for small upsampling convs in transposed-2D form

Adds a specialised small-resolution kernel for the data gradient of upsampling 3x3 convs. It reads the four-phase t2d input plane by plane and does only the 9 nonzero weight units (new pack mode 7) instead of a full 3x3 conv over 4*Cout channels. It also loads the next phase plane while the current one is multiplied. It is used by default for layers of at most 32x32 outside deterministic mode, and adds a new kernel, pack mode and dispatch path.

```diff
diff --git a/deep-gan-encoders_amd/_lib.py b/deep-gan-encoders_amd/_lib.py
--- a/deep-gan-encoders_amd/_lib.py
+++ b/deep-gan-encoders_amd/_lib.py
@@ -58,6 +58,8 @@
 SIGNATURES = {
     "dge_conv2d": [C.POINTER(ConvDesc), _P],
     "dge_fir_t2d": [_P, _P, _P, _I, _I, _I, _I, _I, _P],
+    "dge_up_dgrad_small": [C.POINTER(ConvDesc), _P],
+    "dge_up_dgrad_small_supported": [_I, _I, _I, _I, _I, _I],
     "dge_s2_style_grads": [C.POINTER(S2GradEntry), _I, _P, _I, _I, _I, _F, _P],
     "dge_conv_small_supported": [_I, _I, _I, _I, _I, _I, _I, _I],
     "dge_torgb_bwd_prep": [_P, _P, _P, _P, _P, _P, _I, _P, _P, _P, _I, _I, _I, _F, _F, _I, _P],
diff --git a/deep-gan-encoders_amd/csrc/capi.hip b/deep-gan-encoders_amd/csrc/capi.hip
--- a/deep-gan-encoders_amd/csrc/capi.hip
+++ b/deep-gan-encoders_amd/csrc/capi.hip
@@ -70,7 +70,7 @@
 const DgeEnv& dge_env() { std::call_once(g_env_once, [] { if (!g_env_loaded) env_load(); }); return g_env; }
 extern "C" void dge_env_reload(void) { env_load(); }
 
-extern "C" int dge_conv2d(const dge_conv_desc* d, hipStream_t s) {
+static int conv_desc_to_params(const dge_conv_desc* d, ConvParams& p, bool units) {
     DGE_CHECK(d && d->x && d->w_packed && d->y, "conv2d: null tensor");
     DGE_CHECK(d->B > 0 && d->H > 0 && d->W > 0 && d->Cin > 0 && d->Cout > 0, "conv2d: bad shape");
     DGE_CHECK(d->dtype == DGE_F32 || d->dtype == DGE_BF16, "conv2d: bad dtype %d", d->dtype);
@@ -84,7 +84,6 @@
     DGE_CHECK(d->gain > 0.f, "conv2d: gain must be positive (it is folded through the activation)");
     DGE_CHECK((((uintptr_t)d->in_scale | (uintptr_t)d->in_shift) & 15) == 0, "conv2d: in_scale/in_shift must be 16-byte aligned");
     DGE_CHECK(!d->noise || d->noise_w, "conv2d: noise without noise_w");
-    ConvParams p;
     p.x = d->x; p.w = d->w_packed; p.y = d->y; p.addend = d->addend; p.dot_src = d->dot_src;
     p.in_scale = d->in_scale; p.in_shift = d->in_shift; p.out_scale = d->out_scale;
     p.bias = d->bias; p.noise = d->noise; p.noise_w = d->noise_w; p.stats = d->stats;
@@ -101,7 +100,7 @@
     p.prep = d->prep ? 1 : 0;
     p.mask_relu = d->mask_relu ? 1 : 0;
     p.in_t2d = d->in_t2d ? 1 : 0;
-    DGE_CHECK(!d->in_t2d || (d->ksize == 3 && !d->up && !d->in_s2d && !d->in_up2 && !d->in_scale && !d->in_shift && d->w_layout == 0),
+    DGE_CHECK(!d->in_t2d || (d->ksize == 3 && !d->up && !d->in_s2d && !d->in_up2 && !d->in_scale && !d->in_shift && (d->w_layout == 0 || units)),
               "conv2d: in_t2d is a plain 3x3 launch (no other read mode, no prologue affine, row-major weights)");
     p.prep_gain = d->prep_gain; p.prep_noise = d->prep_noise; p.prep_ns = d->prep_ns; p.prep_stats = d->prep_stats;
     p.prep_noise_bstride = d->prep_noise_batch > 1 ? OH * OW : 0;
@@ -131,7 +130,25 @@
         DGE_CHECK(dge_conv_rgb_ok(p, d->dtype, d->ksize), "conv2d: the fused toRGB is offered where dge_conv_rgb_supported() says so "
                   "(bf16 3x3 32 -> 32 launches of the streaming kernel)");
     }
+    return 0;
+}
+
+extern "C" int dge_conv2d(const dge_conv_desc* d, hipStream_t s) {
+    ConvParams p;
+    if (const int rc = conv_desc_to_params(d, p, false)) return rc;
     return dge_conv_launch(p, d->dtype, d->ksize, s);
+}
+
+extern "C" int dge_up_dgrad_small(const dge_conv_desc* d, hipStream_t s) {
+    DGE_CHECK(d && d->in_t2d && d->w_layout == 1 && d->ksize == 3 && d->Cin % 4 == 0, "up_dgrad_small: an in_t2d launch with fragment-ordered unit weights");
+    DGE_CHECK(!d->bias && !d->noise && d->act == DGE_ACT_NONE && !d->mask_relu && !d->in_bwd_coef && !d->rgb_out && !d->pool_out && !d->in_relu,
+              "up_dgrad_small: data-gradient epilogue only (out_scale, addend, dot_src + stats, prep)");
+    DGE_CHECK(dge_up_dgrad_small_supported(d->B, d->H, d->W, d->Cin / 4, d->Cout, d->dtype),
+              "up_dgrad_small: unsupported launch %dx%d, %d <- %d channels, dtype %d", d->H, d->W, d->Cout, d->Cin / 4, d->dtype);
+    ConvParams p;
+    if (const int rc = conv_desc_to_params(d, p, true)) return rc;
+    p.Cin = d->Cin / 4;
+    return dge_up_dgrad_small_launch(p, s);
 }
 
 extern "C" int dge_conv_pool_supported(int B, int H, int W, int Cin, int Cout, int ksize, int dtype) {
diff --git a/deep-gan-encoders_amd/csrc/conv_params.h b/deep-gan-encoders_amd/csrc/conv_params.h
--- a/deep-gan-encoders_amd/csrc/conv_params.h
+++ b/deep-gan-encoders_amd/csrc/conv_params.h
@@ -60,5 +60,7 @@
 bool dge_conv_pool_ok(const ConvParams& p, int dtype, int ksize);
 bool dge_conv_small_shape_ok(int H, int W, int cin, int ntot, int ksize, int in_s2d, int in_up2, int dtype);
 int dge_conv_small_launch(const ConvParams& p, hipStream_t s);
+extern "C" int dge_up_dgrad_small_supported(int B, int H, int W, int C, int N, int dtype);
+int dge_up_dgrad_small_launch(const ConvParams& p, hipStream_t s);
 bool dge_conv_pw_eligible(const ConvParams& p, int dtype, int ksize);
 int dge_conv_pw_launch(const ConvParams& p, hipStream_t s);
diff --git a/deep-gan-encoders_amd/csrc/conv_small.hip b/deep-gan-encoders_amd/csrc/conv_small.hip
--- a/deep-gan-encoders_amd/csrc/conv_small.hip
+++ b/deep-gan-encoders_amd/csrc/conv_small.hip
@@ -27,6 +27,22 @@
     return __builtin_amdgcn_mfma_f32_32x32x16_bf16(*(const bf16x8_t*)&a, *(const bf16x8_t*)&b, c, 0, 0, 0);
 }
 
+__device__ __forceinline__ void prefetch_next_weights(const ConvParams& p, const unsigned char* lds, int wave, int lane, int tid) {
+    const int xcd = blockIdx.x & 7, r = blockIdx.x >> 3, R = max(1, (int)gridDim.x >> 3);
+    const int nt_n = p.pf_ntot / BN, kst_n = p.pf_cin / 16;
+    const int n_lo = xcd * nt_n / 8, n_hi = max(n_lo + 1, (xcd + 1) * nt_n / 8);
+    const unsigned lines_tap = (unsigned)(n_hi - n_lo) * 2u * kst_n * 8u;
+    const unsigned nlines = 9u * lines_tap;
+    const size_t tap_stride_n = (size_t)(p.pf_ntot / 32) * kst_n * 1024;
+    const unsigned m0v = lds_base_u32(lds) + A_MAX + N_BYTES + wave * 256;
+    for (unsigned l = (unsigned)r * 512u + tid; l - lane < nlines; l += (unsigned)R * 512u) {
+        const unsigned tp = l / lines_tap, within = l - tp * lines_tap;
+        const unsigned char* a = (const unsigned char*)p.pf_w + tp * tap_stride_n + (size_t)n_lo * 2 * kst_n * 1024 + (size_t)within * 128;
+        if (l >= nlines) a = (const unsigned char*)p.pf_w;
+        asm volatile("s_mov_b32 m0, %1\n\ts_nop 0\n\tglobal_load_lds_dword %0, off" : : "v"(a), "s"(m0v) : "memory");
+    }
+}
+
 template <int KQ, int MODE>
 __global__ __launch_bounds__(512, 2) void conv_small_kernel(ConvParams p) {
     constexpr int CIN = KQ * 64, CH = CIN / 8;
@@ -58,21 +74,7 @@
 #pragma unroll
         for (int j = 0; j < KQ; j++) bw[t][j] = *(const uint4*)(wbase + t * tap_stride + j * 1024);
 
-    auto prefetch_next = [&]() {
-        const int xcd = blockIdx.x & 7, r = blockIdx.x >> 3, R = max(1, (int)gridDim.x >> 3);
-        const int nt_n = p.pf_ntot / BN, kst_n = p.pf_cin / 16;
-        const int n_lo = xcd * nt_n / 8, n_hi = max(n_lo + 1, (xcd + 1) * nt_n / 8);
-        const unsigned lines_tap = (unsigned)(n_hi - n_lo) * 2u * kst_n * 8u;
-        const unsigned nlines = 9u * lines_tap;
-        const size_t tap_stride_n = (size_t)(p.pf_ntot / 32) * kst_n * 1024;
-        const unsigned m0v = lds_base_u32(lds) + A_MAX + N_BYTES + wave * 256;
-        for (unsigned l = (unsigned)r * 512u + tid; l - lane < nlines; l += (unsigned)R * 512u) {
-            const unsigned tp = l / lines_tap, within = l - tp * lines_tap;
-            const unsigned char* a = (const unsigned char*)p.pf_w + tp * tap_stride_n + (size_t)n_lo * 2 * kst_n * 1024 + (size_t)within * 128;
-            if (l >= nlines) a = (const unsigned char*)p.pf_w;
-            asm volatile("s_mov_b32 m0, %1\n\ts_nop 0\n\tglobal_load_lds_dword %0, off" : : "v"(a), "s"(m0v) : "memory");
-        }
-    };
+    auto prefetch_next = [&]() { prefetch_next_weights(p, lds, wave, lane, tid); };
     const bool pf_late = gridDim.x <= 256;
     if (p.pf_w && !pf_late) prefetch_next();
 
@@ -186,6 +188,147 @@
     conv_epilogue<bf16_t, SmallCfg, TH, TW, BN, 2, 2, 512, MODE>(p, tile, lds + RED_BYTES, ldsN, b, x0, y0, bn0, ntile, vbid, tx_i, ty_i,
                                                             wave, lane, tid, carrier);
     if (p.pf_w) asm volatile("s_waitcnt vmcnt(0)" ::: "memory");
+}
+
+constexpr int TU_PH[9] = {0, 0, 0, 0, 1, 1, 2, 2, 3}, TU_AY[9] = {0, 0, 1, 1, 0, 1, 0, 0, 0}, TU_AX[9] = {0, 1, 0, 1, 0, 0, 0, 1, 0};
+constexpr int TP_U0[5] = {0, 4, 6, 8, 9};
+constexpr int ZH = TH + 1, ZW = TW + 1;
+
+template <int KQ, int MODE>
+__global__ __launch_bounds__(512, 2) void conv_small_t2d_kernel(ConvParams p) {
+    constexpr int CIN = KQ * 64, CH = CIN / 8;
+    constexpr int PSTR = pstr_of(CIN), RPITCH = rpitch_of(CIN);
+    constexpr int KST = CIN / 16;
+    __shared__ __attribute__((aligned(256))) unsigned char lds[LDS_BYTES];
+    float* ldsN = (float*)(lds + A_MAX);
+    const int tid = threadIdx.x, lane = tid & 63;
+    const int wave = __builtin_amdgcn_readfirstlane(tid >> 6);
+    int bid = blockIdx.x;
+    {
+        const int nb = gridDim.x, per = nb >> 3;
+        if (per > 0 && bid < (per << 3)) bid = (bid & 7) * per + (bid >> 3);
+    }
+    const int vbid = bid;
+    const int tx_i = bid % p.tiles_x; bid /= p.tiles_x;
+    const int ty_i = bid % p.tiles_y; bid /= p.tiles_y;
+    const int b = bid % p.B;
+    const int ntile = bid / p.B;
+    const int x0 = tx_i * TW, y0 = ty_i * TH, bn0 = ntile * BN;
+    const int nt = wave & 1, kq = wave >> 1;
+
+    const unsigned char* wbase = (const unsigned char*)p.w + ((size_t)(bn0 / 32 + nt) * KST + kq * KQ) * 1024 + lane * 16;
+    const size_t unit_stride = (size_t)(p.Ntot / 32) * KST * 1024;
+    constexpr int PF = KQ >= 8 ? 3 : 4;
+    uint4 bw[PF + 1][KQ];
+#pragma unroll
+    for (int t = 0; t < PF; t++)
+#pragma unroll
+        for (int j = 0; j < KQ; j++) bw[t][j] = *(const uint4*)(wbase + t * unit_stride + j * 1024);
+
+    const bool pf_late = gridDim.x <= 256;
+    if (p.pf_w && !pf_late) prefetch_next_weights(p, lds, wave, lane, tid);
+
+    constexpr int NPER = (ZH * ZW - 1) * CH / 512;
+    static_assert(NPER * 512 == (ZH * ZW - 1) * CH, "80 pixels are whole rounds of 512 threads");
+    const int chunk = tid % CH;
+    const bf16_t* __restrict__ Zb = (const bf16_t*)p.x + (size_t)b * (p.H + 1) * (p.W + 1) * 4 * CIN + chunk * 8;
+    uint4 v[NPER];
+    auto plane_load = [&](int ph) {
+#pragma unroll
+        for (int i = 0; i < NPER; i++) {
+            const int pix = tid / CH + i * (512 / CH), hx = pix % ZW, hy = pix / ZW;
+            const int gy = min(y0 + hy, p.H), gx = min(x0 + hx, p.W);
+            v[i] = *(const uint4*)(Zb + ((size_t)(gy * (p.W + 1) + gx) * 4 + ph) * CIN);
+        }
+    };
+    auto plane_store = [&]() {
+#pragma unroll
+        for (int i = 0; i < NPER; i++) {
+            const int pix = tid / CH + i * (512 / CH), hx = pix % ZW, hy = pix / ZW;
+            const bool inside = (y0 + hy <= p.H) & (x0 + hx <= p.W);
+            *(uint4*)(lds + hy * RPITCH + hx * PSTR + chunk * 16) = inside ? v[i] : make_uint4(0, 0, 0, 0);
+        }
+    };
+    if (tid < CH) {
+        uint4 c = make_uint4(0, 0, 0, 0);
+        if (y0 + TH <= p.H && x0 + TW <= p.W) c = *(const uint4*)(Zb + (size_t)((y0 + TH) * (p.W + 1) + x0 + TW) * 4 * CIN);
+        *(uint4*)(lds + TH * RPITCH + TW * PSTR + chunk * 16) = c;
+    }
+    plane_load(0);
+    if (p.prep && p.prep_noise) {
+        for (int idx = tid; idx < SmallCfg::BM; idx += 512) {
+            const int gy = y0 + idx / TW, gx = x0 + idx % TW;
+            ldsN[idx] = (gy < p.H && gx < p.W) ? p.prep_noise[(size_t)b * p.prep_noise_bstride + (size_t)gy * p.W + gx] : 0.f;
+        }
+    }
+    plane_store();
+    __syncthreads();
+
+    f32x16_t acc[2];
+#pragma unroll
+    for (int g = 0; g < 2; g++)
+#pragma unroll
+        for (int r = 0; r < 16; r++) acc[g][r] = 0.f;
+    int aoff[2];
+#pragma unroll
+    for (int g = 0; g < 2; g++) {
+        const int m = g * 32 + (lane & 31);
+        aoff[g] = (m / TW) * RPITCH + (m % TW) * PSTR + kq * KQ * 32 + (lane >> 5) * 16;
+    }
+    StaticFor<4>::run([&](auto pc) {
+        constexpr int ph = decltype(pc)::value;
+        if (ph < 3) plane_load(ph + 1);
+        StaticFor<TP_U0[ph + 1] - TP_U0[ph]>::run([&](auto uc) {
+            constexpr int u = TP_U0[ph] + decltype(uc)::value;
+            if (u + PF < 9) {
+                const unsigned char* wn = wbase + (size_t)(u + PF) * unit_stride;
+#pragma unroll
+                for (int j = 0; j < KQ; j++) bw[(u + PF) % (PF + 1)][j] = *(const uint4*)(wn + j * 1024);
+            }
+            const unsigned char* at = lds + TU_AY[u] * RPITCH + TU_AX[u] * PSTR;
+#pragma unroll
+            for (int j = 0; j < KQ; j++) {
+                const uint4 a0 = *(const uint4*)(at + aoff[0] + j * 32);
+                const uint4 a1 = *(const uint4*)(at + aoff[1] + j * 32);
+                acc[0] = mma(a0, bw[u % (PF + 1)][j], acc[0]);
+                acc[1] = mma(a1, bw[u % (PF + 1)][j], acc[1]);
+            }
+        });
+        if (ph < 3) {
+            __syncthreads();
+            plane_store();
+            __syncthreads();
+        }
+    });
+
+    if (p.pf_w && pf_late) prefetch_next_weights(p, lds, wave, lane, tid);
+    __syncthreads();
+    float* red = (float*)lds;
+#pragma unroll
+    for (int g = 0; g < 2; g++)
+#pragma unroll
+        for (int r = 0; r < 16; r++) red[((wave * 2 + g) * 16 + r) * 64 + lane] = acc[g][r];
+    __syncthreads();
+    const bool carrier = wave < 4;
+    f32x16_t tile[1][1];
+    if (carrier) {
+        const int wm = wave >> 1, wn = wave & 1;
+#pragma unroll
+        for (int r = 0; r < 16; r++) {
+            float s = 0.f;
+#pragma unroll
+            for (int q = 0; q < 4; q++) s += red[(((q * 2 + wn) * 2 + wm) * 16 + r) * 64 + lane];
+            tile[0][0][r] = s;
+        }
+    }
+    conv_epilogue<bf16_t, SmallCfg, TH, TW, BN, 2, 2, 512, MODE>(p, tile, lds + RED_BYTES, ldsN, b, x0, y0, bn0, ntile, vbid, tx_i, ty_i,
+                                                            wave, lane, tid, carrier);
+    if (p.pf_w) asm volatile("s_waitcnt vmcnt(0)" ::: "memory");
+}
+
+int up_dgrad_small_maxhw() {
+    static const int v = [] { const char* e = getenv("DGE_UP_DG_SMALL_MAXHW"); const int n = e ? atoi(e) : 32; return n < 0 ? 0 : n; }();
+    return v;
 }
 
 int max_hw() {
@@ -223,3 +366,30 @@
     DGE_LAUNCH_CHECK("conv_small");
     return 0;
 }
+
+extern "C" int dge_up_dgrad_small_supported(int B, int H, int W, int C, int N, int dtype) {
+    return (dtype == DGE_BF16 && B > 0 && H > 0 && W > 0 && (C == 512 || C == 256) && N >= BN && N % BN == 0 &&
+            H <= up_dgrad_small_maxhw() && W <= up_dgrad_small_maxhw()) ? 1 : 0;
+}
+
+int dge_up_dgrad_small_launch(const ConvParams& p0, hipStream_t s) {
+    ConvParams p = p0;
+    p.dbg = 0;
+    p.tiles_x = (p.W + TW - 1) / TW;
+    p.tiles_y = (p.H + TH - 1) / TH;
+    DGE_CHECK(p.in_t2d && p.w_frag && !p.up && !p.in_s2d && !p.in_up2 && !p.in_scale && !p.in_shift && !p.noise && p.Ntot == p.Cout,
+              "up_dgrad_small: bad launch");
+    const long grid = (long)p.tiles_x * p.tiles_y * p.B * (p.Ntot / BN);
+    DGE_CHECK(grid > 0 && grid < (1L << 31), "up_dgrad_small: bad grid");
+    if (p.stats)
+        DGE_CHECK(dge_det_fits((long long)p.B * (p.Ntot / BN), (long long)p.tiles_x * p.tiles_y * 2, BN * 2),
+                  "up_dgrad_small: the deterministic-mode workspace is too small for this launch");
+    dge_note_kernel("conv_small<bf16,8,8,64,%d>+t2d%s", p.Cin, p.prep ? "+prep" : "");
+    const int mode = p.prep ? 2 : ((p.addend || p.dot_src) ? 1 : 0);
+#define DGE_GO(KQ, MODE) hipLaunchKernelGGL((conv_small_t2d_kernel<KQ, MODE>), dim3((unsigned)grid), dim3(512), 0, s, p)
+    if (p.Cin == 512) { if (mode == 2) DGE_GO(8, 2); else if (mode == 1) DGE_GO(8, 1); else DGE_GO(8, 0); }
+    else { if (mode == 2) DGE_GO(4, 2); else if (mode == 1) DGE_GO(4, 1); else DGE_GO(4, 0); }
+#undef DGE_GO
+    DGE_LAUNCH_CHECK("up_dgrad_small");
+    return 0;
+}
diff --git a/deep-gan-encoders_amd/csrc/s2_kernels.hip b/deep-gan-encoders_amd/csrc/s2_kernels.hip
--- a/deep-gan-encoders_amd/csrc/s2_kernels.hip
+++ b/deep-gan-encoders_amd/csrc/s2_kernels.hip
@@ -44,6 +44,11 @@
     return w[((size_t)o * Cin + i) * 9 + (2 - ky) * 3 + (2 - kx)];
 }
 
+__device__ __forceinline__ float upt2d_unit_weight(const float* __restrict__ w, int o, int i, int Cin, int unit) {
+    const int ky = (0x158a0 >> (2 * unit)) & 3, kx = (0x18588 >> (2 * unit)) & 3;
+    return w[((size_t)o * Cin + i) * 9 + (2 - ky) * 3 + (2 - kx)];
+}
+
 __device__ __forceinline__ size_t pack_out_index(int frag, int tap, int n, int k, int Ntot, int Kdim) {
     if (!frag) return ((size_t)tap * Ntot + n) * Kdim + k;
     const size_t blk = ((size_t)tap * (Ntot >> 5) + (n >> 5)) * (Kdim >> 4) + (k >> 4);
@@ -56,7 +61,7 @@
     const int frag = mode & 0x100;
     mode &= 0xff;
     const int ntap = KS * KS;
-    const int Kdim = (mode == 2) ? Cout : ((mode == 3 || mode == 5 || mode == 6) ? 4 * Cout : Cin);
+    const int Kdim = (mode == 2 || mode == 7) ? Cout : ((mode == 3 || mode == 5 || mode == 6) ? 4 * Cout : Cin);
     const int total = ntap * Ntot * Kdim;
     for (int idx = blockIdx.x * blockDim.x + threadIdx.x; idx < total; idx += gridDim.x * blockDim.x) {
         const int k = idx % Kdim;
@@ -75,6 +80,8 @@
             if (n < Cin) v = sg1_up_weight(w, n, k % Cout, Cout, k / Cout, 8 - tap);
         } else if (mode == 6) {
             if (n < Cin) v = upt2d_weight(w, k % Cout, n, Cin, k / Cout, tap);
+        } else if (mode == 7) {
+            if (n < Cin) v = upt2d_unit_weight(w, k, n, Cin, tap);
         } else {
             if (n < Cin) v = upfold_weight(w, k % Cout, n, Cin, k / Cout, 8 - tap);
         }
@@ -98,6 +105,7 @@
     if (mode == 4) return n < 4 * Cout ? sg1_up_weight(w, k, n % Cout, Cout, n / Cout, tap) : 0.f;
     if (mode == 5) return n < Cin ? sg1_up_weight(w, n, k % Cout, Cout, k / Cout, 8 - tap) : 0.f;
     if (mode == 6) return n < Cin ? upt2d_weight(w, k % Cout, n, Cin, k / Cout, tap) : 0.f;
+    if (mode == 7) return n < Cin ? upt2d_unit_weight(w, k, n, Cin, tap) : 0.f;
     return n < Cin ? upfold_weight(w, k % Cout, n, Cin, k / Cout, 8 - tap) : 0.f;
 }
 __global__ void pack_multi_kernel(const DgePackDesc* __restrict__ descs, int nd, long long total_pairs) {
@@ -483,11 +491,11 @@
     const int frag = mode & 0x100;
     const int mode_full = mode;
     mode &= 0xff;
-    DGE_CHECK(mode >= 0 && mode <= 6 && (mode_full & ~0x1ff) == 0, "pack: bad mode %d", mode_full);
+    DGE_CHECK(mode >= 0 && mode <= 7 && (mode_full & ~0x1ff) == 0, "pack: bad mode %d", mode_full);
     DGE_CHECK((mode != 1 && mode < 3) || ksize == 3, "pack: up fold needs a 3x3 kernel");
     const int nvalid = (mode == 1 || mode == 4) ? 4 * cout : (mode >= 2 ? cin : cout);
     const int ntot = dge_packed_n(nvalid);
-    const int kdim = mode == 2 ? cout : ((mode == 3 || mode == 5 || mode == 6) ? 4 * cout : cin);
+    const int kdim = (mode == 2 || mode == 7) ? cout : ((mode == 3 || mode == 5 || mode == 6) ? 4 * cout : cin);
     DGE_CHECK(!frag || (dtype == DGE_BF16 && ntot % 32 == 0 && kdim % 16 == 0), "pack: fragment order needs bf16, N %% 32 == 0, K %% 16 == 0");
     mode = mode_full;
     const long total = (long)ksize * ksize * ntot * kdim;
@@ -515,11 +523,11 @@
         d.dtype = (int)r[4];
         const unsigned bits = (unsigned)r[5]; memcpy(&d.scale, &bits, 4);
         const int bm = d.mode & 0xff;
-        DGE_CHECK(bm >= 0 && bm <= 6 && (d.mode & ~0x1ff) == 0, "pack_multi: bad mode %d", d.mode);
+        DGE_CHECK(bm >= 0 && bm <= 7 && (d.mode & ~0x1ff) == 0, "pack_multi: bad mode %d", d.mode);
         DGE_CHECK((bm != 1 && bm < 3) || d.ks == 3, "pack_multi: up fold needs a 3x3 kernel");
         const int nvalid = (bm == 1 || bm == 4) ? 4 * d.cout : (bm >= 2 ? d.cin : d.cout);
         d.ntot = dge_packed_n(nvalid);
-        d.kdim = bm == 2 ? d.cout : ((bm == 3 || bm == 5 || bm == 6) ? 4 * d.cout : d.cin);
+        d.kdim = (bm == 2 || bm == 7) ? d.cout : ((bm == 3 || bm == 5 || bm == 6) ? 4 * d.cout : d.cin);
         DGE_CHECK(!(d.mode & 0x100) || (d.dtype == DGE_BF16 && d.ntot % 32 == 0 && d.kdim % 16 == 0),
                   "pack_multi: fragment order needs bf16, N %% 32 == 0, K %% 16 == 0");
         d.pair_start = pairs;
diff --git a/deep-gan-encoders_amd/ops.py b/deep-gan-encoders_amd/ops.py
--- a/deep-gan-encoders_amd/ops.py
+++ b/deep-gan-encoders_amd/ops.py
@@ -8,6 +8,7 @@
 F32, BF16 = 0, 1
 ACT_NONE, ACT_LRELU, ACT_RELU, LIN_RSQRT = 0, 1, 2, 3
 PACK_FWD, PACK_UPFOLD, PACK_DGRAD, PACK_UPFOLD_DGRAD, PACK_SG1_UP, PACK_SG1_UP_DGRAD, PACK_UPT2D_DGRAD = 0, 1, 2, 3, 4, 5, 6
+PACK_UPT2D_UNITS = 7
 PACK_FRAG = 0x100
 import os as _os
 import weakref as _weakref
@@ -182,8 +183,8 @@
 def pack_dims(w, mode):
     cout, cin = _pack_io(w, mode)
     mode &= 0xff
-    nvalid = 4 * cout if mode in (PACK_UPFOLD, PACK_SG1_UP) else (cin if mode in (PACK_DGRAD, PACK_UPFOLD_DGRAD, PACK_SG1_UP_DGRAD, PACK_UPT2D_DGRAD) else cout)
-    kdim = cout if mode == PACK_DGRAD else (4 * cout if mode in (PACK_UPFOLD_DGRAD, PACK_SG1_UP_DGRAD, PACK_UPT2D_DGRAD) else cin)
+    nvalid = 4 * cout if mode in (PACK_UPFOLD, PACK_SG1_UP) else (cin if mode in (PACK_DGRAD, PACK_UPFOLD_DGRAD, PACK_SG1_UP_DGRAD, PACK_UPT2D_DGRAD, PACK_UPT2D_UNITS) else cout)
+    kdim = cout if mode in (PACK_DGRAD, PACK_UPT2D_UNITS) else (4 * cout if mode in (PACK_UPFOLD_DGRAD, PACK_SG1_UP_DGRAD, PACK_UPT2D_DGRAD) else cin)
     return nvalid, kdim
 
 
@@ -1259,6 +1260,57 @@
     return out
 
 
+UP_DGRAD_SMALL_UNITS = ((0, 0), (0, 2), (2, 0), (2, 2), (0, 1), (2, 1), (1, 0), (1, 2), (1, 1))
+
+
+def up_dgrad_small_supported(B, Hin, Win, cin, cout, dtype):
+    return (not is_deterministic()) and bool(lib().dge_up_dgrad_small_supported(int(B), int(Hin), int(Win), int(cout), int(cin), int(dtype)))
+
+
+def pack_up_dgrad_small(w, dtype=BF16, scale=1.0):
+    if dtype != BF16:
+        raise DgeError("pack_up_dgrad_small: bf16 only")
+    return pack_conv_weight(w, PACK_UPT2D_UNITS | PACK_FRAG, dtype, scale)
+
+
+def up_dgrad_small(z_t2d, w_packed, out_scale, addend, stats, dot_src, prep=None):
+    B, H1, W1, C4 = z_t2d.shape
+    H, W, cout = H1 - 1, W1 - 1, C4 // 4
+    cin = w_packed.shape[1]
+    dt = dtype_of(z_t2d)
+    if not getattr(w_packed, "_dge_frag", False) or tuple(w_packed.shape) != (9, cin, cout) or w_packed.dtype != z_t2d.dtype:
+        raise DgeError("up_dgrad_small: w_packed must be pack_up_dgrad_small's copy of this layer's weight")
+    if (dot_src is None) != (stats is None):
+        raise DgeError("up_dgrad_small: stats and dot_src come together")
+    if not up_dgrad_small_supported(B, H, W, cin, cout, dt):
+        raise DgeError(f"up_dgrad_small: unsupported launch {cin} <- {cout} channels on {H}x{W}, dtype {dt}")
+    out = torch.empty((B, H, W, cin), dtype=z_t2d.dtype, device=z_t2d.device)
+    d = ConvDesc()
+    d.in_t2d, d.w_layout, d.ksize = 1, 1, 3
+    d.x, d.w_packed, d.y, d.addend, d.dot_src = _p(z_t2d), _p(w_packed), _p(out), _p(addend), _p(dot_src)
+    d.out_scale = _f32(out_scale)
+    partial, nslot = None, 1
+    lazy = isinstance(stats, SlotStats)
+    if stats is not None:
+        nslot = _stats_slots(B, H, W, 16)
+        partial = stats.alloc(nslot) if lazy else (zeros((nslot,) + tuple(stats.shape), z_t2d.device) if nslot > 1 else stats)
+    d.stats, d.stats_slots = _f32(partial), nslot
+    d.B, d.H, d.W, d.Cin, d.Cout = B, H, W, C4, cin
+    nxt = _PREFETCH.link(_stream().value or 0, w_packed)
+    if nxt is not None:
+        d.prefetch_w, d.prefetch_ntot, d.prefetch_cin = C.c_void_p(nxt[0]), int(nxt[1]), int(nxt[2])
+    if prep is not None:
+        if stats is None:
+            raise DgeError("up_dgrad_small: prep needs stats and dot_src")
+        _set_prep(d, prep, nslot)
+    d.noise_batch, d.act, d.bias_scale, d.gain, d.add_scale, d.dtype = 1, ACT_NONE, 1.0, 1.0, 1.0, dt
+    _launch(lib().dge_up_dgrad_small, (C.byref(d), _stream()), "dge_up_dgrad_small", 9.0 * cin * cout * H * W * B,
+            (B, H, W, C4, cin, 3, False, True), (z_t2d, out, addend, dot_src, w_packed), log=True)
+    if partial is not None and not lazy and partial is not stats:
+        check(lib().dge_sum_slots(_p(partial), _p(stats), nslot, stats.numel(), 1, _stream()), "dge_sum_slots")
+    return out
+
+
 TRACK_ARM_AT, TRACK_ARM_AFTER = 0, 1
 
 
diff --git a/deep-gan-encoders_amd/s2_conv.py b/deep-gan-encoders_amd/s2_conv.py
--- a/deep-gan-encoders_amd/s2_conv.py
+++ b/deep-gan-encoders_amd/s2_conv.py
@@ -9,6 +9,7 @@
 T2D = not os.environ.get("DGE_NO_T2D")
 PP_DG = not os.environ.get("DGE_NO_PP_DG")
 UP_DG_STREAM = not os.environ.get("DGE_NO_UP_DG_STREAM")
+UP_DG_SMALL = not os.environ.get("DGE_NO_UP_DG_SMALL")
 
 
 def prepared(L, dtype):
@@ -88,6 +89,15 @@
     return c if c is not None else store(L._cache, ("dgs", dtype), L.weight, ops.pack_up_dgrad_stream(L.weight, dtype, L.wscale))
 
 
+def _up_small_dgrad(L, B, dtype, fused):
+    return UP_DG_SMALL and fused and L.up and L.ksize == 3 and ops.up_dgrad_small_supported(B, L.res // 2, L.res // 2, L.in_c, L.out_c, dtype)
+
+
+def _dgrad_weight_small(L, dtype):
+    c = lookup(L._cache, ("dgu", dtype), L.weight)
+    return c if c is not None else store(L._cache, ("dgu", dtype), L.weight, ops.pack_up_dgrad_small(L.weight, dtype, L.wscale))
+
+
 def dgrad_takes_prep(L, B=None, dtype=None):
     if B is not None and L.up and _up_stream_dgrad(L, B, dtype, not ops.is_deterministic()):
         return True
@@ -100,6 +110,9 @@
             and set(epilogue) <= {"out_scale", "addend", "stats", "dot_src"}:
         return ops.up_dgrad_stream(g_y, _dgrad_weight_stream(L, dt), d_in, epilogue.get("out_scale"), epilogue.get("addend"),
                                    epilogue.get("stats"), epilogue["dot_src"], prep=prep)
+    if L.up and _up_small_dgrad(L, B, dt, fused) and set(epilogue) <= {"out_scale", "addend", "stats", "dot_src"}:
+        return ops.up_dgrad_small(ops.fir_t2d(g_y, d_in), _dgrad_weight_small(L, dt), epilogue.get("out_scale"), epilogue.get("addend"),
+                                  epilogue.get("stats"), epilogue.get("dot_src"), prep=prep)
     t2d = _up_phase_form(L)
     if fused and d_in is not None and not t2d and _pp_dgrad(L, B, hg, dt):
         return ops.conv_pp(g_y, _dgrad_weight_pp(L, d_in), L.in_c, dgrad=True, in_s2d=L.up, add_scale=1.0, prep=prep, **epilogue)
diff --git a/include/dge_hip.h b/include/dge_hip.h
--- a/include/dge_hip.h
+++ b/include/dge_hip.h
@@ -20,6 +20,7 @@
 #define DGE_PACK_SG1_UP 4
 #define DGE_PACK_SG1_UP_DGRAD 5
 #define DGE_PACK_UPT2D_DGRAD 6
+#define DGE_PACK_UPT2D_UNITS 7
 
 const char* dge_last_error(void);
 int dge_version(void);
@@ -274,6 +275,9 @@
                         const float* prep_noise, int prep_noise_bstride, const float* prep_ns, float* prep_stats,
                         int B, int H, int W, int Cin, int Cout, int dtype, dge_stream_t stream);
 
+int dge_up_dgrad_small_supported(int B, int H, int W, int C, int N, int dtype);
+int dge_up_dgrad_small(const dge_conv_desc* d, dge_stream_t stream);
+
 int dge_up_pp_supported(int B, int H, int W, int Cin, int Cout, int dtype);
 int dge_pack_up_pp(const void* w_units, void* out, int Cout, int Cin, const float* in_scale, const float* out_scale, float gain,
                    int nb, dge_stream_t stream);
```

After: 387.9 images/sec (median of 6 runs). 1.3% higher.
